# subtotechnoblade/Grok_Alpha_Zero

Measured on AMD Instinct MI355X. Metric: self-play positions/sec (whole node), Connect4 200 sims/move, 1/2/4/8 GPU, higher is better.
Workload: dtype bf16; 1 GPU; Connect4 6x7, 4096 concurrent games/GPU, 200 sims/move (MCTS.run iteration_limit), 6-block x128 ResNet bf16, puct self-play, random-init weights; games_per_gpu=4096, sims_per_move=200, evaluator=resnet

## Files before the change

### grok_alpha_zero_amd/build.py

```python
import os
import subprocess
from concurrent.futures import ThreadPoolExecutor

_PKG = os.path.dirname(os.path.abspath(__file__))
CSRC = os.path.join(_PKG, "csrc")
OBJ = os.path.join(CSRC, "build")
LIB = os.path.join(_PKG, "libgaz_engine.so")
HEADER = os.path.join(os.path.dirname(_PKG), "include", "gaz_engine.h")
UNITS = {
    "engine.hip": ["rt.hpp", "wave.hpp", "det.hpp", "games.hpp", "tree.hpp", "resign.hpp", "puct_core.hpp", "gumbel_core.hpp", "evaluator.hpp", "samples.hpp", "tree_export.hpp"],
    "resnet.hip": ["rt.hpp", "wave.hpp", "evaluator.hpp", "netops.hpp", "conv3x3.hpp", "conv_wide.hpp", "resblock.hpp", "trunk.hpp", "tile_perm.hpp", "net_host.hpp",
                   "det.hpp", "games.hpp", "tree.hpp", "resign.hpp", "puct_core.hpp", "gumbel_core.hpp"],
}
FLAGS = ["-O3", "--offload-arch=gfx950", "-fPIC", "-std=c++17", "-ffp-contract=off", "-Wno-unused-result", "-Wno-unused-value",
         "-Wno-int-to-pointer-cast"]


def _newer(target, deps):
    if not os.path.exists(target):
        return True
    t = os.path.getmtime(target)
    return any(os.path.getmtime(d) > t for d in deps)


def build_engine(force=False, verbose=False):
    hipcc = os.environ.get("HIPCC", "/opt/rocm/bin/hipcc")
    os.makedirs(OBJ, exist_ok=True)
    known = {h for hs in UNITS.values() for h in hs} | set(UNITS)
    extra = [f for f in os.listdir(CSRC) if f.endswith((".hpp", ".hip")) and f not in known]
    jobs = []
    for src, hdrs in UNITS.items():
        obj = os.path.join(OBJ, src.replace(".hip", ".o"))
        deps = [os.path.join(CSRC, src), HEADER, os.path.abspath(__file__)] + [os.path.join(CSRC, h) for h in hdrs + extra]
        if force or _newer(obj, deps):
            jobs.append([hipcc] + FLAGS + ["-c", os.path.join(CSRC, src), "-o", obj])

    def run(cmd):
        if verbose:
            print(" ".join(cmd), flush=True)
        subprocess.check_call(cmd, cwd=CSRC)
    with ThreadPoolExecutor(max_workers=max(len(jobs), 1)) as ex:
        list(ex.map(run, jobs))
    objs = [os.path.join(OBJ, s.replace(".hip", ".o")) for s in UNITS]
    if jobs or _newer(LIB, objs):
        run([hipcc, "--offload-arch=gfx950", "-shared", "-fPIC"] + objs + ["-o", LIB])
    return LIB
```

### grok_alpha_zero_amd/csrc/engine.hip

```cpp
#include <stdio.h>
#include <functional>
#include <string>
#include <vector>
#include "../../include/gaz_engine.h"
#include "rt.hpp"
#include "puct_core.hpp"
#include "gumbel_core.hpp"
#include "samples.hpp"
#include "tree_export.hpp"
#include "evaluator.hpp"

using namespace gaz;

static std::string g_create_error;

#define HIP_OK(expr)                                                                  \
    do { hipError_t _e = (expr); if (_e != hipSuccess) { return fail(std::string(#expr) + ": " + hipGetErrorString(_e)); } } while (0)

template <class G> GAZ_DEV void wave_body(const DevParams<G>& E, int g0, int g1) {
    constexpr int PER = WAVE / G::TEAM;
    GAZ_SHARED Scratch<G> S[PER];
    GAZ_SHARED PuctLocal<G> L[PER];
    const int t = team_in_wave<G>();
    const int g = g0 + block_id() * PER + t;
// ... 288 lines not shown
    atomic_add(reinterpret_cast<unsigned long long*>(out + 2), (unsigned long long)gs.n_evals);
    atomic_add(reinterpret_cast<unsigned long long*>(out + 4), (unsigned long long)gs.n_sims);
    atomic_add(reinterpret_cast<unsigned long long*>(out + 6), (unsigned long long)gs.n_plies);
    atomic_add(reinterpret_cast<unsigned long long*>(out + 8), (unsigned long long)gs.n_hits);
}

struct gaz_engine {
    gaz_engine_config cfg;
    std::string err;
    int grouped = 0;
    virtual void note_grouped() {}
    virtual ~gaz_engine() {}
    int fail(const std::string& m) { err = m; return 1; }
    virtual int init() = 0;
    virtual int load_weights(const gaz_tensor* t, int n) = 0;
    virtual int reset_games(const int32_t* slots, int n) = 0;
    virtual int run_move(int32_t* n_waiting) = 0;
    virtual int get_root_stats(uint32_t*, float*, float*, float*, uint32_t*, float*, int32_t*, int32_t*) = 0;
    virtual int apply_moves(const int32_t* moves) = 0;
    virtual int run_waves(int n) = 0;
    virtual int wave_begin() = 0;
    virtual int wave_end() = 0;
    virtual int batch_ptrs(void**, void**, void**) = 0;
    virtual int read_batch(int8_t*, int32_t*) = 0;
    virtual int batch_rows(int32_t*) = 0;
    virtual int write_outputs(const float*, const float*) = 0;
    virtual int evaluate(const int8_t*, int, float*, float*, int, double*) = 0;
    virtual int record_layout(gaz_record_layout*) = 0;
    virtual int drain(void* out, int max_records, int32_t* n_out) = 0;
    virtual int sample_layout(gaz_sample_layout*) = 0;
    virtual int drain_samples(int max_games, int64_t max_rows, int64_t plane_rows, int64_t row_base, int32_t* games, int8_t* boards, float* policies,
                              float* values, int32_t* n_games, int64_t* n_rows, int32_t* blocked_T) = 0;
    virtual int get_stats(uint64_t out[16]) = 0;
    virtual int synchronize() = 0;
    virtual int timing_reset(int enable) = 0;
    virtual int timing_get(double*, double*, double*, int64_t*, int64_t*) = 0;
    virtual int dominant(char*, int, double*) = 0;
    virtual int set_position(int, const int32_t*, int) = 0;
    virtual int set_search_params(int, int) = 0;
    virtual int stop_search(int) = 0;
    virtual int start_search() = 0;
    virtual int set_hyperparams(const gaz_search_hyperparams*) = 0;
    virtual int set_resignation(const gaz_resign_params*) = 0;
    virtual int get_resign_stats(uint64_t out[8]) = 0;
    virtual int set_eval_symmetry(int32_t mode) = 0;
    virtual int get_eval_symmetry(int32_t* mode) = 0;
    virtual int read_batch_symmetry(uint8_t* sym) = 0;
    virtual int set_solver(int32_t mode) = 0;
    virtual int get_solver(int32_t* mode) = 0;
    virtual int get_solver_stats(uint64_t out[8]) = 0;
    virtual int read_head_features(int, float*, float*, int32_t*, int32_t*) = 0;
    virtual int set_fused_wave(int) = 0;
    virtual int debug_fused_fault(int) = 0;
    virtual int read_positions(int32_t*, uint8_t*, int) = 0;
    typedef std::function<int(int64_t n_nodes, int64_t n_edges, gaz_tree_node** nodes, gaz_tree_edge** edges)> TreePlace;
    virtual int read_trees(const int32_t* slots, int n_slots, int tree, int max_depth, uint32_t min_visits, int64_t* node_first, int64_t* edge_first,
                           bool want_records, const TreePlace& place) = 0;
    virtual int read_pv(int tree, const int32_t* first_action, int max_len, uint8_t* actions, uint32_t* N, float* W, int32_t* len) = 0;
    int short_capacity(int64_t need_nodes, int64_t need_edges, int64_t max_nodes, int64_t max_edges) {
        return fail("read_trees: the export needs " + std::to_string(need_nodes) + " nodes and " + std::to_string(need_edges) + " edges, max_nodes is " +
                    std::to_string(max_nodes) + " and max_edges is " + std::to_string(max_edges));
    }
    virtual int repack(int32_t*, int32_t*) = 0;
    virtual int probe_rules(const int32_t*, const int32_t*, int, int, int8_t*, uint8_t*, int32_t*, int8_t*, int32_t*, const float*, float*) = 0;
};

struct CallScratch {
    std::vector<void*> p;
    ~CallScratch() { for (void* q : p) hipFree(q); }
    template <class T> T* get(size_t n) { void* q = nullptr; if (hipMalloc(&q, (n ? n : 1) * sizeof(T)) != hipSuccess) return nullptr; p.push_back(q); return (T*)q; }
};

static const char* group_fault(const gaz_engine_config& c, int k) {
    if (k < 2 || k > c.n_games) return "game_groups must be in [1, n_games]";
    if (c.sync_moves || c.evaluator == GAZ_EVAL_EXTERNAL) return "game_groups > 1 needs continuous self-play (sync_moves = 0) with a built-in evaluator";
    if (c.games_budget > 0 && c.games_budget < c.n_games) return "game_groups > 1 with a games_budget below n_games: a group could be left without a game (use game_groups = 1)";
    return nullptr;
}

static std::string config_fault(const gaz_engine_config& c, int groups) {
    if (c.game_groups < 0) return "game_groups must be >= 0";
    if (c.gumbel_batch < 0 || c.gumbel_batch > 64) return "gumbel_batch must be in [0, 64] (0 and 1 = one candidate of sequential halving per game and wave)";
    if (c.gumbel_batch > 1) {
        if (c.leaf_batch > 1) return "gumbel_batch > 1 cannot be combined with leaf_batch > 1";
        if (c.search != GAZ_SEARCH_GUMBEL) return "gumbel_batch > 1 needs search = GAZ_SEARCH_GUMBEL (the PUCT search has leaf_batch)";
        if (c.eval_cache_log2 > 0) return "gumbel_batch > 1 cannot be combined with eval_cache_log2 > 0";
        if (c.game_groups > 1) return "gumbel_batch > 1 cannot be combined with game_groups > 1";
    }
    if (c.leaf_batch < 0 || c.leaf_batch > 64) return "leaf_batch must be in [0, 64] (0 and 1 = one leaf per game and wave)";
    if (c.leaf_batch > 1) {
        if (c.search == GAZ_SEARCH_GUMBEL) return "leaf_batch > 1 needs search = GAZ_SEARCH_PUCT (the Gumbel search plans its simulations itself)";
        if (c.eval_cache_log2 > 0) return "leaf_batch > 1 cannot be combined with eval_cache_log2 > 0";
        if (c.game_groups > 1) return "leaf_batch > 1 cannot be combined with game_groups > 1";
    }
    if (c.fast_iterations < 0) return "fast_iterations must be >= 0 (0 = no playout cap), not " + std::to_string(c.fast_iterations);
    if (c.fast_iterations > c.run_iterations) return "fast_iterations (" + std::to_string(c.fast_iterations) + ") must not exceed run_iterations (" + std::to_string(c.run_iterations) + ")";
    if (c.fast_iterations > 0 && !(c.full_search_prob > 0.0 && c.full_search_prob <= 1.0)) return "full_search_prob must be in (0, 1] with fast_iterations > 0, not " + std::to_string(c.full_search_prob);
    if (c.fast_iterations == 0 && !(c.full_search_prob == 0.0)) return "full_search_prob must be 0 with fast_iterations = 0 (the playout cap is off)";
    if (c.fast_iterations > 0 && c.move_time_limit > 0.0) return "fast_iterations > 0 cannot be combined with move_time_limit > 0 (a timed move has no iteration cap to randomise)";
    if (c.forced_playouts_k != c.forced_playouts_k) return "forced_playouts_k must be a number (0 = no forced playouts), not NaN";
    if (c.forced_playouts_k < 0.0) return "forced_playouts_k must be >= 0 (0 = no forced playouts), not " + std::to_string(c.forced_playouts_k);
    if (c.forced_playouts_k > 1.7976931348623157e308) return "forced_playouts_k must be finite (KataGo uses 2), not infinity";
    if (c.forced_playouts_k > 0.0 && c.search == GAZ_SEARCH_GUMBEL) return "forced_playouts_k > 0 cannot be combined with search = GAZ_SEARCH_GUMBEL (sequential halving has no PUCT root to force playouts at)";
    if (groups > 1) { const char* g = group_fault(c, groups); return g ? g : ""; }
    int max_t = 0, n_act = 0;
    switch (c.game) {
// ... 188 lines not shown
        if (slots) {
            if (n > E.n_games) return fail("reset_games: too many slots");
            HIP_OK(hipMemcpyAsync(dSlots, slots, sizeof(int32_t) * n, hipMemcpyHostToDevice, stream));
            GAZ_LAUNCH(k_reset_games<G>, n, WAVE, stream, E, (const int32_t*)dSlots, n);
        } else {
            GAZ_LAUNCH(k_reset_games<G>, E.n_games, WAVE, stream, E, (const int32_t*)nullptr, E.n_games);
        }
        HIP_OK(hipGetLastError());
        return 0;
    }

    int new_event(hipEvent_t* e) { HIP_OK(hipEventCreate(e)); ev.push_back(*e); return 0; }
    static constexpr size_t MAX_TIMING_EVENTS = 1 << 16;

    bool prev_marked = false;
    DevParams<G> wave_params() { DevParams<G> P = E; P.wave_epoch = ++fuse_epoch; P.eval_done = prev_marked ? d_evaldone : nullptr; return P; }
    void launch_wave(hipStream_t st, int g0, int g1) { const DevParams<G> P = wave_params(); prev_marked = false; launch_wave(st, g0, g1, P); }
    void launch_wave(hipStream_t st, int g0, int g1, const DevParams<G>& E) {
        if (E.solver) { if (E.eval_symmetry) launch_wave_v<true, true>(st, g0, g1, E); else launch_wave_v<false, true>(st, g0, g1, E); return; }
        if (E.eval_symmetry) launch_wave_v<true>(st, g0, g1, E); else launch_wave_v<false>(st, g0, g1, E);
    }
    template <bool SYM, bool SOLVE = false> void launch_wave_v(hipStream_t st, int g0, int g1, const DevParams<G>& E) {
        typedef typename SolveSel<SOLVE, typename SymSel<SYM, typename PuctVariant<G>::type>::type>::type GP;
        typedef typename SolveSel<SOLVE, typename SymSel<SYM, G>::type>::type GS;
        if constexpr (!SOLVE) {
        if (gbk > 1) {
            constexpr int PER = WAVE / GP::TEAM;
            GAZ_LAUNCH(k_wave_gb<GP>, (g1 - g0 + PER - 1) / PER, WAVE, st, *reinterpret_cast<const DevParams<GP>*>(&E), GB, g0, g1);
            return;
        }
        if (lbk > 1) {
            constexpr int PER = WAVE / GP::TEAM;
            GAZ_LAUNCH(k_wave_lb<GP>, (g1 - g0 + PER - 1) / PER, WAVE, st, *reinterpret_cast<const DevParams<GP>*>(&E), LB, g0, g1);
            return;
        }
        if (cfg.search == GAZ_SEARCH_GUMBEL) {
            static const int gteams_env = env_int("GAZ_TREE_TEAMS", -1);
            constexpr int GPER = WAVE / GP::TEAM;
            if (GPER > 1 && gteams_env == 1) GAZ_LAUNCH(k_wave_gumbel_teams<GP>, (g1 - g0 + GPER - 1) / GPER, WAVE, st, *reinterpret_cast<const DevParams<GP>*>(&E), g0, g1);
            else GAZ_LAUNCH(k_wave_gumbel<GS>, g1 - g0, WAVE, st, *reinterpret_cast<const DevParams<GS>*>(&E), g0, g1);
            return;
        }
        }
        static const int teams_env = env_int("GAZ_TREE_TEAMS", -1);
        const bool teams = teams_env >= 0 ? teams_env != 0 : E.cache == nullptr;
        constexpr int PER = WAVE / GP::TEAM;
        if (PER > 1 && teams) GAZ_LAUNCH(k_wave_teams<GP>, (g1 - g0 + PER - 1) / PER, WAVE, st, *reinterpret_cast<const DevParams<GP>*>(&E), g0, g1);
        else GAZ_LAUNCH(k_wave<GS>, g1 - g0, WAVE, st, *reinterpret_cast<const DevParams<GS>*>(&E), g0, g1);
    }
    void launch_wave() { launch_wave(stream, 0, n_eff); }

    uint32_t* d_done = nullptr; uint32_t* d_evaldone = nullptr; int32_t* d_fault = nullptr;
    unsigned long long* d_queue = nullptr;
    uint32_t fuse_epoch = 0; int fuse_state = -1;
    uint64_t fuse_faults = 0;
    unsigned debug_fault_mod = 0;
    static constexpr unsigned SPIN_TICKS = 2000000;
    int poll_fuse_fault() {
        if (!d_fault) return 0;
        int32_t n = 0;
        HIP_OK(hipMemcpy(&n, d_fault, sizeof(n), hipMemcpyDeviceToHost));
        if (n) {
            fuse_faults += (uint64_t)n; n = 0; fuse_state = 0; debug_fault_mod = 0;
            fault_wave = waves_launched; fault_strikes++;
            HIP_OK(hipMemcpy(d_fault, &n, sizeof(n), hipMemcpyHostToDevice));
            fprintf(stderr, "[gaz_engine] fused tree + trunk launch: %llu trunk workgroup(s) gave up waiting for their games (dispatch order not as assumed); "
                            "falling back to separate launches%s\n", (unsigned long long)fuse_faults,
                    fault_strikes <= REARM_STRIKES ? " (the one-launch form is tried again after 20000 waves)" : " for good");
        }
        return 0;
    }
    int64_t waves_launched = 0, fault_wave = 0; int fault_strikes = 0;
    static constexpr int64_t REARM_WAVES = 20000; static constexpr int REARM_STRIKES = 2;
    bool can_fuse() {
        if (fuse_state == 0 && fault_strikes > 0 && fault_strikes <= REARM_STRIKES && d_queue_or_done() && waves_launched - fault_wave >= REARM_WAVES) fuse_state = 1;
        if (fuse_state >= 0) return fuse_state == 1;
        fuse_state = 0;
        if (lbk > 1) return false;
        static const bool off = !env_on("GAZ_FUSE_WAVE", true);
        typedef typename PuctVariant<G>::type GP;
        static const bool with_cache = env_on("GAZ_FUSE_CACHE", true);
        const bool gumbel = cfg.search == GAZ_SEARCH_GUMBEL;
        const bool gmk = G::ID == GAME_GMK && !gumbel && !E.cache && env_on("GAZ_FUSE_GOMOKU", true);
        const bool c4 = G::ID == GAME_C4 && WAVE / GP::TEAM >= 4 && !E.compact && !(E.cache && !with_cache);
        if (off || !(c4 || gmk) || !eval || !eval->supports_split()) return false;
        if (gumbel && (!env_on("GAZ_FUSE_GUMBEL", true) || E.cache)) return false;
        if (!gumbel && !env_on("GAZ_TREE_TEAMS", true)) return false;
        if (dalloc(&d_done, (size_t)E.n_games) || !ensure_skip_buffers()) return false;
        if (env_on("GAZ_FUSE_QUEUE", true) && dalloc(&d_queue, (size_t)E.n_games + 64)) return false;
        fuse_state = 1;
        return true;
    }

    bool d_queue_or_done() const { return d_done != nullptr; }
    bool fuse_enabled = true;
    int set_fused_wave(int on) override { fuse_enabled = on != 0; return 0; }
    bool ensure_skip_buffers() {
        if (d_evaldone) return true;
        if (dalloc(&d_evaldone, (size_t)E.n_games) || dalloc(&d_fault, 4)) return false;
        return true;
    }
    int debug_fused_fault(int mod) override {
        if (lbk > 1 && mod > 0) return fail(std::string("debug_fused_fault: ") + (gbk > 1 ? "gumbel_batch" : "leaf_batch") + " > 1 runs separate launches only");
        if (mod > 0 && !ensure_skip_buffers()) return 1;
        debug_fault_mod = mod > 0 ? (unsigned)mod : 0u;
        return 0;
    }

    int n_eff = 0;
    int32_t* dMoveList = nullptr;
    int repack(int32_t* n_active_out, int32_t* n_eff_out) override {
        if (E.sync_moves) return fail("repack needs continuous self-play (sync_moves = 0)");
        if (gbk > 1) return fail("repack: not with gumbel_batch > 1 (a game owns gumbel_batch rows of the batch)");
        if (lbk > 1) return fail("repack: not with leaf_batch > 1 (a game owns leaf_batch rows of the batch)");
        if (quiesce()) return 1;
        GAZ_LAUNCH(k_gather_root<G>, E.n_games, WAVE, stream, E, dN, dW, dP, dPol, dRV, dQ, dChosen, dPhase, dPending);
        std::vector<int32_t> ph(E.n_games);
        HIP_OK(hipMemcpyAsync(ph.data(), dPhase, (size_t)E.n_games * 4, hipMemcpyDeviceToHost, stream));
        HIP_OK(hipStreamSynchronize(stream));
        int n_active = 0;
        for (int g = 0; g < n_eff; ++g) n_active += ph[g] != PH_HALT;
        for (int g = n_eff; g < E.n_games; ++g) if (ph[g] != PH_HALT) return fail("repack: a slot beyond the live range is running");
        if (n_active_out) *n_active_out = n_active;
        const int n_new = n_active > 0 ? n_active : 1;
        std::vector<int32_t> mv;
        int hole = 0;
        for (int g = n_eff - 1; g >= n_new; --g) {
            if (ph[g] == PH_HALT) continue;
            while (hole < n_new && ph[hole] != PH_HALT) ++hole;
            if (hole >= n_new) return fail("repack: internal error (no hole left)");
            mv.push_back(g); mv.push_back(hole); ph[hole] = ph[g]; ph[g] = PH_HALT;
        }
        if (!mv.empty()) {
            if (!dMoveList && dalloc(&dMoveList, (size_t)2 * E.n_games)) return 1;
            HIP_OK(hipMemcpyAsync(dMoveList, mv.data(), mv.size() * 4, hipMemcpyHostToDevice, stream));
            const size_t slot_bytes = (size_t)2 * (E.compact ? 2 : 1) * (size_t)E.nodes_per_tree * (size_t)E.node_bytes;
            const size_t gbytes = cfg.search == GAZ_SEARCH_GUMBEL ? sizeof(GumbelState<G>) : 0;
            DevParams<G> Em = E; Em.eval_done = d_evaldone;
            GAZ_LAUNCH(k_move_slots<G>, (int)(mv.size() / 2), 256, stream, Em, (const int32_t*)dMoveList, (int)(mv.size() / 2), slot_bytes, gbytes);
            HIP_OK(hipGetLastError());
            HIP_OK(hipStreamSynchronize(stream));
        }
        n_eff = n_new;
        if (n_eff_out) *n_eff_out = n_eff;
        return 0;
    }

    int fused_wave(bool timing, hipEvent_t e0, hipEvent_t e1, hipEvent_t e2) {
        static const char* stamp_spec = getenv("GAZ_FUSED_STAMPS");
        static const long stamp_at = stamp_spec && strchr(stamp_spec, ':') ? atol(strchr(stamp_spec, ':') + 1) : 3000;
        unsigned long long* d_stamps = nullptr;
        const size_t stamp_blocks = (size_t)n_eff + 4096;
        if (stamp_spec && n_waves_total == stamp_at && hipMalloc((void**)&d_stamps, stamp_blocks * 128 * 8) == hipSuccess) hipMemsetAsync(d_stamps, 0, stamp_blocks * 128 * 8, stream);
        const FuseHandoff ho{d_done, fuse_epoch + 1, d_evaldone, d_fault, SPIN_TICKS, debug_fault_mod, d_stamps, d_queue};
        const void* plan = eval->trunk_plan(E.nn_in, n_eff, 0, ho);
        if (!plan) return -1;
        if (timing) hipEventRecord(e0, stream);
        DevParams<G> Ef = wave_params(); Ef.done_flag = d_done;
        if (eval->plan_uses_queue(plan)) {
            typedef typename PuctVariant<G>::type GPq;
            static const bool gumbel_teams = env_on("GAZ_FUSE_GUMBEL_TEAMS", true);
            static const int rounds_env = env_int("GAZ_FUSE_TREE_ROUNDS", 0);
            const int rounds = rounds_env > 0 ? rounds_env : (G::ID == GAME_GMK ? (this->grouped > 1 ? 4 : 8) : (cfg.search == GAZ_SEARCH_GUMBEL ? (this->grouped > 1 ? 2 : 4) : 1));
            const int gpb = G::ID == GAME_GMK ? rounds * 8 : rounds * 4 * ((cfg.search == GAZ_SEARCH_GUMBEL && !gumbel_teams) ? 1 : WAVE / GPq::TEAM);
            Ef.done_queue = d_queue; Ef.queue_gpb = gpb; Ef.queue_nfull = n_eff / gpb; Ef.queue_rem = n_eff % gpb;
        }
        Ef.handoff_release = G::ID == GAME_GMK;
        const bool launched = G::ID == GAME_GMK ? launch_wave_trunk_gmk(stream, &Ef, 0, n_eff, plan)
                            : cfg.search == GAZ_SEARCH_GUMBEL ? launch_wave_trunk_c4_gumbel(stream, &Ef, 0, n_eff, plan) : launch_wave_trunk_c4(stream, &Ef, 0, n_eff, plan);
        if (!launched) { fuse_state = 0; --fuse_epoch; return -1; }
        prev_marked = true;
        if (d_stamps) {
            std::vector<unsigned long long> hst(stamp_blocks * 128);
            hipStreamSynchronize(stream);
            hipMemcpy(hst.data(), d_stamps, hst.size() * 8, hipMemcpyDeviceToHost); hipFree(d_stamps);
            std::string path(stamp_spec); if (path.find(':') != std::string::npos) path = path.substr(0, path.find(':'));
            if (FILE* f = fopen(path.c_str(), "wb")) { fwrite(hst.data(), 8, hst.size(), f); fclose(f); }
        }
        if (timing) hipEventRecord(e1, stream);
        eval->forward_heads(stream, E.nn_policy, E.nn_value, n_eff, 0);
        if (E.cache) { Ef.eval_done = d_evaldone; GAZ_LAUNCH(k_cache_insert<G>, n_eff, WAVE, stream, Ef, 0, n_eff); E.cache_epoch++; }
        if (timing) {
            hipEventRecord(e2, stream); ev_eval.push_back({e0, e2}); n_waves_timed++;
            ev_fused.push_back({e0, e1});
        }
        n_waves_total++;
        return 0;
    }

    int one_wave(bool with_eval) {
        ++waves_launched;
        const bool timing = this->timing && n_waves_total % TIMING_STRIDE == 0 && ev.size() + 4 <= MAX_TIMING_EVENTS;
        hipEvent_t e0 = 0, e1 = 0, e2 = 0;
        if (timing && (new_event(&e0) || new_event(&e1) || new_event(&e2))) return 1;
        if (with_eval && eval && fuse_enabled && can_fuse()) { const int rc = fused_wave(timing, e0, e1, e2); if (rc >= 0) return rc; }
        if (timing) hipEventRecord(e0, stream);
        DevParams<G> P = wave_params();
        launch_wave(stream, 0, n_eff, P);
        prev_marked = false;
        if (timing) hipEventRecord(e1, stream);
        if (with_eval && eval) eval->forward(stream, E.nn_in, E.nn_policy, E.nn_value, n_eff * lbk, timing);
        if (timing) { hipEventRecord(e2, stream); ev_tree.push_back({e0, e1}); ev_eval.push_back({e1, e2}); n_waves_timed++; }
        P.eval_done = nullptr;
        if (with_eval && eval && debug_fault_mod && d_evaldone) {
            GAZ_LAUNCH(k_debug_skip<G>, n_eff, WAVE, stream, P, d_evaldone, n_eff, debug_fault_mod, d_fault);
            prev_marked = true; P.eval_done = d_evaldone;
        }
        if (with_eval && eval && E.cache) { GAZ_LAUNCH(k_cache_insert<G>, n_eff, WAVE, stream, P, 0, n_eff); E.cache_epoch++; }
        n_waves_total++;
        return 0;
    }

    hipStream_t tstream = 0, hstream = 0;
    static constexpr int MAXGRP = 8;
    int n_grp = 0, grp0[MAXGRP + 1] = {};
    hipEvent_t ev_tree_done[2][MAXGRP] = {}, ev_trunk_done[2][MAXGRP] = {}, ev_heads_done[2][MAXGRP] = {}, ev_join = 0;
    bool pipeline_ready = false;
    int quiesce() { HIP_OK(hipStreamSynchronize(stream)); if (pipeline_ready) { HIP_OK(hipStreamSynchronize(tstream)); HIP_OK(hipStreamSynchronize(hstream)); } return 0; }
    bool can_pipeline() {
        static const char* spec = getenv("GAZ_PIPELINE");
        if (!spec || !*spec || atoi(spec) == 0) return false;
        if (lbk > 1 || E.sync_moves || !eval || !eval->supports_split() || E.n_games < 1024 || E.cache || n_eff != E.n_games) return false;
        if (!pipeline_ready) {
            std::vector<int> sizes;
            if (strchr(spec, ',')) { for (const char* p = spec; *p;) { sizes.push_back(atoi(p)); p = strchr(p, ','); if (!p) break; ++p; } }
            else { const int round = eval->round_rows(); for (int left = E.n_games; left > 0; left -= round) sizes.push_back(left < round ? left : round); }
            int sum = 0; for (int v : sizes) sum += v;
            if (sizes.size() < 2 || sizes.size() > (size_t)MAXGRP || sum != E.n_games) return false;
            for (int v : sizes) if (v <= 0) return false;
            n_grp = (int)sizes.size(); grp0[0] = 0;
            for (int i = 0; i < n_grp; ++i) grp0[i + 1] = grp0[i] + sizes[i];
            int lo = 0, hi = 0;
            hipDeviceGetStreamPriorityRange(&lo, &hi);
// ... 684 lines not shown
        for (int c = 0; c < K(); ++c) {
            uint64_t s[16];
            if (up(kid[c], kid[c]->get_stats(s))) return 1;
            if (s[0] > out[0]) out[0] = s[0];
            for (int i = 1; i < 9; ++i) out[i] += s[i];
            out[10] += s[10]; out[13] += s[13];
            if (s[9] > out[9]) out[9] = s[9];
            if (!s[12]) out[12] = 0;
        }
        out[14] = (uint64_t)K();
        return 0;
    }
    int synchronize() override { return all(&gaz_engine::synchronize); }
    int timing_reset(int en) override { return all(&gaz_engine::timing_reset, en); }
    int timing_get(double* ms_tree, double* ms_eval, double* ms_dom, int64_t* n_dom, int64_t* n_waves) override {
        double t = 0, e = 0, d = 0; int64_t nd = 0, nw = 0;
        for (int c = 0; c < K(); ++c) {
            double a = 0, b = 0, x = 0; int64_t y = 0, z = 0;
            if (up(kid[c], kid[c]->timing_get(&a, &b, &x, &y, &z))) return 1;
            t += a; e += b; d += x; nd += y; if (z > nw) nw = z;
        }
        if (ms_tree) *ms_tree = t; if (ms_eval) *ms_eval = e; if (ms_dom) *ms_dom = d; if (n_dom) *n_dom = nd; if (n_waves) *n_waves = nw;
        return 0;
    }
    int dominant(char* name, int cap, double* flops) override { return lead(&gaz_engine::dominant, name, cap, flops); }
    int set_position(int slot, const int32_t* a, int n) override {
        if (slot < 0 || slot >= cfg.n_games) return fail("set_position: bad slot / history length");
        const int c = group_of(slot);
        return up(kid[c], kid[c]->set_position(slot - first[c], a, n));
    }
    int set_search_params(int it, int tau) override { return all(&gaz_engine::set_search_params, it, tau); }
    int stop_search(int s) override { return all(&gaz_engine::stop_search, s); }
    int start_search() override { return all(&gaz_engine::start_search); }
    int set_hyperparams(const gaz_search_hyperparams* hp) override { return all(&gaz_engine::set_hyperparams, hp); }
    int set_resignation(const gaz_resign_params* p) override { return all(&gaz_engine::set_resignation, p); }
    int set_eval_symmetry(int32_t mode) override { return all(&gaz_engine::set_eval_symmetry, mode); }
    int get_eval_symmetry(int32_t* mode) override { return lead(&gaz_engine::get_eval_symmetry, mode); }
    int set_solver(int32_t mode) override { return all(&gaz_engine::set_solver, mode); }
    int get_solver(int32_t* mode) override { return lead(&gaz_engine::get_solver, mode); }
    int get_solver_stats(uint64_t out[8]) override { return sum8(&gaz_engine::get_solver_stats, out); }
    int get_resign_stats(uint64_t out[8]) override { return sum8(&gaz_engine::get_resign_stats, out); }
    int read_head_features(int n, float* p, float* v, int32_t* p_row, int32_t* v_row) override {
        if (n < 0 || n > cfg.n_games) return fail("read_head_features: n must be in [0, n_games]");
        int32_t pr = 0, vr = 0;
        if (lead(&gaz_engine::read_head_features, 0, nullptr, nullptr, &pr, &vr)) return 1;
        if (p_row) *p_row = pr; if (v_row) *v_row = vr;
        return each([&](gaz_engine* k, int c) {
            const int nc = rows_of(c, n);
            return nc ? k->read_head_features(nc, p ? p + (size_t)first[c] * pr : p, v ? v + (size_t)first[c] * vr : v, nullptr, nullptr) : 0;
        });
    }
    int set_fused_wave(int on) override { return all(&gaz_engine::set_fused_wave, on); }
    int debug_fused_fault(int mod) override { return all(&gaz_engine::debug_fused_fault, mod); }
    int read_positions(int32_t* n_hist, uint8_t* hist, int stride) override {
        if (!n_hist || !hist || stride < lay.max_T) return fail("read_positions: hist must hold at least max_T actions per slot");
        return each([&](gaz_engine* k, int c) { return k->read_positions(n_hist + first[c], hist + (size_t)first[c] * stride, stride); });
    }
    int read_trees(const int32_t* slots, int n, int tree, int max_depth, uint32_t min_visits, int64_t* node_first, int64_t* edge_first,
                   bool want_records, const TreePlace& place) override {
        std::vector<std::vector<int32_t>> local(K()), pos(K());
        for (int i = 0; i < n; ++i) { const int c = group_of(slots[i]); local[c].push_back(slots[i] - first[c]); pos[c].push_back(i); }
        std::vector<std::vector<int64_t>> nf(K()), ef(K());
        std::vector<std::vector<gaz_tree_node>> tn(K()); std::vector<std::vector<gaz_tree_edge>> te(K());
        std::vector<int64_t> cn((size_t)n, 0), ce((size_t)n, 0);
        for (int c = 0; c < K(); ++c) {
            const int m = (int)local[c].size();
            nf[c].assign((size_t)m + 1, 0); ef[c].assign((size_t)m + 1, 0);
            const TreePlace stage = [&, c](int64_t nn, int64_t ne, gaz_tree_node** pn, gaz_tree_edge** pe) {
                tn[c].resize((size_t)nn + 1); te[c].resize((size_t)ne + 1); *pn = tn[c].data(); *pe = te[c].data(); return 0;
            };
            if (up(kid[c], kid[c]->read_trees(local[c].data(), m, tree, max_depth, min_visits, nf[c].data(), ef[c].data(), want_records, stage))) return 1;
            for (int j = 0; j < m; ++j) { cn[pos[c][j]] = nf[c][j + 1] - nf[c][j]; ce[pos[c][j]] = ef[c][j + 1] - ef[c][j]; }
        }
        node_first[0] = 0; edge_first[0] = 0;
        for (int i = 0; i < n; ++i) { node_first[i + 1] = node_first[i] + cn[i]; edge_first[i + 1] = edge_first[i] + ce[i]; }
        if (!want_records) return 0;
        gaz_tree_node* nodes = nullptr; gaz_tree_edge* edges = nullptr;
        if (place(node_first[n], edge_first[n], &nodes, &edges)) return 1;
        for (int c = 0; c < K(); ++c)
            for (size_t j = 0; j < pos[c].size(); ++j) {
                const int i = pos[c][j];
                if (cn[i]) memcpy(nodes + node_first[i], tn[c].data() + nf[c][j], sizeof(gaz_tree_node) * (size_t)cn[i]);
                if (ce[i]) memcpy(edges + edge_first[i], te[c].data() + ef[c][j], sizeof(gaz_tree_edge) * (size_t)ce[i]);
            }
        return 0;
    }
    int read_pv(int tree, const int32_t* fa, int max_len, uint8_t* actions, uint32_t* N, float* W, int32_t* len) override {
        return each([&](gaz_engine* k, int c) {
            const size_t o = (size_t)first[c] * (size_t)max_len;
            return k->read_pv(tree, fa ? fa + first[c] : fa, max_len, actions + o, N + o, W + o, len + first[c]);
        });
    }
    int repack(int32_t* n_active, int32_t* n_launch) override {
        int32_t a = 0, l = 0;
        if (each([&](gaz_engine* k, int) { int32_t x = 0, y = 0; if (k->repack(&x, &y)) return 1; a += x; l += y; return 0; })) return 1;
        if (n_active) *n_active = a; if (n_launch) *n_launch = l;
        return 0;
    }
    int probe_rules(const int32_t* actions, const int32_t* n_actions, int n_pos, int stride, int8_t* b, uint8_t* l, int32_t* w, int8_t* in, int32_t* t,
                    const float* pin, float* pout) override { return lead(&gaz_engine::probe_rules, actions, n_actions, n_pos, stride, b, l, w, in, t, pin, pout); }
};

static int choose_game_groups(const gaz_engine_config& c) {
    if (c.game_groups != 0) return c.game_groups;
    if (c.leaf_batch > 1 || c.gumbel_batch > 1) return 1;
    static const int env = env_int("GAZ_GAME_GROUPS", 0);
// ... 49 lines not shown
int gaz_engine_evaluate(gaz_engine* h, const int8_t* in, int32_t n, float* p, float* v, int32_t repeats, double* ms) { return h->evaluate(in, n, p, v, repeats, ms); }
int gaz_engine_record_layout(gaz_engine* h, gaz_record_layout* o) { return h->record_layout(o); }
int gaz_engine_drain_finished(gaz_engine* h, void* out, int32_t max_records, int32_t* n_out) { return h->drain(out, max_records, n_out); }
int gaz_engine_sample_layout(gaz_engine* h, gaz_sample_layout* o) { return o ? h->sample_layout(o) : h->fail("sample_layout: null argument"); }
int gaz_engine_drain_samples(gaz_engine* h, int32_t max_games, int64_t max_rows, int32_t* games, int8_t* boards, float* policies, float* values,
                             int32_t* n_games, int64_t* n_rows) {
    if (!games || !boards || !policies || !values || !n_games || !n_rows) return h->fail("drain_samples: null argument");
    if (max_games < 0 || max_rows < 0) return h->fail("drain_samples: max_games and max_rows must be >= 0");
    int32_t blocked = 0;
    if (h->drain_samples(max_games, max_rows, max_rows, 0, games, boards, policies, values, n_games, n_rows, &blocked)) return 1;
    if (*n_games == 0 && blocked)
        return h->fail("drain_samples: the oldest finished game has " + std::to_string(blocked) + " rows, max_rows is " + std::to_string(max_rows) +
                       " (no game was taken: call again with room for at least max_T rows)");
    return 0;
}
int gaz_engine_get_stats(gaz_engine* h, uint64_t out[16]) { return h->get_stats(out); }
int gaz_engine_synchronize(gaz_engine* h) { return h->synchronize(); }
int gaz_engine_timing_reset(gaz_engine* h, int32_t enable) { return h->timing_reset(enable); }
int gaz_engine_set_position(gaz_engine* h, int32_t slot, const int32_t* actions, int32_t n) { return h->set_position(slot, actions, n); }
int gaz_engine_set_search_params(gaz_engine* h, int32_t run_iterations, int32_t tau_mode) { return h->set_search_params(run_iterations, tau_mode); }
int gaz_engine_stop_search(gaz_engine* h, int32_t stop) { return h->stop_search(stop); }
int gaz_engine_start_search(gaz_engine* h) { return h->start_search(); }
int gaz_engine_set_hyperparams(gaz_engine* h, const gaz_search_hyperparams* hp) { return h->set_hyperparams(hp); }
int gaz_engine_set_resignation(gaz_engine* h, const gaz_resign_params* p) {
    if (!p) return h->fail("set_resignation: null argument");
    if (p->struct_size != sizeof(gaz_resign_params))
        return h->fail("set_resignation: struct_size is " + std::to_string(p->struct_size) + ", this library's gaz_resign_params has " + std::to_string(sizeof(gaz_resign_params)) + " bytes");
    if (p->threshold != p->threshold) return h->fail("set_resignation: threshold must be a number (0 = no resignation), not NaN");
    if (p->threshold > 1.7976931348623157e308 || p->threshold < -1.7976931348623157e308) return h->fail("set_resignation: threshold must be finite, not infinity");
    if (p->threshold < 0.0) return h->fail("set_resignation: threshold must be >= 0 (0 = no resignation), not " + std::to_string(p->threshold));
    if (p->threshold >= 1.0) return h->fail("set_resignation: threshold must be below 1 (q lies in [-1, 1], so no ply could trigger), not " + std::to_string(p->threshold));
    if (p->threshold == 0.0) return h->set_resignation(p);
    if (p->consecutive < 1 || p->consecutive > RESIGN_MAX_CONSECUTIVE)
        return h->fail("set_resignation: consecutive must be in [1, " + std::to_string(RESIGN_MAX_CONSECUTIVE) + "], not " + std::to_string(p->consecutive));
    if (p->min_ply < 0) return h->fail("set_resignation: min_ply must be >= 0, not " + std::to_string(p->min_ply));
    if (!(p->no_resign_prob >= 0.0 && p->no_resign_prob <= 1.0)) return h->fail("set_resignation: no_resign_prob must be in [0, 1], not " + std::to_string(p->no_resign_prob));
    return h->set_resignation(p);
}
int gaz_engine_get_resign_stats(gaz_engine* h, uint64_t out[8]) { return out ? h->get_resign_stats(out) : h->fail("get_resign_stats: null argument"); }
int gaz_engine_set_eval_symmetry(gaz_engine* h, int32_t mode) {
    if (mode != 0 && mode != 1) return h->fail("set_eval_symmetry: mode must be 0 (off) or 1 (a random board symmetry per evaluator request), not " + std::to_string(mode));
    return h->set_eval_symmetry(mode);
}
int gaz_engine_set_solver(gaz_engine* h, int32_t mode) {
    if (mode != 0 && mode != 1) return h->fail("set_solver: mode must be 0 (off) or 1 (prove wins, draws and losses in the PUCT tree), not " + std::to_string(mode));
    return h->set_solver(mode);
}
int gaz_engine_get_solver(gaz_engine* h, int32_t* mode) { return mode ? h->get_solver(mode) : h->fail("get_solver: null argument"); }
int gaz_engine_get_solver_stats(gaz_engine* h, uint64_t out[8]) { return out ? h->get_solver_stats(out) : h->fail("get_solver_stats: null argument"); }
int gaz_engine_get_eval_symmetry(gaz_engine* h, int32_t* mode) { return mode ? h->get_eval_symmetry(mode) : h->fail("get_eval_symmetry: null argument"); }
int gaz_engine_read_batch_symmetry(gaz_engine* h, uint8_t* sym) { return sym ? h->read_batch_symmetry(sym) : h->fail("read_batch_symmetry: null argument"); }
int gaz_engine_set_fused_wave(gaz_engine* h, int32_t on) { return h->set_fused_wave(on); }
int gaz_engine_debug_fused_fault(gaz_engine* h, int32_t mod) { return h->debug_fused_fault(mod); }
int gaz_engine_read_positions(gaz_engine* h, int32_t* n_hist, uint8_t* hist, int32_t stride) { return h->read_positions(n_hist, hist, stride); }
static int check_tree_arg(gaz_engine* h, const char* fn, int32_t tree) {
    if (tree < -1 || tree > 1) return h->fail(std::string(fn) + ": tree must be 0, 1 or -1 (the tree running the game's move), not " + std::to_string(tree));
    if (tree == 1 && (h->cfg.single_tree || h->cfg.search == GAZ_SEARCH_GUMBEL))
        return h->fail(std::string(fn) + ": tree = 1 on an engine with one tree per game (single_tree or the Gumbel search); use tree = 0 or -1");
    return 0;
}
int gaz_engine_read_trees(gaz_engine* h, const int32_t* slots, int32_t n_slots, int32_t tree, int32_t max_depth, uint32_t min_visits, int64_t max_nodes,
                          int64_t max_edges, gaz_tree_node* nodes, gaz_tree_edge* edges, int64_t* node_first, int64_t* edge_first) {
    if (n_slots < 0) return h->fail("read_trees: n_slots must be >= 0, not " + std::to_string(n_slots));
    if (!node_first || !edge_first || (n_slots > 0 && !slots)) return h->fail("read_trees: slots, node_first and edge_first must not be null");
    if (check_tree_arg(h, "read_trees", tree)) return 1;
    if ((nodes == nullptr) != (edges == nullptr)) return h->fail("read_trees: nodes and edges must both be given, or both be null (counting call)");
    if (nodes && (max_nodes < 0 || max_edges < 0)) return h->fail("read_trees: max_nodes and max_edges must be >= 0");
    for (int32_t i = 0; i < n_slots; ++i)
        if (slots[i] < 0 || slots[i] >= h->cfg.n_games)
            return h->fail("read_trees: slots[" + std::to_string(i) + "] = " + std::to_string(slots[i]) + " is out of range [0, " + std::to_string(h->cfg.n_games) + ")");
    const gaz_engine::TreePlace place = [&](int64_t nn, int64_t ne, gaz_tree_node** pn, gaz_tree_edge** pe) {
        if (nn > max_nodes || ne > max_edges) return h->short_capacity(nn, ne, max_nodes, max_edges);
        *pn = nodes; *pe = edges; return 0;
    };
    return h->read_trees(slots, n_slots, tree, max_depth, min_visits, node_first, edge_first, nodes != nullptr, place);
}
int gaz_engine_read_pv(gaz_engine* h, int32_t tree, const int32_t* first_action, int32_t max_len, uint8_t* actions, uint32_t* N, float* W, int32_t* len) {
    if (max_len <= 0) return h->fail("read_pv: max_len must be positive, not " + std::to_string(max_len));
    if (!actions || !N || !W || !len) return h->fail("read_pv: actions, N, W and len must not be null");
    if (check_tree_arg(h, "read_pv", tree)) return 1;
    return h->read_pv(tree, first_action, max_len, actions, N, W, len);
}
int gaz_engine_repack(gaz_engine* h, int32_t* n_active, int32_t* n_launch) { return h->repack(n_active, n_launch); }
int gaz_engine_read_head_features(gaz_engine* h, int32_t n, float* p, float* v, int32_t* p_row, int32_t* v_row) { return h->read_head_features(n, p, v, p_row, v_row); }
int gaz_engine_probe_rules(gaz_engine* h, const int32_t* actions, const int32_t* n_actions, int32_t n_positions, int32_t stride, int8_t* board,
                           uint8_t* legal, int32_t* winner, int8_t* input, int32_t* terminal, const float* policy_in, float* policy_out) {
    return h->probe_rules(actions, n_actions, n_positions, stride, board, legal, winner, input, terminal, policy_in, policy_out);
}
int gaz_engine_dominant_kernel(gaz_engine* h, char* name, int32_t cap, double* flops) { return h->dominant(name, cap, flops); }
int gaz_engine_timing_get(gaz_engine* h, double* a, double* b, double* c, int64_t* d, int64_t* e) { return h->timing_get(a, b, c, d, e); }

}
```

### grok_alpha_zero_amd/csrc/evaluator.hpp

```cpp
#pragma once
#include <string>
#include "../../include/gaz_engine.h"
#include "rt.hpp"

namespace gaz {

struct FuseHandoff { const unsigned* ready; unsigned epoch; unsigned* eval_done; int* fuse_fault; unsigned spin_ticks; unsigned test_fault_mod;
                     unsigned long long* stamps;
                     const unsigned long long* queue; };

struct Evaluator {
    virtual ~Evaluator() {}
    virtual int load(const gaz_tensor* t, int n, hipStream_t s, std::string* err) { (void)t; (void)n; (void)s; (void)err; return 0; }
    virtual void forward(hipStream_t s, const int8_t* in, float* policy, float* value, int n, bool timing, int p0 = 0) = 0;
    virtual bool supports_row_base() const { return false; }
    virtual bool supports_split() const { return false; }
    virtual int round_rows() const { return 0; }
    virtual void forward_trunk(hipStream_t s, const int8_t* in, int n, bool timing, int p0) { (void)s; (void)in; (void)n; (void)timing; (void)p0; }
    virtual void forward_heads(hipStream_t s, float* policy, float* value, int n, int p0) { (void)s; (void)policy; (void)value; (void)n; (void)p0; }
    virtual const void* trunk_plan(const int8_t* in, int n, int p0, const struct FuseHandoff& h) { (void)in; (void)n; (void)p0; (void)h; return nullptr; }
    virtual bool plan_uses_queue(const void* plan) const { (void)plan; return false; }
    virtual void set_shared_chip(bool on) { (void)on; }
    virtual bool ready() const { return true; }
    virtual void timing_reset() {}
    virtual void timing_get(double* ms, int64_t* launches) { *ms = 0; *launches = 0; }
    virtual const char* dominant_kernel(int n, double* flops) { (void)n; *flops = 0; return ""; }
    virtual bool head_features(const float** p_feat, const float** v_feat, int* p_row_floats, int* v_row_floats) { (void)p_feat; (void)v_feat; (void)p_row_floats; (void)v_row_floats; return false; }
};

GAZ_DEV uint32_t hash_row(const int8_t* s, int n, uint32_t seed) {
    uint32_t h = 2166136261u ^ seed;
    for (int i = 0; i < n; ++i) { h ^= (uint8_t)s[i]; h *= 16777619u; }
    h ^= h >> 16; h *= 0x85EBCA6Bu; h ^= h >> 13; h *= 0xC2B2AE35u; h ^= h >> 16;
    return h;
}

template <int UNUSED> GAZ_KERNEL_WIDE k_hash_eval(const int8_t* in, float* policy, float* value, int n, int row_bytes, int A, uint32_t salt) {
#ifdef GAZ_HOST_EMU
    const int first = block_id(), step = 1 << 30;
#else
    const int first = blockIdx.x * blockDim.x + threadIdx.x, step = gridDim.x * blockDim.x;
#endif
    for (int idx = first; idx < n * (A + 1); idx += step) {
        const int g = idx / (A + 1), a = idx % (A + 1);
        const int8_t* row = in + (size_t)g * row_bytes;
        if (a < A) {
            uint32_t h = hash_row(row, row_bytes, salt ^ ((uint32_t)(a + 1) * 0x9E3779B1u));
            policy[(size_t)g * A + a] = (float)((h >> 8) + 1u) * (1.0f / 16777216.0f);
        } else {
            uint32_t h = hash_row(row, row_bytes, salt ^ 0x51ED270Bu);
            value[g] = (float)(h >> 8) * (1.0f / 8388608.0f) - 1.0f;
        }
    }
}

struct HashEvaluator : Evaluator {
    int row_bytes, A; uint32_t salt;
    HashEvaluator(int rb, int a, uint32_t s) : row_bytes(rb), A(a), salt(s) {}
    void forward(hipStream_t s, const int8_t* in, float* policy, float* value, int n, bool, int = 0) override {
        const int total = n * (A + 1);
#ifdef GAZ_HOST_EMU
        GAZ_LAUNCH(k_hash_eval<0>, total, 1, s, in, policy, value, n, row_bytes, A, salt);
#else
        GAZ_LAUNCH(k_hash_eval<0>, (total + 255) / 256, 256, s, in, policy, value, n, row_bytes, A, salt);
#endif
    }
};

Evaluator* make_resnet_evaluator(const gaz_engine_config& cfg, int H, int W, int C, int A, std::string* err);
bool launch_wave_trunk_c4(hipStream_t s, const void* dev_params, int g0, int g1, const void* plan);
bool launch_wave_trunk_c4_gumbel(hipStream_t s, const void* dev_params, int g0, int g1, const void* plan);
bool launch_wave_trunk_gmk(hipStream_t s, const void* dev_params, int g0, int g1, const void* plan);

inline Evaluator* make_evaluator(const gaz_engine_config& cfg, int H, int W, int C, int A, std::string* err) {
// ... 9 lines not shown
```

### grok_alpha_zero_amd/csrc/resnet.hip

```cpp
#include <math.h>
#include <map>
#include <string>
#include <vector>
#include <algorithm>
#include "evaluator.hpp"
#include "conv3x3.hpp"
#include "conv_wide.hpp"
#include "netops.hpp"
#include "resblock.hpp"
#include "trunk.hpp"
#include "tile_perm.hpp"
#include "net_host.hpp"
#include "puct_core.hpp"
#include "gumbel_core.hpp"

namespace gaz {

struct Rb3Plan { int tm, halo, tile_rows; };
static Rb3Plan rb3_plan(int M, int H, int W, int n_cus) {
    Rb3Plan best{3, W + 1, 64 * 3 - 2 * (W + 1)}; double best_cost = 1e30;
    for (int aligned = 0; aligned < 2; ++aligned)
        for (int c = 2; c <= 4; ++c) {
            const int rows = aligned ? (64 * c / (H * W)) * (H * W) : 64 * c - 2 * (W + 1);
            if (rows <= 0) continue;
// ... 281 lines not shown
            const size_t rb = (size_t)min(b0 + p, a.B - 1) * F;
#pragma unroll
            for (int c = 0; c < 6; ++c) v[pi][c] = feat[rb + min(lane + 64 * c, F - 1)];
        }
#pragma unroll
        for (int pi = 0; pi < 4; ++pi) {
            const int p = wave + 8 * pi;
            const bool rok = b0 + p < a.B;
#pragma unroll
            for (int c = 0; c < 6; ++c) { const int k = lane + 64 * c; if (k < FP) fl[p * FP + k] = (rok && k < F) ? v[pi][c] : 0.0f; }
        }
        for (int p = wave; p < 32; p += 8)
            for (int k = lane + 64 * 6; k < FP; k += 64) fl[p * FP + k] = (b0 + p < a.B && k < F) ? feat[(size_t)min(b0 + p, a.B - 1) * F + k] : 0.0f;
    }
    __syncthreads();
    f32x16 acc;
#pragma unroll
    for (int r = 0; r < 16; ++r) acc[r] = 0.0f;
    for (int g0 = gA; g0 < gB; g0 += D) {
#pragma unroll
        for (int d = 0; d < D; ++d) {
            const int g = g0 + d;
            ldg(g + D - 1, bq[(d + D - 1) % D]);
            if (g < gB) {
                float av[G];
#pragma unroll
                for (int j = 0; j < G; ++j) av[j] = fl[l31 * FP + g * 2 * G + 2 * j + lhi];
#pragma unroll
                for (int j = 0; j < G; ++j) acc = __builtin_amdgcn_mfma_f32_32x32x2f32(av[j], bq[d][j], acc, 0, 0, 0);
            }
        }
    }
    float* part = fl + 32 * FP;
    if (half) {
#pragma unroll
        for (int r = 0; r < 16; ++r) part[(wq * 16 + r) * 64 + lane] = acc[r];
    }
    __syncthreads();
    if (half) return;
    const float s = a.scale[head][n], t = a.shift[head][n];
#pragma unroll
    for (int r = 0; r < 16; ++r) {
        const int row = (r & 3) + 8 * (r >> 2) + 4 * lhi;
        if (b0 + row < a.B) a.out[head][(size_t)(b0 + row) * 128 + n] = fmaxf((acc[r] + part[(wq * 16 + r) * 64 + lane]) * s + t, 0.0f);
    }
}

struct TailArgs {
    const float* p_d1; const float* v_d1;
    const float* p_w2; const float* p_b2; const float* p_w3; const float* p_b3;
    const float* v_w2; const float* v_b2; const float* v_w3; const float* v_b3;
    float* policy; float* value; int B, A, logits;
};
__device__ __forceinline__ float policy_entry(const float* lg, int nout, int o, int logits) {
    if (logits == 1) return lg[o];
    if (logits == 2) {
        float sum = 0.f;
        for (int k = 0; k < nout; ++k) { const float x = lg[k]; sum += x >= 0.0f ? x + 1.0f : 1.0f / (1.0f - x); }
        const float x = lg[o];
        return (x >= 0.0f ? x + 1.0f : 1.0f / (1.0f - x)) / sum;
    }
    float mx = lg[0];
    for (int k = 1; k < nout; ++k) mx = fmaxf(mx, lg[k]);
    float sum = 0.f;
    for (int k = 0; k < nout; ++k) sum += expf(lg[k] - mx);
    return expf(lg[o] - mx) / sum;
}
__global__ __launch_bounds__(128) void k_tail(TailArgs a) {
    __shared__ float w2l[128 * 64]; __shared__ float xl[16][128]; __shared__ float hl[16][64]; __shared__ float lg[16][64];
    __shared__ float w3l[64 * 8];
    const int head = blockIdx.y, tid = threadIdx.x, p = tid >> 3, q = tid & 7, b0 = blockIdx.x * 16;
    const float* d1 = head == 0 ? a.p_d1 : a.v_d1;
    const float* w2 = head == 0 ? a.p_w2 : a.v_w2; const float* b2 = head == 0 ? a.p_b2 : a.v_b2;
    const float* w3 = head == 0 ? a.p_w3 : a.v_w3; const float* b3 = head == 0 ? a.p_b3 : a.v_b3;
    const int nout = head == 0 ? a.A : 1;
    {
        float4 wv[16], xv[4];
#pragma unroll
        for (int c = 0; c < 16; ++c) wv[c] = reinterpret_cast<const float4*>(w2)[tid + 128 * c];
#pragma unroll
        for (int c = 0; c < 4; ++c) {
            const int i = tid + 128 * c, pp = min(b0 + i / 32, a.B - 1);
            xv[c] = reinterpret_cast<const float4*>(d1 + (size_t)pp * 128)[i % 32];
        }
#pragma unroll
        for (int c = 0; c < 16; ++c) reinterpret_cast<float4*>(w2l)[tid + 128 * c] = wv[c];
#pragma unroll
        for (int c = 0; c < 4; ++c) reinterpret_cast<float4*>(&xl[0][0])[tid + 128 * c] = xv[c];
        if (nout <= 8) {
            float w3v[4];
#pragma unroll
            for (int c = 0; c < 4; ++c) w3v[c] = w3[min(tid + 128 * c, 64 * nout - 1)];
#pragma unroll
            for (int c = 0; c < 4; ++c) w3l[tid + 128 * c] = w3v[c];
        }
    }
    __syncthreads();
    float acc[8];
#pragma unroll
    for (int j = 0; j < 8; ++j) acc[j] = b2[q * 8 + j];
    for (int k = 0; k < 128; ++k) {
        const float xv = xl[p][k];
        const float4 wa = *reinterpret_cast<const float4*>(&w2l[k * 64 + q * 8]), wb = *reinterpret_cast<const float4*>(&w2l[k * 64 + q * 8 + 4]);
        acc[0] += xv * wa.x; acc[1] += xv * wa.y; acc[2] += xv * wa.z; acc[3] += xv * wa.w;
        acc[4] += xv * wb.x; acc[5] += xv * wb.y; acc[6] += xv * wb.z; acc[7] += xv * wb.w;
    }
#pragma unroll
    for (int j = 0; j < 8; ++j) hl[p][q * 8 + j] = acc[j];
    __syncthreads();
    for (int o = q; o < nout; o += 8) {
        float z = b3[o];
        if (nout <= 8) { for (int k = 0; k < 64; ++k) z += hl[p][k] * w3l[k * nout + o]; }
        else { for (int k = 0; k < 64; ++k) z += hl[p][k] * w3[k * nout + o]; }
        lg[p][o] = z;
    }
    __syncthreads();
    if (b0 + p >= a.B) return;
    const int b = b0 + p;
    if (head == 0) {
        for (int o = q; o < nout; o += 8) a.policy[(size_t)b * a.A + o] = policy_entry(lg[p], nout, o, a.logits);
    } else if (q == 0) {
        a.value[b] = tanhf(lg[p][0]);
    }
}

struct HeadsC4Args {
    const float* feat[2]; const float* w1[2]; const float* s1[2]; const float* t1[2];
    const float* w2[2]; const float* b2[2]; const float* w3[2]; const float* b3[2];
    float* policy; float* value; int B, F, A, logits;
};
constexpr int HC4_THREADS = 256, HC4_POS = 32, HC4_XP = 132;
constexpr int HC4_FCH = 6, HC4_TAIL = 128 * 64 + HC4_POS * 64 + HC4_POS * 8;
static size_t heads_c4_lds_bytes(int F) { return (size_t)(std::max(HC4_POS * (F + 1), HC4_TAIL) + HC4_POS * HC4_XP + 64 * 8) * 4; }
__global__ __launch_bounds__(HC4_THREADS) void k_heads_c4(HeadsC4Args a) {
    typedef __attribute__((ext_vector_type(4))) float f32x4;
    extern __shared__ float fl[];
    constexpr int D = 12;
    const int tid = threadIdx.x, F = a.F, FP = F + 1, F4 = F >> 2;
    float* const w2l = fl; float* const hl = fl + 128 * 64; float* const lg = hl + HC4_POS * 64;
    float* const xl = fl + max(HC4_POS * FP, HC4_TAIL);
    float* const w3l = xl + HC4_POS * HC4_XP;
    const int lane = tid & 63, wave = tid >> 6, c = lane & 15, kq = lane >> 4, half = wave >> 1, n0 = (wave & 1) * 64 + c * 4;
    const int NG = F >> 4, NGH = (NG + 1) / 2, sA = half ? NGH * 4 : 0, sB = half ? NG * 4 : NGH * 4;
    const int p = tid >> 3, q = tid & 7;
    const int items = 2 * ((a.B + HC4_POS - 1) / HC4_POS);
    for (int item = blockIdx.x; item < items; item += gridDim.x) {
        const int head = item & 1, b0 = (item >> 1) * HC4_POS, nout = head == 0 ? a.A : 1;
        const float* feat = a.feat[head]; const float* w1 = a.w1[head]; const float* w3 = a.w3[head];
        float4 bq[D]; f32x4 wv[8];
        auto ldw = [&](int s) { return *reinterpret_cast<const float4*>(w1 + (size_t)min(4 * s + kq, F - 1) * 128 + n0); };
#pragma unroll
        for (int d = 0; d < D - 1; ++d) bq[d] = ldw(sA + d);
        {
            float w3v[2];
#pragma unroll
            for (int i = 0; i < 2; ++i) w3v[i] = w3[min(tid + HC4_THREADS * i, 64 * nout - 1)];
#pragma unroll 1
            for (int e0 = tid; e0 < HC4_POS * F4; e0 += HC4_THREADS * HC4_FCH) {
                float4 fv[HC4_FCH];
#pragma unroll
                for (int i = 0; i < HC4_FCH; ++i) {
                    const int e = min(e0 + HC4_THREADS * i, HC4_POS * F4 - 1), r = e / F4;
                    fv[i] = reinterpret_cast<const float4*>(feat + (size_t)min(b0 + r, a.B - 1) * F)[e - r * F4];
                }
#pragma unroll
                for (int i = 0; i < HC4_FCH; ++i) {
                    const int e = e0 + HC4_THREADS * i, r = e / F4, k = (e - r * F4) * 4;
                    if (e < HC4_POS * F4) {
                        const bool rok = b0 + r < a.B;
                        float* dst = fl + r * FP + k;
                        dst[0] = rok ? fv[i].x : 0.0f; dst[1] = rok ? fv[i].y : 0.0f; dst[2] = rok ? fv[i].z : 0.0f; dst[3] = rok ? fv[i].w : 0.0f;
                    }
                }
            }
#pragma unroll
            for (int i = 0; i < 2; ++i) w3l[tid + HC4_THREADS * i] = w3v[i];
#pragma unroll
            for (int i = 0; i < 8; ++i) wv[i] = reinterpret_cast<const f32x4*>(a.w2[head])[tid + HC4_THREADS * i];
        }
        __syncthreads();
        f32x4 acc[2][4];
#pragma unroll
        for (int m = 0; m < 2; ++m)
#pragma unroll
            for (int t = 0; t < 4; ++t) acc[m][t] = f32x4{0.0f, 0.0f, 0.0f, 0.0f};
        for (int s0 = sA; s0 < sB; s0 += D) {
#pragma unroll
            for (int d = 0; d < D; ++d) {
                const int s = s0 + d;
                if (s + D - 1 < sB) bq[(d + D - 1) % D] = ldw(s + D - 1);
                if (s < sB) {
#pragma unroll
                    for (int m = 0; m < 2; ++m) {
                        const float av = fl[(16 * m + c) * FP + 4 * s + kq];
                        acc[m][0] = __builtin_amdgcn_mfma_f32_16x16x4f32(av, bq[d].x, acc[m][0], 0, 0, 0);
                        acc[m][1] = __builtin_amdgcn_mfma_f32_16x16x4f32(av, bq[d].y, acc[m][1], 0, 0, 0);
                        acc[m][2] = __builtin_amdgcn_mfma_f32_16x16x4f32(av, bq[d].z, acc[m][2], 0, 0, 0);
                        acc[m][3] = __builtin_amdgcn_mfma_f32_16x16x4f32(av, bq[d].w, acc[m][3], 0, 0, 0);
                    }
                }
            }
        }
        if (half) {
#pragma unroll
            for (int m = 0; m < 2; ++m)
#pragma unroll
                for (int r = 0; r < 4; ++r)
                    *reinterpret_cast<float4*>(&xl[(16 * m + 4 * kq + r) * HC4_XP + n0]) = make_float4(acc[m][0][r], acc[m][1][r], acc[m][2][r], acc[m][3][r]);
        }
        __syncthreads();
        if (!half) {
            const float4 s = *reinterpret_cast<const float4*>(a.s1[head] + n0), t = *reinterpret_cast<const float4*>(a.t1[head] + n0);
#pragma unroll
            for (int m = 0; m < 2; ++m)
#pragma unroll
                for (int r = 0; r < 4; ++r) {
                    float4* x = reinterpret_cast<float4*>(&xl[(16 * m + 4 * kq + r) * HC4_XP + n0]);
                    const float4 pv = *x;
                    *x = make_float4(fmaxf((acc[m][0][r] + pv.x) * s.x + t.x, 0.0f), fmaxf((acc[m][1][r] + pv.y) * s.y + t.y, 0.0f),
                                     fmaxf((acc[m][2][r] + pv.z) * s.z + t.z, 0.0f), fmaxf((acc[m][3][r] + pv.w) * s.w + t.w, 0.0f));
                }
        }
#pragma unroll
        for (int i = 0; i < 8; ++i) reinterpret_cast<f32x4*>(w2l)[tid + HC4_THREADS * i] = wv[i];
        __syncthreads();
        {
            const float* b2 = a.b2[head];
            float h[8];
#pragma unroll
            for (int j = 0; j < 8; ++j) h[j] = b2[q * 8 + j];
            for (int k = 0; k < 128; ++k) {
                const float xv = xl[p * HC4_XP + k];
                const float4 wa = *reinterpret_cast<const float4*>(&w2l[k * 64 + q * 8]), wb = *reinterpret_cast<const float4*>(&w2l[k * 64 + q * 8 + 4]);
                h[0] += xv * wa.x; h[1] += xv * wa.y; h[2] += xv * wa.z; h[3] += xv * wa.w;
                h[4] += xv * wb.x; h[5] += xv * wb.y; h[6] += xv * wb.z; h[7] += xv * wb.w;
            }
#pragma unroll
            for (int j = 0; j < 8; ++j) hl[p * 64 + q * 8 + j] = h[j];
        }
        __syncthreads();
        for (int o = q; o < nout; o += 8) {
            float z = a.b3[head][o];
            for (int k = 0; k < 64; ++k) z += hl[p * 64 + k] * w3l[k * nout + o];
            lg[p * 8 + o] = z;
        }
        __syncthreads();
        const int b = b0 + p;
        if (b < a.B) {
            if (head == 0) { for (int o = q; o < nout; o += 8) a.policy[(size_t)b * a.A + o] = policy_entry(lg + p * 8, nout, o, a.logits); }
            else if (q == 0) a.value[b] = tanhf(lg[p * 8]);
        }
        __syncthreads();
    }
}

static bool net_width_supported(int f) { return f == 64 || f == 128 || f == 192 || f == 256; }
static std::string net_width_error(int f) {
    return "num_filters (net_filters) = " + std::to_string(f) + " is not supported: the Connect4 and Gomoku networks run num_filters in {64, 128, 192, 256}";
}

struct ResNetEvaluator : Evaluator {
    int H, W, C, A, HW, blocks, filters, nmax, logits;
    DeviceStore st;
    bf16_t *X = nullptr, *Aa = nullptr, *Hh = nullptr, *X2 = nullptr;
    bool fused = true;
    int stamp_calls = 0, n_cus = 256;
    bf16_t* stem_frag = nullptr;
    bool trunk_m16 = true;
    bool trunk_mix = true;
    bool trunk_whole = true;
    bool trunk = true;
    bool heads_one = true;
    int heads_wgs = 128;
    int heads_one_rows = 2048;
    bf16_t* trunk_w = nullptr; float* trunk_prm = nullptr;
    std::string dom_label;
    uint8_t *perm_big = nullptr, *perm_small = nullptr;
    unsigned boff_big = 0, boff_small = 0; int perm_clashes = 0;
    float *pfeat = nullptr, *vfeat = nullptr, *pd1 = nullptr, *vd1 = nullptr;
    bool loaded = false;
    TrunkTimer timer;
    int64_t n_trunk_launches = 0;

    int load(const gaz_tensor* t, int n, hipStream_t s, std::string* err) override {
        st.set_tensors(t, n);
        if (!load_tensors()) { *err = st.err; return 1; }
        hipStreamSynchronize(s);
        loaded = true;
        return 0;
    }
    bool load_tensors() {
        const int Fc = filters, F = HW * 8;
        if (!st.up_f32("stem.w", 9 * 128 * C) || !st.up_f32("stem.scale", 128) || !st.up_f32("stem.shift", 128)) return false;
        {
            if (C != 4) { st.err = "stem expects 4 input planes"; return false; }
            const std::vector<bf16_t> h = stem_fragments(st.by["stem.w"]->data, st.by["stem.scale"]->data, 4, 128);
            if (!(stem_frag = st.upload(h.data(), h.size()))) return false;
        }
        for (int i = 0; i < blocks; ++i) {
            const std::string b = "block" + std::to_string(i); const int cin = i == 0 && Fc != 128 ? 128 : Fc;
            if (!st.up_f32(b + ".bn1.scale", cin) || !st.up_f32(b + ".bn1.shift", cin)) return false;
            if (Fc == 128 ? !st.up_conv_pair(b + ".conv1.w", b + ".conv2.w", Fc)
                          : !st.up_conv(b + ".conv1.w", Fc, cin, 9, CONV_WIDE) || !st.up_conv(b + ".conv2.w", Fc, Fc, 9, CONV_WIDE)) return false;
            if (!st.up_f32(b + ".conv1.scale", Fc) || !st.up_f32(b + ".conv1.shift", Fc) || !st.up_f32(b + ".conv2.bias", Fc)) return false;
        }
        if (Fc != 128 && (!st.up_conv("block0.proj.w", Fc, 128, 1, CONV_WIDE) || !st.up_f32("block0.proj.bias", Fc) ||
                          !st.up_bias_sum("block0.bias2p", "block0.conv2.bias", "block0.proj.bias"))) return false;
        if (Fc == 128 && !st.pack_trunk(0, blocks, &trunk_w, &trunk_prm)) return false;
        if (env_on("GAZ_TILE_PERM", true) && !perm_big && 96 / HW >= 1 && Fc == 128) {
            unsigned want_big[8] = {0x007u, 0x049u, 0, 0, 0x1C0u, 0x124u, 0, 0}, want_small[6] = {0x007u, 0x1C0u, 0x049u, 0, 0, 0};
            const TileLayout lb = tile_layout(H, W, 128 / HW, 128, 64, 2, want_big), ls = tile_layout(H, W, 96 / HW, 96, 96, 3, want_small);
            const bool ok = !lb.perm.empty() && !ls.perm.empty() && lb.boff.size() <= 3 && ls.boff.size() <= 3;
            if (ok && (perm_big = st.upload(lb.perm.data(), lb.perm.size())) && (perm_small = st.upload(ls.perm.data(), ls.perm.size()))) {
                boff_big = boff_small = 0;
                for (size_t b = 0; b < lb.boff.size(); ++b) boff_big |= (unsigned)lb.boff[b] << (8 * b);
                for (size_t b = 0; b < ls.boff.size(); ++b) boff_small |= (unsigned)ls.boff[b] << (8 * b);
                perm_clashes = lb.clashes + ls.clashes;
            } else { perm_big = perm_small = nullptr; }
        }
        if (!st.up_conv("heads.conv.w", 32, Fc, 9, Fc == 128 ? CONV_MFMA : CONV_WIDE) || !st.up_f32("heads.conv.bias", 32)) return false;
        for (const char* pre : {"p", "v"}) {
            const std::string p = pre; const int nout = p == "p" ? A : 1;
            if (!st.up_f32(p + ".bn0.scale", F) || !st.up_f32(p + ".bn0.shift", F) || !st.up_f32(p + ".d1.w", (int64_t)F * 128) ||
                !st.up_f32(p + ".d1.scale", 128) || !st.up_f32(p + ".d1.shift", 128) || !st.up_f32(p + ".d2.w", 128 * 64) ||
                !st.up_f32(p + ".d2.bias", 64) || !st.up_f32(p + ".d3.w", 64 * nout) || !st.up_f32(p + ".d3.bias", nout)) return false;
        }
        return true;
    }

    void conv_trunk(hipStream_t s, const bf16_t* in, const bf16_t* w, const float* sA, const float* tA, const bf16_t* res,
                    bf16_t* out1, int act1, const float* sB, const float* tB, bf16_t* out2, int M) {
        ConvArgs a; memset(&a, 0, sizeof(a));
        a.in = in; a.wgt = w; a.scaleA = sA; a.shiftA = tA; a.res = res; a.out1 = out1; a.act1 = act1;
        a.scaleB = sB; a.shiftB = tB; a.out2 = out2; a.M = M; a.H = H; a.W = W;
        static const int variant = env_int("GAZ_CONV_VARIANT", 0);
        if (variant == 0) {
            const size_t lds = conv_lds_bytes<128, 128, 256, 1>();
            hipLaunchKernelGGL((k_conv3x3<128, 128, 256, 4, 2, 2, 2, 1, 1, 0>), dim3((M + 255) / 256), dim3(512), lds, s, a);
        } else {
            const size_t lds = conv_lds_bytes<128, 128, 128, 2>();
            hipLaunchKernelGGL((k_conv3x3<128, 128, 128, 2, 2, 2, 2, 2, 2, 0>), dim3((M + 127) / 128), dim3(256), lds, s, a);
        }
        n_trunk_launches++;
    }

    bool supports_row_base() const override { return true; }
    bool head_features(const float** p, const float** v, int* pr, int* vr) override { *p = pfeat; *v = vfeat; *pr = HW * 8; *vr = HW * 8; return true; }
    bool supports_split() const override { return filters == 128 && fused && trunk && trunk_whole && blocks > 0 && HW <= 128; }
    void make_trunk_plan(const int8_t* in, int n, int p0, bool mix_allowed, bool fill_big, TrunkLaunchPlan& P) {
        TrunkArgs& r = P.args; memset(&r, 0, sizeof(r));
        r.xin = this->X + (size_t)p0 * HW * 128; r.xout = this->X2 + (size_t)p0 * HW * 128; r.w = trunk_w; r.prm = trunk_prm; r.M = n * HW; r.H = H; r.W = W; r.nblocks = blocks;
        r.tile_rows = (128 / HW) * HW; r.stamps = nullptr; r.perm = perm_big; r.perm_small = perm_small; r.boff = boff_big; r.boff_small = boff_small;
        r.planes = in; r.stem_frag = reinterpret_cast<const uint4*>(stem_frag); r.stem_shift = st.g("stem.shift");
        r.hw = st.w("heads.conv.w"); r.hbias = st.g("heads.conv.bias"); r.p_fs = st.g("p.bn0.scale"); r.p_ft = st.g("p.bn0.shift");
        r.v_fs = st.g("v.bn0.scale"); r.v_ft = st.g("v.bn0.shift");
        r.p_feat = this->pfeat + (size_t)p0 * HW * 8; r.v_feat = this->vfeat + (size_t)p0 * HW * 8;
        const TrunkSplit sp = trunk_split(n, HW, n_cus, mix_allowed, fill_big);
        if (sp.mix) { r.n_big = sp.n_big; r.small_rows = (96 / HW) * HW; }
        P.nwg = sp.nwg; P.mix = sp.mix; P.lds_bytes = (unsigned)trunk_lds_bytes(128);
    }
    TrunkLaunchPlan fused_plan;
    const void* trunk_plan(const int8_t* in, int n, int p0, const FuseHandoff& h) override {
        if (!trunk_m16 || !loaded || !supports_split()) return nullptr;
        make_trunk_plan(in, n, p0, trunk_mix, shared_chip && perm_big && perm_small, fused_plan);
        TrunkArgs& r = fused_plan.args;
        r.ready = h.ready; r.epoch = h.epoch; r.eval_done = h.eval_done; r.fuse_fault = h.fuse_fault; r.spin_ticks = h.spin_ticks; r.test_fault_mod = h.test_fault_mod; r.stamps = h.stamps;
        r.queue = (perm_big && perm_small && fused_plan.mix) ? h.queue : nullptr;
        return &fused_plan;
    }
    bool plan_uses_queue(const void* plan) const override { return plan && static_cast<const TrunkLaunchPlan*>(plan)->args.queue != nullptr; }
    bool shared_chip = false;
    bool grouped = false;
    void set_shared_chip(bool on) override { static const bool off = !env_on("GAZ_GROUP_BIG_TILES", true); shared_chip = on && !off; grouped = on; }
    int round_rows() const override { return 2 * n_cus * (128 / HW); }
    void forward(hipStream_t s, const int8_t* in, float* policy, float* value, int n, bool timing, int p0 = 0) override {
        forward_trunk(s, in, n, timing, p0);
        forward_heads(s, policy, value, n, p0);
    }
    void forward_trunk(hipStream_t s, const int8_t* in, int n, bool timing, int p0) override {
        if (!loaded) return;
        if (filters != 128) { forward_trunk_wide(s, in, n, timing, p0); return; }
        const int M = n * HW;
        bf16_t* const X = this->X + (size_t)p0 * HW * 128; bf16_t* const X2 = this->X2 + (size_t)p0 * HW * 128;
        bf16_t* const Aa = this->Aa + (size_t)p0 * HW * 128; bf16_t* const Hh = this->Hh + (size_t)p0 * HW * 128;
        float* const pfeat = this->pfeat + (size_t)p0 * HW * 8; float* const vfeat = this->vfeat + (size_t)p0 * HW * 8;
        StemArgs sa; sa.in = in; sa.w = st.g("stem.w"); sa.scale = st.g("stem.scale"); sa.shift = st.g("stem.shift");
        sa.scaleB = blocks ? st.g("block0.bn1.scale") : st.g("stem.scale"); sa.shiftB = blocks ? st.g("block0.bn1.shift") : st.g("stem.shift");
        sa.out1 = X; sa.out2 = fused ? nullptr : Aa; sa.M = M; sa.H = H; sa.W = W;
        const bool use_trunk = fused && trunk && blocks > 0 && HW <= 128;
        const bool whole = use_trunk && trunk_whole;
        if (whole) {
        } else if (fused) {
            StemMArgs sm; memset(&sm, 0, sizeof(sm)); sm.in = in; sm.wfrag = reinterpret_cast<const uint4*>(stem_frag); sm.shift = st.g("stem.shift"); sm.out = X;
            sm.M = M; sm.H = H; sm.W = W;
            launch_stem_mfma<4, 128, true, false>(s, sm);
        } else {
            hipLaunchKernelGGL(k_stem, dim3((M + 63) / 64), dim3(256), 0, s, sa);
        }
        timer.begin(s, timing);
        bf16_t* cur = X;
        if (use_trunk) {
            TrunkLaunchPlan P; make_trunk_plan(in, n, p0, whole && trunk_mix, false, P);
            TrunkArgs& r = P.args;
            const int nwg = P.nwg; const bool mix = P.mix;
            static const char* stamp_path = getenv("GAZ_TRUNK_STAMPS");
            StampDump stamps(stamp_path && ++stamp_calls == 3 ? stamp_path : nullptr, (size_t)nwg * 128, s);
            r.stamps = stamps.dev;
            if (mix && trunk_m16 && r.perm && r.perm_small) hipLaunchKernelGGL((k_trunk_mix<8, 2, true, true, true, true>), dim3(nwg), dim3(TR_THREADS), trunk_lds_bytes(128), s, r);
            else if (mix && trunk_m16) hipLaunchKernelGGL((k_trunk_mix<8, 2, true, true, true>), dim3(nwg), dim3(TR_THREADS), trunk_lds_bytes(128), s, r);
            else if (whole && trunk_m16) hipLaunchKernelGGL((k_trunk<2, 2, 8, 2, true, true, false, true>), dim3(nwg), dim3(TR_THREADS), trunk_lds_bytes(128), s, r);
            else if (mix) hipLaunchKernelGGL((k_trunk_mix<8, 2, true, true>), dim3(nwg), dim3(TR_THREADS), trunk_lds_bytes(128), s, r);
            else if (whole) hipLaunchKernelGGL((k_trunk<2, 2, 8, 2, true, true>), dim3(nwg), dim3(TR_THREADS), trunk_lds_bytes(128), s, r);
            else hipLaunchKernelGGL((k_trunk<2, 2, 8, 2, false, false>), dim3(nwg), dim3(TR_THREADS), trunk_lds_bytes(128), s, r);
            stamps.finish();
            cur = X2;
        }
        for (int i = 0; fused && !use_trunk && i < blocks; ++i) {
            const std::string b = "block" + std::to_string(i);
            ResBlockArgs r; r.xin = cur; r.xout = cur == X ? X2 : X; r.w1 = st.w(b + ".conv1.w"); r.w2 = st.w(b + ".conv2.w");
            r.s1 = st.g(b + ".bn1.scale"); r.t1 = st.g(b + ".bn1.shift"); r.s2 = st.g(b + ".conv1.scale"); r.t2 = st.g(b + ".conv1.shift");
            r.b2 = st.g(b + ".conv2.bias"); r.M = M; r.H = H; r.W = W; r.stamps = nullptr;
            static const int rbv = env_int("GAZ_RB", 3);
            static const int rb_tm = env_int("GAZ_RB_TM", 0);
            static const int rb_ring = env_int("GAZ_RB_RING", 8);
            Rb3Plan plan = rb3_plan(M, H, W, n_cus);
            if (rb_tm) plan = Rb3Plan{rb_tm, W + 1, 64 * rb_tm - 2 * (W + 1)};
            const int bmo = rbv == 3 ? plan.tile_rows : RB_ROWS - 2 * (W + 1);
            const size_t lds = conv_lds_bytes<128, 128, 256, 1>();
            const int nwg = (M + bmo - 1) / bmo;
            static const char* stamp_path = getenv("GAZ_RB_STAMPS");
            StampDump stamps(stamp_path && i == 1 && ++stamp_calls == 3 ? stamp_path : nullptr, (size_t)nwg * RB_STAMPS, s);
            r.stamps = stamps.dev;
            if (rbv == 3) rb3_launch(s, r, plan, rb_ring);
            else hipLaunchKernelGGL(k_resblock, dim3(nwg), dim3(RB_THREADS), lds, s, r);
            stamps.finish();
            cur = r.xout;
        }
        for (int i = 0; !fused && i < blocks; ++i) {
            const std::string b = "block" + std::to_string(i), nb = "block" + std::to_string(i + 1);
            conv_trunk(s, Aa, st.w(b + ".conv1.w"), st.g(b + ".conv1.scale"), st.g(b + ".conv1.shift"), nullptr, Hh, ACT_RELU,
                       nullptr, nullptr, nullptr, M);
            const bool last = i + 1 == blocks;
            conv_trunk(s, Hh, st.w(b + ".conv2.w"), nullptr, st.g(b + ".conv2.bias"), X, X, ACT_NONE,
                       last ? nullptr : st.g(nb + ".bn1.scale"), last ? nullptr : st.g(nb + ".bn1.shift"), last ? nullptr : Aa, M);
        }
        timer.end(s);
        if (!whole) {
            HeadsConvArgs hc; hc.in = cur; hc.wgt = st.w("heads.conv.w"); hc.bias = st.g("heads.conv.bias");
            hc.p_fs = st.g("p.bn0.scale"); hc.p_ft = st.g("p.bn0.shift"); hc.v_fs = st.g("v.bn0.scale"); hc.v_ft = st.g("v.bn0.shift");
            hc.p_feat = pfeat; hc.v_feat = vfeat; hc.M = M; hc.H = H; hc.W = W;
            hipLaunchKernelGGL(k_conv_heads, dim3((M + HC_ROWS - 1) / HC_ROWS), dim3(RB3_THREADS), hc_lds_bytes(), s, hc);
        }
    }
    void forward_trunk_wide(hipStream_t s, const int8_t* in, int n, bool timing, int p0) {
        const int M = n * HW, CW = std::max(filters, 128);
        bf16_t* const X = this->X + (size_t)p0 * HW * CW; bf16_t* const X2 = this->X2 + (size_t)p0 * HW * CW;
        bf16_t* const Aa = this->Aa + (size_t)p0 * HW * CW; bf16_t* const Hh = this->Hh + (size_t)p0 * HW * CW;
        float* const pfeat = this->pfeat + (size_t)p0 * HW * 8; float* const vfeat = this->vfeat + (size_t)p0 * HW * 8;
        StemMArgs sm; memset(&sm, 0, sizeof(sm)); sm.in = in; sm.wfrag = reinterpret_cast<const uint4*>(stem_frag); sm.shift = st.g("stem.shift"); sm.out = X;
        sm.M = M; sm.H = H; sm.W = W;
        launch_stem_mfma<4, 128, true, false>(s, sm);
        WideTrunk t; t.stem_c = 128; t.F = filters; t.blocks = blocks; t.M = M; t.H = H; t.W = W;
        t.x0 = X; t.a0 = X2; t.x = X2; t.a = Aa; t.h = Hh; t.policy_preact = false;
        gaz::forward_trunk_wide(s, st, timer, timing, t);
        WideConvArgs h; memset(&h, 0, sizeof(h));
        h.in = X2; h.wgt = st.w("heads.conv.w"); h.shiftA = st.g("heads.conv.bias"); h.M = M; h.H = H; h.W = W;
        h.feat_p = pfeat; h.feat_v = vfeat; h.p_fs = st.g("p.bn0.scale"); h.p_ft = st.g("p.bn0.shift"); h.v_fs = st.g("v.bn0.scale"); h.v_ft = st.g("v.bn0.shift");
        with_width(filters, [&](auto Fc) { conv_wide_launch<decltype(Fc)::value, 32, 9, 0, CW_EPI_HEADS>(s, h); });
    }
    void forward_heads(hipStream_t s, float* policy, float* value, int n, int p0) override {
        if (!loaded) return;
        float* const pfeat = this->pfeat + (size_t)p0 * HW * 8; float* const vfeat = this->vfeat + (size_t)p0 * HW * 8;
        float* const pd1 = this->pd1 + (size_t)p0 * 128; float* const vd1 = this->vd1 + (size_t)p0 * 128;
        const int F = HW * 8;
        if (heads_one && filters == 128 && F % 16 == 0 && F <= 384 && A <= 8 && !(grouped && n > heads_one_rows)) {
            HeadsC4Args h; h.B = n; h.F = F; h.A = A; h.logits = logits; h.policy = policy; h.value = value;
            h.feat[0] = pfeat; h.feat[1] = vfeat;
            for (int i = 0; i < 2; ++i) {
                const std::string p = i == 0 ? "p" : "v";
                h.w1[i] = st.g(p + ".d1.w"); h.s1[i] = st.g(p + ".d1.scale"); h.t1[i] = st.g(p + ".d1.shift");
                h.w2[i] = st.g(p + ".d2.w"); h.b2[i] = st.g(p + ".d2.bias"); h.w3[i] = st.g(p + ".d3.w"); h.b3[i] = st.g(p + ".d3.bias");
            }
            const int items = 2 * ((n + HC4_POS - 1) / HC4_POS);
            hipLaunchKernelGGL(k_heads_c4, dim3(grouped ? std::min(items, heads_wgs) : items), dim3(HC4_THREADS), heads_c4_lds_bytes(F), s, h);
            return;
        }
        Dense1Args d; d.B = n; d.F = F;
        d.feat[0] = pfeat; d.w[0] = st.g("p.d1.w"); d.scale[0] = st.g("p.d1.scale"); d.shift[0] = st.g("p.d1.shift"); d.out[0] = pd1;
        d.feat[1] = vfeat; d.w[1] = st.g("v.d1.w"); d.scale[1] = st.g("v.d1.scale"); d.shift[1] = st.g("v.d1.shift"); d.out[1] = vd1;
        hipLaunchKernelGGL(k_dense1_mfma, dim3((n + 31) / 32, 2), dim3(D1_THREADS), (size_t)32 * ((F + 15) / 16 * 16 + 1) * 4 + 4 * 16 * 64 * 4, s, d);
        TailArgs t; t.p_d1 = pd1; t.v_d1 = vd1; t.p_w2 = st.g("p.d2.w"); t.p_b2 = st.g("p.d2.bias"); t.p_w3 = st.g("p.d3.w");
        t.p_b3 = st.g("p.d3.bias"); t.v_w2 = st.g("v.d2.w"); t.v_b2 = st.g("v.d2.bias"); t.v_w3 = st.g("v.d3.w"); t.v_b3 = st.g("v.d3.bias");
        t.policy = policy; t.value = value; t.B = n; t.A = A; t.logits = logits;
        hipLaunchKernelGGL(k_tail, dim3((n + 15) / 16, 2), dim3(128), 0, s, t);
    }

    bool ready() const override { return loaded; }
    void timing_reset() override { timer.reset(); n_trunk_launches = 0; }
    void timing_get(double* ms, int64_t* launches) override {
        *ms = timer.total_ms();
        const bool per_forward = filters != 128 || (fused && trunk);
        *launches = timer.brackets() * (per_forward ? 1 : (fused ? 1 : 2) * blocks);
    }
    const char* dominant_kernel(int n, double* flops) override {
        if (filters != 128) {
            const double Fw = filters, rows = (double)n * HW;
            *flops = 2.0 * rows * (9.0 * 128.0 * Fw + 9.0 * Fw * Fw + 128.0 * Fw) + 2.0 * rows * 2.0 * 9.0 * Fw * Fw * (blocks - 1);
            dom_label = "k_conv_wide (the residual trunk at " + std::to_string(filters) + " filters, priced per forward: block 0 = 3x3 conv 128->F + 3x3 conv "
                        "F->F with the 1x1 projection 128->F in one accumulator, then blocks - 1 x two 3x3 convs F->F; implicit GEMM on v_mfma_f32_32x32x16_bf16)";
            return dom_label.c_str();
        }
        const double conv = 2.0 * (double)n * HW * 128.0 * 1152.0;
        *flops = fused ? 2 * conv : conv;
        if (fused && trunk) {
            *flops = 2 * conv * blocks;
            if (trunk_whole && trunk_m16 && trunk_mix && perm_big && perm_small) {
                const TrunkSplit sp = trunk_split(n, HW, n_cus, true, false);
                const bool mix = sp.mix;
                const double share = n > 0 && mix ? (sp.n_big * 128.0 * 30.0 / 36.0 + sp.n_small * 96.0 * 45.0 / 54.0) / ((double)n * HW) : 1.0;
                char buf[640];
                snprintf(buf, sizeof(buf), "k_trunk_mix (stem + the whole residual trunk + heads' first conv in one launch: blocks x two 3x3 convs 128->128 counted, "
                         "implicit GEMM on v_mfma_f32_16x16x32_bf16, activations resident in LDS; the cells of each board edge form whole MFMA tiles that sit out "
                         "the taps on which they read only zero padding: MFMA work issued = %.3f of the counted FLOPs)", share);
                dom_label = buf;
                if (mix) return dom_label.c_str();
            }
            if (trunk_whole) return trunk_m16 ? "k_trunk_mix (stem + the whole residual trunk + heads' first conv in one launch: blocks x two 3x3 convs 128->128 counted, implicit GEMM on v_mfma_f32_16x16x32_bf16, activations resident in LDS)"
                                              : "k_trunk_mix (stem + the whole residual trunk + heads' first conv in one launch: blocks x two 3x3 convs 128->128 counted, implicit GEMM on v_mfma_f32_32x32x16_bf16, activations resident in LDS)";
            return trunk_m16 ? "k_trunk (the whole residual trunk: blocks x two 3x3 convs 128->128, implicit GEMM on v_mfma_f32_16x16x32_bf16, activations resident in LDS)"
                             : "k_trunk (the whole residual trunk: blocks x two 3x3 convs 128->128, implicit GEMM on v_mfma_f32_32x32x16_bf16, activations resident in LDS)";
        }
        return fused ? "k_resblock3 (whole residual block: two 3x3 convs 128->128, implicit GEMM on MFMA 32x32x16 bf16)"
                     : "k_conv3x3<128,128> (trunk 3x3 conv, implicit GEMM on MFMA 32x32x16 bf16)";
    }
};
// ... 361 lines not shown
    if (!gomoku && cfg.net_filters != 64 && cfg.net_filters != 0 && cfg.net_filters != 128) { *err = "TicTacToe net uses 64 filters"; return nullptr; }
    if (cfg.net_blocks < 1 || cfg.net_blocks > 64) { *err = "net_blocks out of range"; return nullptr; }
    GenericEvaluator* e = new GenericEvaluator();
    e->H = H; e->W = W; e->C = C; e->A = A; e->HW = H * W; e->blocks = cfg.net_blocks; e->F = gomoku ? cfg.net_filters : 64; e->nmax = cfg.n_games;
    e->logits = cfg.policy_is_logits; e->gomoku = gomoku;
    e->fused = env_on("GAZ_FUSED", true);
    e->trunk = env_on("GAZ_TRUNK", true);
    e->trunk_m16 = env_on("GAZ_TRUNK_M16", true);
    e->block0_in_trunk = env_on("GAZ_BLOCK0_IN_TRUNK", true);
    e->stem_in_trunk_ok = env_on("GAZ_STEM_IN_TRUNK", false);
    { hipDeviceProp_t pr; int dev = 0; hipGetDevice(&dev); if (hipGetDeviceProperties(&pr, dev) == hipSuccess) e->n_cus = pr.multiProcessorCount; }
    const size_t M = (size_t)cfg.n_games * e->HW, SC = gomoku ? 256 : 128, F = e->F, n = cfg.n_games;
    e->X0 = e->st.dalloc<bf16_t>(M * SC); e->A0 = e->st.dalloc<bf16_t>(M * SC); e->X = e->st.dalloc<bf16_t>(M * F); e->Aa = e->st.dalloc<bf16_t>(M * F);
    e->Hh = e->st.dalloc<bf16_t>(M * F); e->Va = e->st.dalloc<bf16_t>(M * F); e->PH = e->st.dalloc<bf16_t>(M * 32); e->VH = e->st.dalloc<bf16_t>(M * 32);
    e->pfeat = e->st.dalloc<float>(n * e->HW * 8); e->vfeat = e->st.dalloc<float>(n * e->HW * 8); e->pd1 = e->st.dalloc<float>(n * 512); e->vd1 = e->st.dalloc<float>(n * 256);
    e->pd2 = e->st.dalloc<float>(n * 128); e->vd2 = e->st.dalloc<float>(n * 128); e->plog = e->st.dalloc<float>(n * 256);
    if (!e->X0 || !e->A0 || !e->X || !e->Aa || !e->Hh || !e->Va || !e->PH || !e->VH || !e->pfeat || !e->vfeat || !e->pd1 || !e->vd1 || !e->pd2 || !e->vd2 || !e->plog) {
        *err = "hipMalloc failed"; delete e; return nullptr;
    }
    hipFuncSetAttribute((const void*)(k_block0<4, 4>), hipFuncAttributeMaxDynamicSharedMemorySize, (int)rb3_lds_bytes<4>());
    hipFuncSetAttribute((const void*)k_conv_head32, hipFuncAttributeMaxDynamicSharedMemorySize, (int)hc_lds_bytes());
    hipFuncSetAttribute((const void*)(k_trunk<4, 2, 4, 2, false, false, true>), hipFuncAttributeMaxDynamicSharedMemorySize, (int)trunk_lds_bytes(256, true));
    hipFuncSetAttribute((const void*)(k_trunk<2, 2, 8, 2, false, false, false, true, 8>), hipFuncAttributeMaxDynamicSharedMemorySize, (int)trunk_lds_bytes(256));
    hipFuncSetAttribute((const void*)(k_trunk<2, 2, 8, 2, false, false, false, true, 8, true>), hipFuncAttributeMaxDynamicSharedMemorySize, (int)trunk_lds_bytes(256));
    hipFuncSetAttribute((const void*)(k_trunk<2, 2, 8, 2, false, false, false, true, 8, true, 0, true>), hipFuncAttributeMaxDynamicSharedMemorySize, (int)trunk_lds_bytes_s0());
    hipFuncSetAttribute((const void*)(k_resblock3<4, 4>), hipFuncAttributeMaxDynamicSharedMemorySize, (int)rb3_lds_bytes<4>());
    hipFuncSetAttribute((const void*)(k_conv3x3<128, 128, 256, 4, 2, 2, 2, 1, 1, 0, 9>), hipFuncAttributeMaxDynamicSharedMemorySize, 160 * 1024);
    hipFuncSetAttribute((const void*)(k_conv3x3<256, 128, 128, 2, 2, 2, 2, 4, 1, 0, 9>), hipFuncAttributeMaxDynamicSharedMemorySize, 160 * 1024);
    hipFuncSetAttribute((const void*)(k_conv3x3<256, 128, 128, 2, 2, 2, 2, 4, 1, 0, 1>), hipFuncAttributeMaxDynamicSharedMemorySize, 160 * 1024);
    hipFuncSetAttribute((const void*)(k_conv3x3<128, 128, 256, 4, 2, 2, 2, 1, 1, 0, 1>), hipFuncAttributeMaxDynamicSharedMemorySize, 160 * 1024);
    hipFuncSetAttribute((const void*)(k_conv3x3<128, 32, 256, 8, 1, 1, 1, 1, 1, 0, 9>), hipFuncAttributeMaxDynamicSharedMemorySize, 160 * 1024);
    hipFuncSetAttribute((const void*)k_dense, hipFuncAttributeMaxDynamicSharedMemorySize, 64 * 1024);
    return e;
}

Evaluator* make_resnet_evaluator(const gaz_engine_config& cfg, int H, int W, int C, int A, std::string* err) {
    if (H == 15 && W == 15) return make_generic_evaluator(cfg, H, W, C, A, true, err);
    if (H == 3 && W == 3) return make_generic_evaluator(cfg, H, W, C, A, false, err);
    if (!(H == 6 && W == 7 && C == 4)) { *err = "no network is defined for this board"; return nullptr; }
    if (!net_width_supported(cfg.net_filters)) { *err = net_width_error(cfg.net_filters); return nullptr; }
    if (cfg.net_blocks < 1 || cfg.net_blocks > 64) { *err = "net_blocks out of range"; return nullptr; }
    ResNetEvaluator* e = new ResNetEvaluator();
    e->H = H; e->W = W; e->C = C; e->A = A; e->HW = H * W; e->blocks = cfg.net_blocks; e->filters = cfg.net_filters; e->nmax = cfg.n_games;
    e->logits = cfg.policy_is_logits;
    const size_t M = (size_t)cfg.n_games * e->HW, CW = std::max(cfg.net_filters, 128);
    e->X2 = e->st.dalloc<bf16_t>(M * CW + 1024); e->fused = env_on("GAZ_FUSED", true);
    e->trunk = env_on("GAZ_TRUNK", true);
    e->trunk_whole = env_on("GAZ_TRUNK_WHOLE", true);
    e->trunk_mix = env_on("GAZ_TRUNK_MIX", true);
    e->trunk_m16 = env_on("GAZ_TRUNK_M16", true);
    e->heads_one = env_on("GAZ_HEADS_ONE", true);
    e->heads_wgs = std::max(1, env_int("GAZ_HEADS_WGS", e->heads_wgs));
    e->heads_one_rows = env_int("GAZ_HEADS_ONE_ROWS", e->heads_one_rows);
    { hipDeviceProp_t pr; int dev = 0; hipGetDevice(&dev); if (hipGetDeviceProperties(&pr, dev) == hipSuccess) e->n_cus = pr.multiProcessorCount; }
    e->X = e->st.dalloc<bf16_t>(M * CW + 1024); e->Aa = e->st.dalloc<bf16_t>(M * CW + 1024); e->Hh = e->st.dalloc<bf16_t>(M * CW + 1024);
    e->pfeat = e->st.dalloc<float>((size_t)cfg.n_games * e->HW * 8); e->vfeat = e->st.dalloc<float>((size_t)cfg.n_games * e->HW * 8);
    e->pd1 = e->st.dalloc<float>((size_t)cfg.n_games * 128); e->vd1 = e->st.dalloc<float>((size_t)cfg.n_games * 128);
    if (!e->X || !e->Aa || !e->Hh || !e->pfeat || !e->vfeat || !e->pd1 || !e->vd1) { *err = "hipMalloc failed"; delete e; return nullptr; }
    hipFuncSetAttribute((const void*)k_resblock, hipFuncAttributeMaxDynamicSharedMemorySize, 160 * 1024);
    hipFuncSetAttribute((const void*)(k_resblock3<4, 4>), hipFuncAttributeMaxDynamicSharedMemorySize, (int)rb3_lds_bytes<4>());
    hipFuncSetAttribute((const void*)k_conv_heads, hipFuncAttributeMaxDynamicSharedMemorySize, (int)hc_lds_bytes());
    hipFuncSetAttribute((const void*)k_heads_c4, hipFuncAttributeMaxDynamicSharedMemorySize, (int)heads_c4_lds_bytes(384));
    hipFuncSetAttribute((const void*)(k_trunk<2, 2, 8, 2, true, true>), hipFuncAttributeMaxDynamicSharedMemorySize, (int)trunk_lds_bytes(128));
    hipFuncSetAttribute((const void*)(k_trunk_mix<8, 2, true, true>), hipFuncAttributeMaxDynamicSharedMemorySize, (int)trunk_lds_bytes(128));
    hipFuncSetAttribute((const void*)(k_trunk<2, 2, 8, 2, true, true, false, true>), hipFuncAttributeMaxDynamicSharedMemorySize, (int)trunk_lds_bytes(128));
    hipFuncSetAttribute((const void*)(k_trunk_mix<8, 2, true, true, true>), hipFuncAttributeMaxDynamicSharedMemorySize, (int)trunk_lds_bytes(128));
    hipFuncSetAttribute((const void*)(k_trunk_mix<8, 2, true, true, true, true>), hipFuncAttributeMaxDynamicSharedMemorySize, (int)trunk_lds_bytes(128));
    hipFuncSetAttribute((const void*)(k_trunk<2, 2, 8, 2, false, false>), hipFuncAttributeMaxDynamicSharedMemorySize, (int)trunk_lds_bytes(128));
    hipFuncSetAttribute((const void*)(k_conv3x3<128, 128, 256, 4, 2, 2, 2, 1, 1, 0>), hipFuncAttributeMaxDynamicSharedMemorySize, 160 * 1024);
    hipFuncSetAttribute((const void*)(k_conv3x3<128, 128, 128, 2, 2, 2, 2, 2, 2, 0>), hipFuncAttributeMaxDynamicSharedMemorySize, 160 * 1024);
    return e;
}

}

namespace gaz {

typedef TeamGame<GAME_C4> GP4;

#ifndef GAZ_TREE_ROLE_ATTR
#define GAZ_TREE_ROLE_ATTR __forceinline__
#endif
template <class GP, class LOCAL, bool GUMBEL, int THREADS = TR_THREADS, size_t LDS_BYTES = trunk_lds_bytes(96)>
__device__ GAZ_TREE_ROLE_ATTR void tree_role(const DevParams<GP>& E, int g0, int g1, uint4* lds) {
    constexpr int PER = WAVE / GP::TEAM, NT = (THREADS / WAVE) * PER;
    Scratch<GP>* S = reinterpret_cast<Scratch<GP>*>(lds);
    LOCAL* L = reinterpret_cast<LOCAL*>(S + NT);
    uint32_t* rank = reinterpret_cast<uint32_t*>(L + NT);
    static_assert(NT * (sizeof(Scratch<GP>) + sizeof(LOCAL)) + 16 <= LDS_BYTES, "tree scratch must fit the trunk's LDS allocation");
    if (E.done_queue) {
        if (threadIdx.x == 0) *rank = 0;
        __syncthreads();
    }
    const int w = threadIdx.x >> 6, t = team_in_wave<GP>(), i = w * PER + t;
    const int per_block = E.done_queue ? E.queue_gpb : NT;
    for (int r = 0; r * NT < per_block; ++r) {
        const int g = g0 + (int)blockIdx.x * per_block + r * NT + w * PER + t;
        if (g < g1) {
            if constexpr (GUMBEL) g_game_step<GP>(E, g, S[i], L[i], rank, (int)blockIdx.x);
            else game_step<GP>(E, g, S[i], L[i], rank, (int)blockIdx.x);
        }
    }
}

template <bool MIX, bool SKIP, class GP, class LOCAL, bool GUMBEL>
__device__ __forceinline__ void wave_trunk_body(const DevParams<GP>& E, int g0, int g1, int n_tree_blocks, const TrunkArgs& a) {
    if ((int)blockIdx.x < n_tree_blocks) {
        extern __shared__ uint4 lds[];
        const DevParams<GP> El = E;
        if (a.stamps && (threadIdx.x & 63) == 0) a.stamps[(size_t)blockIdx.x * 128 + (threadIdx.x >> 6)] = wall_clock64();
        tree_role<GP, LOCAL, GUMBEL>(El, g0, g1, lds);
        if (a.stamps && (threadIdx.x & 63) == 0) a.stamps[(size_t)blockIdx.x * 128 + 4 + (threadIdx.x >> 6)] = wall_clock64();
        return;
    }
    const int bid = (int)blockIdx.x - n_tree_blocks;
    if (MIX && bid >= a.n_big) trunk_tile<3, 4, 8, true, true, false, true, 4, false, SKIP ? 2 : 0>(a, (long)a.n_big * a.tile_rows + (long)(bid - a.n_big) * a.small_rows, a.small_rows, SKIP ? a.perm_small : nullptr, a.boff_small);
    else trunk_tile<2, 2, 8, true, true, false, true, 4, false, SKIP ? 1 : 0>(a, (long)bid * a.tile_rows, a.tile_rows, SKIP ? a.perm : nullptr, a.boff);
}

template <bool MIX, bool SKIP, bool SYM = false, bool SOLVE = false> __global__ __launch_bounds__(TR_THREADS, 2) void k_wave_trunk(DevParams<typename SolveSel<SOLVE, typename SymSel<SYM, GP4>::type>::type> E, int g0, int g1, int n_tree_blocks, TrunkArgs a) {
    typedef typename SolveSel<SOLVE, typename SymSel<SYM, GP4>::type>::type GP;
    wave_trunk_body<MIX, SKIP, GP, PuctLocal<GP>, false>(E, g0, g1, n_tree_blocks, a);
}

typedef Game<GAME_GMK> GGMK;
template <bool SYM, bool SOLVE = false> __global__ __launch_bounds__(512, 1) void k_wave_trunk_gmk(DevParams<typename SolveSel<SOLVE, typename SymSel<SYM, GGMK>::type>::type> E, int g0, int g1, int n_tree_blocks, TrunkArgs a) {
    typedef typename SolveSel<SOLVE, typename SymSel<SYM, GGMK>::type>::type GP;
    if ((int)blockIdx.x < n_tree_blocks) {
        extern __shared__ uint4 lds[];
        if (a.stamps && (threadIdx.x & 63) == 0) a.stamps[(size_t)blockIdx.x * 128 + (threadIdx.x >> 6)] = wall_clock64();
        tree_role<GP, PuctLocal<GP>, false, 512, trunk_lds_bytes_s0()>(E, g0, g1, lds);
        if (a.stamps && (threadIdx.x & 63) == 0) a.stamps[(size_t)blockIdx.x * 128 + 8 + (threadIdx.x >> 6)] = wall_clock64();
        return;
    }
    const int bid = (int)blockIdx.x - n_tree_blocks;
    trunk_tile<2, 2, 8, false, false, false, true, 8, true, 0, true>(a, (long)bid * a.tile_rows, a.tile_rows, nullptr, 0);
}

template <class GP> static bool wave_trunk_launch(void (*kernel)(DevParams<GP>, int, int, int, TrunkArgs), int threads, int games_per_block, hipStream_t s,
                                                  const void* dev_params, int g0, int g1, const void* plan) {
    if (!plan || !dev_params) return false;
    const TrunkLaunchPlan& P = *static_cast<const TrunkLaunchPlan*>(plan);
    const DevParams<GP>& E = *static_cast<const DevParams<GP>*>(dev_params);
    const int per_block = E.done_queue ? E.queue_gpb : games_per_block, n_tree = (g1 - g0 + per_block - 1) / per_block;
    hipLaunchKernelGGL(kernel, dim3(n_tree + P.nwg), dim3(threads), P.lds_bytes, s, E, g0, g1, n_tree, P.args);
    return true;
}

bool launch_wave_trunk_gmk(hipStream_t s, const void* dev_params, int g0, int g1, const void* plan) {
    const bool sym = dev_params && static_cast<const DevParams<GGMK>*>(dev_params)->eval_symmetry != 0;
    const bool solve = dev_params && static_cast<const DevParams<GGMK>*>(dev_params)->solver != 0;
    static bool attr = false;
    if (!attr) {
        hipFuncSetAttribute((const void*)k_wave_trunk_gmk<false>, hipFuncAttributeMaxDynamicSharedMemorySize, (int)trunk_lds_bytes_s0());
        hipFuncSetAttribute((const void*)k_wave_trunk_gmk<true>, hipFuncAttributeMaxDynamicSharedMemorySize, (int)trunk_lds_bytes_s0());
        hipFuncSetAttribute((const void*)k_wave_trunk_gmk<false, true>, hipFuncAttributeMaxDynamicSharedMemorySize, (int)trunk_lds_bytes_s0());
        hipFuncSetAttribute((const void*)k_wave_trunk_gmk<true, true>, hipFuncAttributeMaxDynamicSharedMemorySize, (int)trunk_lds_bytes_s0());
        attr = true;
    }
    if (solve && sym) return wave_trunk_launch<WithSolve<WithSym<GGMK>>>(k_wave_trunk_gmk<true, true>, 512, 8, s, dev_params, g0, g1, plan);
    if (solve) return wave_trunk_launch<WithSolve<GGMK>>(k_wave_trunk_gmk<false, true>, 512, 8, s, dev_params, g0, g1, plan);
    if (sym) return wave_trunk_launch<WithSym<GGMK>>(k_wave_trunk_gmk<true>, 512, 8, s, dev_params, g0, g1, plan);
    return wave_trunk_launch<GGMK>(k_wave_trunk_gmk<false>, 512, 8, s, dev_params, g0, g1, plan);
}

template <bool MIX, bool SKIP, bool TEAMS, bool SYM = false> __global__ __launch_bounds__(TR_THREADS, 2) void k_wave_trunk_gumbel(DevParams<typename SymSel<SYM, Game<GAME_C4>>::type> E, int g0, int g1, int n_tree_blocks, TrunkArgs a) {
    typedef typename SymSel<SYM, GP4>::type GT;
    typedef typename SymSel<SYM, Game<GAME_C4>>::type GW;
    if constexpr (TEAMS) wave_trunk_body<MIX, SKIP, GT, GumbelLocal<GT>, true>(*reinterpret_cast<const DevParams<GT>*>(&E), g0, g1, n_tree_blocks, a);
    else wave_trunk_body<MIX, SKIP, GW, GumbelLocal<GW>, true>(E, g0, g1, n_tree_blocks, a);
}

bool launch_wave_trunk_c4_gumbel(hipStream_t s, const void* dev_params, int g0, int g1, const void* plan) {
    const bool sym = dev_params && static_cast<const DevParams<GP4>*>(dev_params)->eval_symmetry != 0;
    static const bool teams = env_on("GAZ_FUSE_GUMBEL_TEAMS", true);
    const TrunkLaunchPlan* P = static_cast<const TrunkLaunchPlan*>(plan);
    if (!P || !P->mix || !(P->args.perm && P->args.perm_small)) return false;
    if (sym) return wave_trunk_launch<WithSym<Game<GAME_C4>>>(teams ? k_wave_trunk_gumbel<true, true, true, true> : k_wave_trunk_gumbel<true, true, false, true>, TR_THREADS,
                                                              (TR_THREADS / WAVE) * (teams ? WAVE / GP4::TEAM : 1), s, dev_params, g0, g1, plan);
    return wave_trunk_launch<Game<GAME_C4>>(teams ? k_wave_trunk_gumbel<true, true, true> : k_wave_trunk_gumbel<true, true, false>, TR_THREADS,
                                            (TR_THREADS / WAVE) * (teams ? WAVE / GP4::TEAM : 1), s, dev_params, g0, g1, plan);
}

bool launch_wave_trunk_c4(hipStream_t s, const void* dev_params, int g0, int g1, const void* plan) {
    const bool sym = dev_params && static_cast<const DevParams<GP4>*>(dev_params)->eval_symmetry != 0;
    const TrunkLaunchPlan* P = static_cast<const TrunkLaunchPlan*>(plan);
    const bool mix = P && P->mix, skip = P && P->args.perm && P->args.perm_small;
    const bool solve = dev_params && static_cast<const DevParams<GP4>*>(dev_params)->solver != 0;
    if (solve && sym) return wave_trunk_launch<WithSolve<WithSym<GP4>>>(mix && skip ? k_wave_trunk<true, true, true, true> : mix ? k_wave_trunk<true, false, true, true> : k_wave_trunk<false, false, true, true>,
                                                                       TR_THREADS, (TR_THREADS / WAVE) * (WAVE / GP4::TEAM), s, dev_params, g0, g1, plan);
    if (solve) return wave_trunk_launch<WithSolve<GP4>>(mix && skip ? k_wave_trunk<true, true, false, true> : mix ? k_wave_trunk<true, false, false, true> : k_wave_trunk<false, false, false, true>,
                                                        TR_THREADS, (TR_THREADS / WAVE) * (WAVE / GP4::TEAM), s, dev_params, g0, g1, plan);
    if (sym) return wave_trunk_launch<WithSym<GP4>>(mix && skip ? k_wave_trunk<true, true, true> : mix ? k_wave_trunk<true, false, true> : k_wave_trunk<false, false, true>, TR_THREADS,
                                                    (TR_THREADS / WAVE) * (WAVE / GP4::TEAM), s, dev_params, g0, g1, plan);
    return wave_trunk_launch<GP4>(mix && skip ? k_wave_trunk<true, true> : mix ? k_wave_trunk<true, false> : k_wave_trunk<false, false>, TR_THREADS,
                                  (TR_THREADS / WAVE) * (WAVE / GP4::TEAM), s, dev_params, g0, g1, plan);
}

}
```

### grok_alpha_zero_amd/csrc/trunk.hpp

```cpp
#pragma once
#include "resblock.hpp"

namespace gaz {

struct TrunkArgs {
    const bf16_t* xin; bf16_t* xout;
    const bf16_t* w;
    const float* prm;
    int M, H, W, nblocks;
    int tile_rows;
    int n_big, small_rows;
    unsigned long long* stamps;
    const int8_t* planes; const uint4* stem_frag; const float* stem_shift;
    const unsigned* ready; unsigned epoch;
    unsigned* eval_done; int* fuse_fault; unsigned spin_ticks;
    const unsigned long long* queue;
    unsigned test_fault_mod;
    const bf16_t* x0; const float* prm0;
    const uint8_t* perm; const uint8_t* perm_small;
    unsigned boff, boff_small;
    const bf16_t* hw; const float* hbias;
    const float* p_fs; const float* p_ft; const float* v_fs; const float* v_ft; float* p_feat; float* v_feat;
};

struct TrunkLaunchPlan { TrunkArgs args; int nwg; int mix; unsigned lds_bytes; };

typedef float f32x2_t __attribute__((ext_vector_type(2)));
__device__ __forceinline__ float gelu_as(float v) {
    const float x = fabsf(v) * 0.70710678118654752440f;
    const float t = __builtin_amdgcn_rcpf(__builtin_fmaf(0.3275911f, x, 1.0f));
    float p = __builtin_fmaf(t, 1.061405429f, -1.453152027f);
    p = __builtin_fmaf(t, p, 1.421413741f); p = __builtin_fmaf(t, p, -0.284496736f); p = __builtin_fmaf(t, p, 0.254829592f);
    p = p * t;
    const float e = __builtin_amdgcn_exp2f((x * x) * -1.44269504088896340736f);
    p = (0.5f * p) * e;
    return v * (v < 0.0f ? p : 1.0f - p);
}
__device__ __forceinline__ f32x2_t gelu_as2(f32x2_t v) {
    const f32x2_t av = {fabsf(v.x), fabsf(v.y)};
    const f32x2_t x = av * 0.70710678118654752440f;
    const f32x2_t d = __builtin_elementwise_fma((f32x2_t)(0.3275911f), x, (f32x2_t)(1.0f));
    const f32x2_t t = {__builtin_amdgcn_rcpf(d.x), __builtin_amdgcn_rcpf(d.y)};
    f32x2_t p = __builtin_elementwise_fma(t, (f32x2_t)(1.061405429f), (f32x2_t)(-1.453152027f));
    p = __builtin_elementwise_fma(t, p, (f32x2_t)(1.421413741f)); p = __builtin_elementwise_fma(t, p, (f32x2_t)(-0.284496736f)); p = __builtin_elementwise_fma(t, p, (f32x2_t)(0.254829592f));
    p = p * t;
    const f32x2_t q = (x * x) * -1.44269504088896340736f;
    const f32x2_t e = {__builtin_amdgcn_exp2f(q.x), __builtin_amdgcn_exp2f(q.y)};
    p = (p * 0.5f) * e;
    const f32x2_t one_m = (f32x2_t)(1.0f) - p;
    const f32x2_t ph = {v.x < 0.0f ? p.x : one_m.x, v.y < 0.0f ? p.y : one_m.y};
    return v * ph;
}
__device__ __forceinline__ unsigned s8x2_to_bf16x2(int lo, int hi) {
    return (__float_as_uint((float)lo) >> 16) | (__float_as_uint((float)hi) & 0xFFFF0000u);
}
#define TR_STAMP(i) do { if (a.stamps && tid == 0) { a.stamps[(size_t)blockIdx.x * 128 + (i)] = wall_clock64(); a.stamps[(size_t)blockIdx.x * 128 + 64 + (i)] = clock64(); } } while (0)
constexpr int TR_THREADS = 256, TR_PRM = 5 * 128;
constexpr int TR_ZROWS = 16;
constexpr int TR_XTRA = 64;
constexpr size_t trunk_lds_bytes(int rows, bool resg = false) { return (size_t)((resg ? 1 : 2) * rows + TR_ZROWS) * 256 + 2 * TR_PRM * 4 + TR_XTRA; }

template <bool M16> __device__ __forceinline__ int swz_slot(int g, int row) { return M16 ? (((g & 1) << 3) | ((g >> 1) ^ (row & 7))) : (g ^ (row & 15)); }
template <bool M16> __device__ __forceinline__ int swz_inv(int sp, int row) { return M16 ? ((((sp & 7) ^ (row & 7)) << 1) | (sp >> 3)) : (sp ^ (row & 15)); }

template <int TM, int WN, int RING, bool STEM, bool HEADS, bool RESG = false, bool M16 = false, int NW = 4, bool B0 = false, int SKIPSET = 0, bool S0 = false>
__device__ __forceinline__ void trunk_tile(const TrunkArgs& a, const long m0_, const int tile_rows, const uint8_t* perm = nullptr, const unsigned boffp = 0) {
    static_assert(!S0 || (B0 && TM == 2 && WN == 2), "in-kernel 256-channel stem: block-0 variant, 64 x 64 wave tile");
    long m0 = m0_;
    static_assert(!B0 || (M16 && !STEM && !HEADS && !RESG), "block 0 inside the launch: 16x16x32 build with both images in LDS");
    static_assert(SKIPSET == 0 || (STEM && HEADS && M16), "board offsets in the image: only where the kernel itself maps image rows to global rows");
    constexpr int SL0 = B0 ? 29 : 0;
    constexpr int BN = 128, SLOTS = 16, WM = NW / WN, TN = 4 / WN, KS = 8, ROWS = 32 * TM * WM, ZROW = ROWS, BSL = BN * SLOTS, THREADS = 64 * NW;
    static_assert(NW == 4 || (!STEM && !HEADS), "stem / heads phases assume four waves");
    static_assert(KS % RING == 0, "ring slot must not depend on the tap");
    extern __shared__ uint4 lds[];
    uint4* As = lds;
    uint4* Xs = lds + (ROWS + TR_ZROWS) * SLOTS;
    float* Ps = reinterpret_cast<float*>(Xs + (RESG ? 0 : ROWS * SLOTS));
    volatile int* Xt = reinterpret_cast<volatile int*>(Ps + 2 * TR_PRM);
    static_assert(!RESG || (!STEM && !HEADS), "the stem / heads phases work on the x image");
    constexpr int NB = TM >= 4 ? 2 : 4, PD = NB - 1;
    char* Ab = reinterpret_cast<char*>(As);
    char* Xb = reinterpret_cast<char*>(Xs);

    const int tid = threadIdx.x, lane = tid & 63, wave = tid >> 6;
    const int wm = wave / WN, wn = wave % WN, l31 = lane & 31, lhi = lane >> 5;
    const int HW = a.H * a.W;
    auto cell_yx = [&](const int cell, int& y, int& x) { y = (int)(((unsigned)cell * (unsigned)Xt[4]) >> 16); x = cell - y * a.W; };
    if (tid == 0) {
        Xt[4] = (int)((65536u + (unsigned)a.W - 1u) / (unsigned)a.W); Xt[5] = (int)((65536u + (unsigned)HW - 1u) / (unsigned)HW);
        Xt[6] = (int)((unsigned)m0_ / (unsigned)HW);
    }
    auto locate = [&](const int row, int& cell, long& grow, const unsigned bo = 0xFFFFFFFFu) -> bool {
        const unsigned boffq = bo == 0xFFFFFFFFu ? boffp : bo;
        if constexpr (SKIPSET == 0) {
            cell = row - (int)(((unsigned)row * (unsigned)Xt[5]) >> 16) * HW; grow = m0 + row;
            return row < tile_rows && grow < a.M;
        } else {
            bool ok = false; cell = 0; grow = 0;
#pragma unroll
            for (int b = 0; b < 3; ++b) {
                const int o = (int)((boffq >> (8 * b)) & 0xFFu);
                if (b * HW < tile_rows && row >= o && row < o + HW) {
                    cell = row - o;
                    const long gb = a.queue ? (long)Xt[1 + b] : (long)(Xt[6] + b);
                    ok = gb >= 0; grow = gb * HW + cell;
                }
            }
            return ok && grow < a.M;
        }
    };
    const uint4* in4 = reinterpret_cast<const uint4*>(a.xin);
    const int last_slice = SL0 + a.nblocks * 18 - 1;
    TR_STAMP(0);

    constexpr int n_slots = ROWS * SLOTS;
    auto load_x0_half = [&](int half) {
        const uint4* x04 = reinterpret_cast<const uint4*>(a.x0);
        for (int base = wave * 64; base < n_slots; base += THREADS) {
            const int i = base + lane, lr = i / SLOTS, sp = i % SLOTS;
// ... 30 lines not shown
    if (!M16)
#pragma unroll
    for (int g = 0; g < RING; ++g)
#pragma unroll
        for (int tn = 0; tn < TN; ++tn) bfr[g][tn] = ldb(0, g, tn);

    int lrow[TM]; unsigned vmask[TM];
#pragma unroll
    for (int tm = 0; tm < TM; ++tm) lrow[tm] = (wm * TM + tm) * 32 + l31;
    auto img_off = [&](int tm, int tn, int j) -> int {
        const int row = lrow[tm], cslot = (wn * TN + tn) * 4 + j;
        return row * 256 + (swz_slot<M16>(cslot, row) << 4) + lhi * 8;
    };
    if ((STEM || S0) && (a.ready || a.queue)) {
        if (tid == 0) Xt[0] = 0;
        const long b = (long)((unsigned)m0_ / (unsigned)HW) + tid;
        if (tid < tile_rows / HW) {
            int game = -1;
            if (b * HW < a.M) {
                bool fail = a.test_fault_mod && blockIdx.x % a.test_fault_mod == 1;
                auto arrived = [&]() -> bool {
                    if ((SKIPSET != 0 || S0) && a.queue) {
                        const unsigned long long v = __hip_atomic_load(a.queue + b, __ATOMIC_RELAXED, __HIP_MEMORY_SCOPE_SYSTEM);
                        game = (int)(unsigned)v;
                        return (unsigned)(v >> 32) == a.epoch;
                    }
                    game = (int)b;
                    return (int)(__hip_atomic_load(a.ready + b, __ATOMIC_RELAXED, __HIP_MEMORY_SCOPE_SYSTEM) - a.epoch) >= 0;
                };
                if (!fail && !arrived()) {
                    const unsigned long long t0 = wall_clock64();
                    fail = a.fuse_fault && __hip_atomic_load(a.fuse_fault, __ATOMIC_RELAXED, __HIP_MEMORY_SCOPE_SYSTEM) != 0;
                    while (!fail && !arrived()) {
                        __builtin_amdgcn_s_sleep(16);
                        fail = wall_clock64() - t0 > (unsigned long long)a.spin_ticks;
                    }
                }
                if (fail) { Xt[0] = 1; game = -1; }
                else if (S0) {
                    __builtin_amdgcn_fence(__ATOMIC_ACQUIRE, "agent");
                    asm volatile("s_waitcnt vmcnt(0)" ::: "memory");
                }
            }
            Xt[1 + tid] = game;
        }
        asm volatile("" ::: "memory");
    }
    __syncthreads();
    if ((STEM || S0) && (a.ready || a.queue)) {
        if (__builtin_amdgcn_readfirstlane(Xt[0])) {
            if (tid == 0 && a.fuse_fault) atomicAdd(a.fuse_fault, 1);
            return;
        }
        if (tid < tile_rows / HW && Xt[1 + tid] >= 0 && a.eval_done) a.eval_done[Xt[1 + tid]] = a.epoch;
        if (S0 && a.queue) m0 = (long)__builtin_amdgcn_readfirstlane(Xt[1]) * HW;
    }
#pragma unroll
    for (int tm = 0; tm < TM; ++tm) {
        unsigned mm = 0;
        int cell; long grow_;
        if (locate(lrow[tm], cell, grow_)) {
            int y, x; cell_yx(cell, y, x);
#pragma unroll
            for (int t = 0; t < 9; ++t) {
                const int dy = t / 3 - 1, dx = t % 3 - 1;
                mm |= (((unsigned)(y + dy) < (unsigned)a.H && (unsigned)(x + dx) < (unsigned)a.W) ? 1u : 0u) << t;
            }
        }
        vmask[tm] = mm;
    }
    TR_STAMP(1);

    f32x16 acc[TM][TN];
    if (STEM) {
        const int* in32 = reinterpret_cast<const int*>(a.planes);
        uint4 sw[6][TN];
#pragma unroll
        for (int ks2 = 0; ks2 < 6; ++ks2)
#pragma unroll
            for (int tn = 0; tn < TN; ++tn) sw[ks2][tn] = a.stem_frag[(ks2 * 2 + lhi) * 128 + col0 + tn * 32];
#pragma unroll
        for (int tm = 0; tm < TM; ++tm) {
            int cell_; long gr;
            const bool rok = locate(lrow[tm], cell_, gr);
            uint4 cf[3];
#pragma unroll
            for (int ks = 0; ks < 3; ++ks) {
                int pl[8];
#pragma unroll
                for (int h = 0; h < 2; ++h) {
                    const int tap = ks * 4 + lhi * 2 + h;
                    const int dy = tap / 3 - 1, dx = tap - (tap / 3) * 3 - 1;
                    int packed = 0;
                    if (rok && tap < 9 && ((vmask[tm] >> tap) & 1u))
                        packed = (a.ready || a.queue) ? __hip_atomic_load(in32 + (gr + dy * a.W + dx), __ATOMIC_RELAXED, __HIP_MEMORY_SCOPE_SYSTEM) : in32[gr + dy * a.W + dx];
#pragma unroll
                    for (int c = 0; c < 4; ++c) pl[h * 4 + c] = (int)(int8_t)((packed >> (8 * c)) & 0xFF);
                }
                cf[ks] = make_uint4(s8x2_to_bf16x2(pl[0], pl[1]), s8x2_to_bf16x2(pl[2], pl[3]), s8x2_to_bf16x2(pl[4], pl[5]), s8x2_to_bf16x2(pl[6], pl[7]));
            }
#pragma unroll
            for (int tn = 0; tn < TN; ++tn) {
#pragma unroll
                for (int r = 0; r < 16; ++r) acc[tm][tn][r] = 0.0f;
#pragma unroll
                for (int ks2 = 0; ks2 < 6; ++ks2)
                    acc[tm][tn] = __builtin_amdgcn_mfma_f32_32x32x16_bf16(*reinterpret_cast<const bf16x8*>(&sw[ks2][tn]), *reinterpret_cast<const bf16x8*>(&cf[ks2 % 3]), acc[tm][tn], 0, 0, 0);
// ... 533 lines not shown
        int hcell; long hgr;
        const bool hok = locate(hrow, hcell, hgr, boh);
        if (hok) {
            int y, x; cell_yx(hcell, y, x);
#pragma unroll
            for (int t = 0; t < 9; ++t) {
                const int dy = t / 3 - 1, dx = t % 3 - 1;
                hmask |= (((unsigned)(y + dy) < (unsigned)a.H && (unsigned)(x + dx) < (unsigned)a.W) ? 1u : 0u) << t;
            }
        }
        float4 hbi[2], hsc[2], hsh[2];
#pragma unroll
        for (int j = 0; j < 2; ++j) { hbi[j] = hsc[j] = hsh[j] = make_float4(0.0f, 0.0f, 0.0f, 0.0f); }
        if (hok) {
            const int f = hcell * 8 + 4 * lhih;
#pragma unroll
            for (int j = 0; j < 2; ++j) {
                hbi[j] = *reinterpret_cast<const float4*>(a.hbias + 8 * j + 4 * lhih);
                hsc[j] = *reinterpret_cast<const float4*>((j ? a.v_fs : a.p_fs) + f);
                hsh[j] = *reinterpret_cast<const float4*>((j ? a.v_ft : a.p_ft) + f);
            }
        }
        if (waveh * 32 < ROWS) {
        f32x16 hacc;
#pragma unroll
        for (int r = 0; r < 16; ++r) hacc[r] = 0.0f;
#pragma unroll 1
        for (int t3 = 0; t3 < 3; ++t3) {
#pragma unroll
            for (int tt = 0; tt < 3; ++tt) {
                const int tap = t3 * 3 + tt, off = (t3 - 1) * a.W + (tt - 1);
                const bool ok = (hmask >> tap) & 1u;
                const int ar = hrow + off;
                const int pbh = (ok ? ROWS + TR_ZROWS + ar : ZROW + (ar & 15)) * 256 + (swz_slot<M16>(lhih, ar) << 4);
                uint4 hf[KS];
#pragma unroll
                for (int ks = 0; ks < KS; ++ks) hf[ks] = *reinterpret_cast<const uint4*>(Ab + (pbh ^ (ks * (M16 ? 16 : 32))));
#pragma unroll
                for (int ks = 0; ks < KS; ++ks) {
                    hacc = __builtin_amdgcn_mfma_f32_32x32x16_bf16(*reinterpret_cast<bf16x8*>(&hfr[tt * KS + ks]), *reinterpret_cast<bf16x8*>(&hf[ks]), hacc, 0, 0, 0);
                    const int ntap = tap + 3 < 9 ? tap + 3 : tap;
                    hfr[tt * KS + ks] = ldh(ntap, ks);
                }
            }
        }
        const long gr = hgr;
        if (hok) {
#pragma unroll
            for (int j = 0; j < 2; ++j) {
                const float4 bi = hbi[j], sc = hsc[j], sh = hsh[j];
                float4 o;
                o.x = fmaxf((hacc[4 * j + 0] + bi.x) * sc.x + sh.x, 0.0f); o.y = fmaxf((hacc[4 * j + 1] + bi.y) * sc.y + sh.y, 0.0f);
                o.z = fmaxf((hacc[4 * j + 2] + bi.z) * sc.z + sh.z, 0.0f); o.w = fmaxf((hacc[4 * j + 3] + bi.w) * sc.w + sh.w, 0.0f);
                *reinterpret_cast<float4*>((j ? a.v_feat : a.p_feat) + (size_t)gr * 8 + 4 * lhih) = o;
            }
        }
        }
    } else if (!RESG) {
    uint4* out4 = reinterpret_cast<uint4*>(a.xout);
    for (int i = tid; i < tile_rows * SLOTS; i += THREADS) {
        const int lr = i / SLOTS, sp = i % SLOTS;
        const long gr = m0 + lr;
        if (gr < a.M) out4[gr * SLOTS + sp] = Xs[lr * SLOTS + swz_slot<M16>(sp, lr)];
    }
    }
    TR_STAMP(63);
}

template <int TM, int WN, int RING, int OCC, bool STEM, bool HEADS, bool RESG = false, bool M16 = false, int NW = 4, bool B0 = false, int SKIPSET = 0, bool S0 = false>
__global__ __launch_bounds__(64 * NW, OCC) void k_trunk(TrunkArgs a) {
    trunk_tile<TM, WN, RING, STEM, HEADS, RESG, M16, NW, B0, SKIPSET, S0>(a, (long)blockIdx.x * a.tile_rows, a.tile_rows, SKIPSET ? a.perm : nullptr, a.boff);
}
constexpr size_t trunk_lds_bytes_s0() { return trunk_lds_bytes(256) + 4 * 2 * 2 * 64 * 16; }

template <int RING, int OCC, bool STEM, bool HEADS, bool M16 = false, bool SKIP = false>
__global__ __launch_bounds__(TR_THREADS, OCC) void k_trunk_mix(TrunkArgs a) {
    if ((int)blockIdx.x < a.n_big) trunk_tile<2, 2, RING, STEM, HEADS, false, M16, 4, false, SKIP ? 1 : 0>(a, (long)blockIdx.x * a.tile_rows, a.tile_rows, SKIP ? a.perm : nullptr, a.boff);
    else trunk_tile<3, 4, RING, STEM, HEADS, false, M16, 4, false, SKIP ? 2 : 0>(a, (long)a.n_big * a.tile_rows + (long)((int)blockIdx.x - a.n_big) * a.small_rows, a.small_rows, SKIP ? a.perm_small : nullptr, a.boff_small);
}

}
```

### grok_alpha_zero_amd/engine.py

```python
import ctypes as C
import os

import numpy as np

_PKG = os.path.dirname(os.path.abspath(__file__))
DEFAULT_LIB = os.path.join(_PKG, "libgaz_engine.so")

GAME_IDS = {"TicTacToe": 0, "Connect4": 1, "Gomoku": 2}
GAME_DIMS = {0: (3, 3, 2, 9), 1: (6, 7, 4, 7), 2: (15, 15, 2, 225)}
SEARCH_PUCT, SEARCH_GUMBEL = 0, 1
EVAL_HASH, EVAL_RESNET, EVAL_EXTERNAL = 0, 1, 2
PH_WAIT_HOST, PH_HALT, PH_IDLE = 5, 8, 9


ABI_VERSION = 10


class EngineConfig(C.Structure):
    _fields_ = [("struct_size", C.c_uint32), ("game", C.c_int32), ("search", C.c_int32), ("n_games", C.c_int32), ("run_iterations", C.c_int32),
                ("max_actions", C.c_int32), ("num_explore_actions_first", C.c_int32), ("num_explore_actions_second", C.c_int32),
                ("c_puct_init", C.c_double), ("c_puct_base", C.c_double), ("dirichlet_alpha", C.c_double),
                ("dirichlet_epsilon", C.c_double), ("use_dirichlet", C.c_int32), ("create_new_root", C.c_int32),
                ("sync_moves", C.c_int32), ("nodes_per_tree", C.c_int32), ("ring_capacity", C.c_int32),
                ("seed", C.c_uint64), ("slot_offset", C.c_uint32), ("evaluator", C.c_int32), ("hash_salt", C.c_uint32),
# ... 47 lines not shown
def load_library(lib_path=None):
    path = lib_path or os.environ.get("GAZ_ENGINE_LIB") or DEFAULT_LIB
    if path in _LIBS:
        return _LIBS[path]
    if not os.path.exists(path):
        raise RuntimeError(f"{path} not found: build the HIP engine first (python -c 'import __graft_entry__ as g; g.build()'); "
                           "there is no CPU fallback")
    L = C.CDLL(path)
    H = C.c_void_p
    L.gaz_engine_abi_version.restype = C.c_int; L.gaz_engine_config_size.restype = C.c_int
    if L.gaz_engine_abi_version() != ABI_VERSION or L.gaz_engine_config_size() != C.sizeof(EngineConfig):
        raise RuntimeError(f"{path}: ABI version {L.gaz_engine_abi_version()} / config size {L.gaz_engine_config_size()} does not match "
                           f"this binding ({ABI_VERSION} / {C.sizeof(EngineConfig)}): rebuild the library")
    L.gaz_engine_create.argtypes = [C.POINTER(EngineConfig), C.POINTER(H)]
    L.gaz_engine_destroy.argtypes = [H]; L.gaz_engine_destroy.restype = None
    L.gaz_engine_last_error.argtypes = [H]; L.gaz_engine_last_error.restype = C.c_char_p
    L.gaz_engine_load_weights.argtypes = [H, C.POINTER(Tensor), C.c_int32]
    L.gaz_engine_reset_games.argtypes = [H, C.POINTER(C.c_int32), C.c_int32]
    L.gaz_engine_run_move.argtypes = [H, C.POINTER(C.c_int32)]
    L.gaz_engine_get_root_stats.argtypes = [H] + [C.c_void_p] * 8
    L.gaz_engine_apply_moves.argtypes = [H, C.POINTER(C.c_int32)]
    L.gaz_engine_run_waves.argtypes = [H, C.c_int32]
    L.gaz_engine_wave_begin.argtypes = [H]
    L.gaz_engine_wave_end.argtypes = [H]
    L.gaz_engine_batch_ptrs.argtypes = [H, C.POINTER(C.c_void_p), C.POINTER(C.c_void_p), C.POINTER(C.c_void_p)]
    L.gaz_engine_read_batch.argtypes = [H, C.c_void_p, C.c_void_p]
    L.gaz_engine_write_outputs.argtypes = [H, C.c_void_p, C.c_void_p]
    L.gaz_engine_batch_rows.argtypes = [H, C.POINTER(C.c_int32)]
    L.gaz_engine_evaluate.argtypes = [H, C.c_void_p, C.c_int32, C.c_void_p, C.c_void_p, C.c_int32, C.POINTER(C.c_double)]
    L.gaz_engine_record_layout.argtypes = [H, C.POINTER(RecordLayout)]
    L.gaz_engine_drain_finished.argtypes = [H, C.c_void_p, C.c_int32, C.POINTER(C.c_int32)]
    L.gaz_engine_sample_layout.argtypes = [H, C.POINTER(SampleLayout)]
    L.gaz_engine_drain_samples.argtypes = [H, C.c_int32, C.c_int64, C.c_void_p, C.c_void_p, C.c_void_p, C.c_void_p,
                                           C.POINTER(C.c_int32), C.POINTER(C.c_int64)]
    L.gaz_engine_get_stats.argtypes = [H, C.POINTER(C.c_uint64)]
    L.gaz_engine_synchronize.argtypes = [H]
    L.gaz_engine_timing_reset.argtypes = [H, C.c_int32]
    L.gaz_engine_set_position.argtypes = [H, C.c_int32, C.POINTER(C.c_int32), C.c_int32]
    L.gaz_engine_set_search_params.argtypes = [H, C.c_int32, C.c_int32]
    L.gaz_engine_stop_search.argtypes = [H, C.c_int32]
    L.gaz_engine_start_search.argtypes = [H]
    L.gaz_engine_set_hyperparams.argtypes = [H, C.POINTER(SearchHyperparams)]
    L.gaz_engine_set_resignation.argtypes = [H, C.POINTER(ResignParams)]
    L.gaz_engine_get_resign_stats.argtypes = [H, C.POINTER(C.c_uint64)]
    L.gaz_engine_set_eval_symmetry.argtypes = [H, C.c_int32]
    L.gaz_engine_get_eval_symmetry.argtypes = [H, C.POINTER(C.c_int32)]
    L.gaz_engine_read_batch_symmetry.argtypes = [H, C.c_void_p]
    L.gaz_engine_set_solver.argtypes = [H, C.c_int32]
    L.gaz_engine_get_solver.argtypes = [H, C.POINTER(C.c_int32)]
    L.gaz_engine_get_solver_stats.argtypes = [H, C.POINTER(C.c_uint64)]
    L.gaz_engine_probe_rules.argtypes = [H, C.c_void_p, C.c_void_p, C.c_int32, C.c_int32] + [C.c_void_p] * 7
    L.gaz_engine_set_fused_wave.argtypes = [H, C.c_int32]
    L.gaz_engine_debug_fused_fault.argtypes = [H, C.c_int32]
    L.gaz_engine_read_positions.argtypes = [H, C.c_void_p, C.c_void_p, C.c_int32]
    L.gaz_engine_repack.argtypes = [H, C.POINTER(C.c_int32), C.POINTER(C.c_int32)]
    L.gaz_engine_read_trees.argtypes = [H, C.c_void_p, C.c_int32, C.c_int32, C.c_int32, C.c_uint32, C.c_int64, C.c_int64] + [C.c_void_p] * 4
    L.gaz_engine_read_pv.argtypes = [H, C.c_int32, C.c_void_p, C.c_int32] + [C.c_void_p] * 4
    L.gaz_engine_read_head_features.argtypes = [H, C.c_int32, C.c_void_p, C.c_void_p, C.POINTER(C.c_int32), C.POINTER(C.c_int32)]
    L.gaz_engine_dominant_kernel.argtypes = [H, C.c_char_p, C.c_int32, C.POINTER(C.c_double)]
    L.gaz_engine_timing_get.argtypes = [H, C.POINTER(C.c_double), C.POINTER(C.c_double), C.POINTER(C.c_double),
                                        C.POINTER(C.c_int64), C.POINTER(C.c_int64)]
    for f in ("create", "load_weights", "reset_games", "run_move", "get_root_stats", "apply_moves", "run_waves", "wave_begin",
              "wave_end", "batch_ptrs", "read_batch", "write_outputs", "batch_rows", "evaluate", "record_layout", "drain_finished", "sample_layout", "drain_samples", "get_stats",
              "synchronize", "timing_reset", "timing_get", "dominant_kernel", "set_position", "set_search_params", "start_search", "stop_search",
              "set_hyperparams", "set_resignation", "get_resign_stats", "set_eval_symmetry", "get_eval_symmetry", "read_batch_symmetry", "set_solver", "get_solver", "get_solver_stats", "probe_rules", "read_head_features", "set_fused_wave", "debug_fused_fault", "read_positions", "repack", "read_trees", "read_pv"):
        getattr(L, "gaz_engine_" + f).restype = C.c_int
    _LIBS[path] = L
    return L


class EngineError(RuntimeError):
    pass


class SampleBatch:

    def __init__(self, games, boards, policies, values):
        self.games, self.boards, self.policies, self.values = games, boards, policies, values

    @property
    def n(self):
        return self.games.shape[0]

    def __len__(self):
        return self.games.shape[0]

    @property
    def rows(self):
        return self.values.shape[0]

    @property
    def nbytes(self):
        return self.games.nbytes + self.boards.nbytes + self.policies.nbytes + self.values.nbytes

    def copy(self):
        return SampleBatch(self.games.copy(), self.boards.copy(), self.policies.copy(), self.values.copy())

    def game(self, i):
        T, winner, r0 = int(self.games[i, 0]), int(self.games[i, 1]), int(self.games[i, 4]) - int(self.games[0, 4])
        n = T - int(self.games[i, 5])
        v = np.broadcast_to(self.values[None, r0:r0 + n], (self.policies.shape[0], n, 1))
        return self.boards[:, r0:r0 + n], self.policies[:, r0:r0 + n], v, T, T, winner


class SearchTree:

# ... 312 lines not shown
            self._ck(self.L.gaz_engine_sample_layout(self.h, C.byref(sl)))
            cap_games = max(int(self.cfg.ring_capacity), 1)
            row_bytes = sl.n_aug * (sl.state_bytes + 4 * sl.A) + 4
            cap_rows = max(min(cap_games * sl.max_T, self.sample_buffer_bytes // row_bytes), sl.max_T)
            self._sbuf = (sl, cap_games, cap_rows, np.empty((cap_games, 6), np.int32), np.empty((sl.n_aug, cap_rows, self.H, self.W, self.Cc), np.int8),
                          np.empty((sl.n_aug, cap_rows, sl.A), np.float32), np.empty((cap_rows, 1), np.float32))
        sl, cap_games, cap_rows, games, boards, policies, values = self._sbuf
        n, r = C.c_int32(), C.c_int64()
        take_rows, b, p = cap_rows, boards, policies
        if max_rows is not None and int(max_rows) < cap_rows:
            take_rows = int(max_rows)
            b = np.empty((sl.n_aug, max(take_rows, 1), self.H, self.W, self.Cc), np.int8)
            p = np.empty((sl.n_aug, max(take_rows, 1), sl.A), np.float32)
        self._ck(self.L.gaz_engine_drain_samples(self.h, min(int(max_games), cap_games) if max_games else cap_games, take_rows, games.ctypes.data,
                                                 b.ctypes.data, p.ctypes.data, values.ctypes.data, C.byref(n), C.byref(r)))
        return SampleBatch(games[:n.value], b[:, :r.value], p[:, :r.value], values[:r.value])

    def decode_record(self, raw):
        lay, A = self.layout, self.A
        hdr = raw[lay.off_hdr:lay.off_hdr + 16].view(np.int32)
        T, winner, slot, seq = (int(x) for x in hdr)

        def arr(off, dt, shape):
            n = int(np.prod(shape)) * np.dtype(dt).itemsize
            return raw[off:off + n].view(dt).reshape(shape).copy()
        actions = arr(lay.off_actions, np.uint8, (lay.t_pad,))[:T].astype(np.int32)
        q = arr(lay.off_q, np.float32, (lay.max_T,))[:T]
        mover = np.where(np.arange(T) % 2 == 0, -1, 1)
        z = (mover * winner).astype(np.float32)
        raw_kind = arr(lay.off_move_kind, np.uint8, (lay.t_pad,))[:T]
        resigned_at = np.flatnonzero(raw_kind & MK_RESIGNED)
        return dict(T=T, winner=winner, slot=slot, game_seq=seq, actions=actions, q=q, z=z,
                    values=(np.float32(0.5) * (z + q)).astype(np.float32),
                    policies=arr(lay.off_policy, np.float32, (lay.max_T, A))[:T],
                    root_N=arr(lay.off_N, np.uint32, (lay.max_T, A))[:T], root_W=arr(lay.off_W, np.float32, (lay.max_T, A))[:T],
                    root_P=arr(lay.off_P, np.float32, (lay.max_T, A))[:T],
                    root_visits=arr(lay.off_root_visits, np.uint32, (lay.max_T,))[:T],
                    evals=arr(lay.off_evals, np.uint32, (lay.max_T,))[:T],
                    move_kind=raw_kind & np.uint8(MK_KIND_MASK), proven=(raw_kind & np.uint8(MK_PROVEN)) != 0, resigned=bool(resigned_at.size),
                    resign_ply=int(resigned_at[0]) if resigned_at.size else -1,
                    would_resign_plies=np.flatnonzero(raw_kind & MK_WOULD_RESIGN).astype(np.int32))

    def repack(self):
        a, b = C.c_int32(), C.c_int32()
        self._ck(self.L.gaz_engine_repack(self.h, C.byref(a), C.byref(b)))
        return a.value, b.value

    def set_fused_wave(self, on=True):
        self._ck(self.L.gaz_engine_set_fused_wave(self.h, int(bool(on))))

    def debug_fused_fault(self, mod):
        self._ck(self.L.gaz_engine_debug_fused_fault(self.h, int(mod)))

    def timing_reset(self, enable=True):
        self._ck(self.L.gaz_engine_timing_reset(self.h, int(enable)))

    def dominant_kernel(self):
        buf = C.create_string_buffer(1024); fl = C.c_double()
        self._ck(self.L.gaz_engine_dominant_kernel(self.h, buf, 1024, C.byref(fl)))
        return buf.value.decode(), fl.value

    def timing(self):
        a, b, c = C.c_double(), C.c_double(), C.c_double()
        d, e = C.c_int64(), C.c_int64()
        self._ck(self.L.gaz_engine_timing_get(self.h, C.byref(a), C.byref(b), C.byref(c), C.byref(d), C.byref(e)))
        return dict(ms_tree=a.value, ms_eval=b.value, ms_dominant=c.value, n_dominant=d.value, n_waves=e.value)
```

### include/gaz_engine.h

```cpp
#ifndef GAZ_ENGINE_H
#define GAZ_ENGINE_H
#include <stdint.h>
#ifdef __cplusplus
extern "C" {
#endif

typedef struct gaz_engine gaz_engine;

enum { GAZ_GAME_TICTACTOE = 0, GAZ_GAME_CONNECT4 = 1, GAZ_GAME_GOMOKU = 2 };
enum { GAZ_SEARCH_PUCT = 0, GAZ_SEARCH_GUMBEL = 1 };
enum { GAZ_EVAL_HASH = 0,
       GAZ_EVAL_RESNET = 1,
       GAZ_EVAL_EXTERNAL = 2    };

#define GAZ_ENGINE_ABI_VERSION 10

typedef struct {
    uint32_t struct_size;
    int32_t game;
    int32_t search;
    int32_t n_games;
    int32_t run_iterations;
    int32_t max_actions;
    int32_t num_explore_actions_first, num_explore_actions_second;
// ... 79 lines not shown
int gaz_engine_read_batch(gaz_engine* h, int8_t* inputs, int32_t* pending);
int gaz_engine_write_outputs(gaz_engine* h, const float* policy, const float* value);
int gaz_engine_batch_rows(gaz_engine* h, int32_t* rows);

int gaz_engine_set_eval_symmetry(gaz_engine* h, int32_t mode);
int gaz_engine_get_eval_symmetry(gaz_engine* h, int32_t* mode);
int gaz_engine_read_batch_symmetry(gaz_engine* h, uint8_t* sym);

int gaz_engine_set_solver(gaz_engine* h, int32_t mode);
int gaz_engine_get_solver(gaz_engine* h, int32_t* mode);
int gaz_engine_get_solver_stats(gaz_engine* h, uint64_t out[8]);

int gaz_engine_set_position(gaz_engine* h, int32_t slot, const int32_t* actions, int32_t n);
int gaz_engine_set_search_params(gaz_engine* h, int32_t run_iterations, int32_t tau_mode);
int gaz_engine_set_hyperparams(gaz_engine* h, const gaz_search_hyperparams* hp);
typedef struct {
    uint32_t struct_size;
    int32_t consecutive;
    int32_t min_ply;
    int32_t reserved_;
    double threshold;
    double no_resign_prob;
} gaz_resign_params;
int gaz_engine_set_resignation(gaz_engine* h, const gaz_resign_params* p);
int gaz_engine_get_resign_stats(gaz_engine* h, uint64_t out[8]);
int gaz_engine_stop_search(gaz_engine* h, int32_t stop);

int gaz_engine_start_search(gaz_engine* h);

int gaz_engine_probe_rules(gaz_engine* h, const int32_t* actions, const int32_t* n_actions, int32_t n_positions, int32_t stride,
                           int8_t* board, uint8_t* legal, int32_t* winner, int8_t* input, int32_t* terminal,
                           const float* policy_in, float* policy_out);

int gaz_engine_evaluate(gaz_engine* h, const int8_t* inputs, int32_t n, float* policy, float* value, int32_t repeats, double* ms_per_batch);

int gaz_engine_read_head_features(gaz_engine* h, int32_t n, float* p_feat, float* v_feat, int32_t* p_row_floats, int32_t* v_row_floats);

int gaz_engine_record_layout(gaz_engine* h, gaz_record_layout* out);
int gaz_engine_drain_finished(gaz_engine* h, void* out, int32_t max_records, int32_t* n_out);

typedef struct { int32_t n_aug, state_bytes, A, max_T; } gaz_sample_layout;
int gaz_engine_sample_layout(gaz_engine* h, gaz_sample_layout* out);
int gaz_engine_drain_samples(gaz_engine* h, int32_t max_games, int64_t max_rows,
                             int32_t* games, int8_t* boards, float* policies, float* values,
                             int32_t* n_games, int64_t* n_rows);

int gaz_engine_get_stats(gaz_engine* h, uint64_t out[16]);
int gaz_engine_synchronize(gaz_engine* h);

int gaz_engine_set_fused_wave(gaz_engine* h, int32_t on);

int gaz_engine_debug_fused_fault(gaz_engine* h, int32_t mod);

int gaz_engine_repack(gaz_engine* h, int32_t* n_active, int32_t* n_launch);

int gaz_engine_read_positions(gaz_engine* h, int32_t* n_hist, uint8_t* hist, int32_t stride);

typedef struct {
    int32_t parent;
    int32_t slot;
    int32_t depth;
    int32_t edge0;
    int32_t n_actions;
    int32_t n_children;
    int32_t flags;
    int32_t n_reserved;
    int32_t player;
    int32_t action;
    int32_t n_hist;
    int32_t reserved_;
} gaz_tree_node;
typedef struct {
    int32_t action;
    uint32_t N;
    float W;
    float P;
    float raw;
    int32_t child;
} gaz_tree_edge;
enum { GAZ_TREE_CHILD_NONE = -1, GAZ_TREE_CHILD_DRAW = -2, GAZ_TREE_CHILD_WIN = -3, GAZ_TREE_CHILD_FILTERED = -4 };

int gaz_engine_read_trees(gaz_engine* h, const int32_t* slots, int32_t n_slots, int32_t tree, int32_t max_depth, uint32_t min_visits,
                          int64_t max_nodes, int64_t max_edges, gaz_tree_node* nodes, gaz_tree_edge* edges,
                          int64_t* node_first , int64_t* edge_first );
int gaz_engine_read_pv(gaz_engine* h, int32_t tree, const int32_t* first_action , int32_t max_len,
                       uint8_t* actions, uint32_t* N, float* W , int32_t* len );

int gaz_engine_timing_reset(gaz_engine* h, int32_t enable);
int gaz_engine_dominant_kernel(gaz_engine* h, char* name, int32_t cap, double* flops_per_launch);
int gaz_engine_timing_get(gaz_engine* h, double* ms_tree, double* ms_eval, double* ms_dominant, int64_t* n_dominant, int64_t* n_waves);

#ifdef __cplusplus
}
#endif
#endif
```

Measured before the change: 70120 positions/s.

## Run Connect4 policy/value heads inside the fused tree+trunk launch

Moves the Connect4 head MLP (previously a separate k_heads_c4 launch after the trunk) into the fused wave/trunk kernel. Each trunk tile atomically counts finished games per 32-position item using epoch-tagged counters, and the workgroup that completes an item runs both heads for it in LDS, then publishes eval_done. This removes a separate kernel launch and its serialization point, letting tree work consume evaluations sooner. In exchange it adds atomics, a fence, extra LDS pressure and per-tile tail work that can unbalance workgroups. A debug counter API is added to report how many head items ran in-launch.

```diff
diff --git a/grok_alpha_zero_amd/build.py b/grok_alpha_zero_amd/build.py
--- a/grok_alpha_zero_amd/build.py
+++ b/grok_alpha_zero_amd/build.py
@@ -9,7 +9,7 @@
 HEADER = os.path.join(os.path.dirname(_PKG), "include", "gaz_engine.h")
 UNITS = {
     "engine.hip": ["rt.hpp", "wave.hpp", "det.hpp", "games.hpp", "tree.hpp", "resign.hpp", "puct_core.hpp", "gumbel_core.hpp", "evaluator.hpp", "samples.hpp", "tree_export.hpp"],
-    "resnet.hip": ["rt.hpp", "wave.hpp", "evaluator.hpp", "netops.hpp", "conv3x3.hpp", "conv_wide.hpp", "resblock.hpp", "trunk.hpp", "tile_perm.hpp", "net_host.hpp",
+    "resnet.hip": ["rt.hpp", "wave.hpp", "evaluator.hpp", "netops.hpp", "conv3x3.hpp", "conv_wide.hpp", "resblock.hpp", "trunk.hpp", "heads_c4.hpp", "tile_perm.hpp", "net_host.hpp",
                    "det.hpp", "games.hpp", "tree.hpp", "resign.hpp", "puct_core.hpp", "gumbel_core.hpp"],
 }
 FLAGS = ["-O3", "--offload-arch=gfx950", "-fPIC", "-std=c++17", "-ffp-contract=off", "-Wno-unused-result", "-Wno-unused-value",
diff --git a/grok_alpha_zero_amd/csrc/engine.hip b/grok_alpha_zero_amd/csrc/engine.hip
--- a/grok_alpha_zero_amd/csrc/engine.hip
+++ b/grok_alpha_zero_amd/csrc/engine.hip
@@ -364,6 +364,7 @@
     virtual int read_head_features(int, float*, float*, int32_t*, int32_t*) = 0;
     virtual int set_fused_wave(int) = 0;
     virtual int debug_fused_fault(int) = 0;
+    virtual int debug_heads_in_launch(uint64_t*) = 0;
     virtual int read_positions(int32_t*, uint8_t*, int) = 0;
     typedef std::function<int(int64_t n_nodes, int64_t n_edges, gaz_tree_node** nodes, gaz_tree_edge** edges)> TreePlace;
     virtual int read_trees(const int32_t* slots, int n_slots, int tree, int max_depth, uint32_t min_visits, int64_t* node_first, int64_t* edge_first,
@@ -658,6 +659,16 @@
 
     uint32_t* d_done = nullptr; uint32_t* d_evaldone = nullptr; int32_t* d_fault = nullptr;
     unsigned long long* d_queue = nullptr;
+    unsigned long long* d_hitems = nullptr; unsigned long long* d_hrun = nullptr;
+    int debug_heads_in_launch(uint64_t* out) override {
+        *out = 0;
+        if (!d_hrun) return 0;
+        if (quiesce()) return 1;
+        unsigned long long n = 0;
+        HIP_OK(hipMemcpy(&n, d_hrun, sizeof(n), hipMemcpyDeviceToHost));
+        *out = n;
+        return 0;
+    }
     uint32_t fuse_epoch = 0; int fuse_state = -1;
     uint64_t fuse_faults = 0;
     unsigned debug_fault_mod = 0;
@@ -694,6 +705,7 @@
         if (!gumbel && !env_on("GAZ_TREE_TEAMS", true)) return false;
         if (dalloc(&d_done, (size_t)E.n_games) || !ensure_skip_buffers()) return false;
         if (env_on("GAZ_FUSE_QUEUE", true) && dalloc(&d_queue, (size_t)E.n_games + 64)) return false;
+        if (G::ID == GAME_C4 && !gumbel && (dalloc(&d_hitems, (size_t)(E.n_games + 31) / 32) || dalloc(&d_hrun, 1))) return false;
         fuse_state = 1;
         return true;
     }
@@ -758,7 +770,7 @@
         unsigned long long* d_stamps = nullptr;
         const size_t stamp_blocks = (size_t)n_eff + 4096;
         if (stamp_spec && n_waves_total == stamp_at && hipMalloc((void**)&d_stamps, stamp_blocks * 128 * 8) == hipSuccess) hipMemsetAsync(d_stamps, 0, stamp_blocks * 128 * 8, stream);
-        const FuseHandoff ho{d_done, fuse_epoch + 1, d_evaldone, d_fault, SPIN_TICKS, debug_fault_mod, d_stamps, d_queue};
+        const FuseHandoff ho{d_done, fuse_epoch + 1, d_evaldone, d_fault, SPIN_TICKS, debug_fault_mod, d_stamps, d_queue, d_hitems, d_hrun, E.nn_policy, E.nn_value, stream};
         const void* plan = eval->trunk_plan(E.nn_in, n_eff, 0, ho);
         if (!plan) return -1;
         if (timing) hipEventRecord(e0, stream);
@@ -784,7 +796,7 @@
             if (FILE* f = fopen(path.c_str(), "wb")) { fwrite(hst.data(), 8, hst.size(), f); fclose(f); }
         }
         if (timing) hipEventRecord(e1, stream);
-        eval->forward_heads(stream, E.nn_policy, E.nn_value, n_eff, 0);
+        if (!eval->plan_runs_heads(plan)) eval->forward_heads(stream, E.nn_policy, E.nn_value, n_eff, 0);
         if (E.cache) { Ef.eval_done = d_evaldone; GAZ_LAUNCH(k_cache_insert<G>, n_eff, WAVE, stream, Ef, 0, n_eff); E.cache_epoch++; }
         if (timing) {
             hipEventRecord(e2, stream); ev_eval.push_back({e0, e2}); n_waves_timed++;
@@ -1575,6 +1587,11 @@
     }
     int set_fused_wave(int on) override { return all(&gaz_engine::set_fused_wave, on); }
     int debug_fused_fault(int mod) override { return all(&gaz_engine::debug_fused_fault, mod); }
+    int debug_heads_in_launch(uint64_t* out) override {
+        *out = 0;
+        for (int c = 0; c < K(); ++c) { uint64_t n = 0; if (up(kid[c], kid[c]->debug_heads_in_launch(&n))) return 1; *out += n; }
+        return 0;
+    }
     int read_positions(int32_t* n_hist, uint8_t* hist, int stride) override {
         if (!n_hist || !hist || stride < lay.max_T) return fail("read_positions: hist must hold at least max_T actions per slot");
         return each([&](gaz_engine* k, int c) { return k->read_positions(n_hist + first[c], hist + (size_t)first[c] * stride, stride); });
@@ -1730,6 +1747,7 @@
 int gaz_engine_read_batch_symmetry(gaz_engine* h, uint8_t* sym) { return sym ? h->read_batch_symmetry(sym) : h->fail("read_batch_symmetry: null argument"); }
 int gaz_engine_set_fused_wave(gaz_engine* h, int32_t on) { return h->set_fused_wave(on); }
 int gaz_engine_debug_fused_fault(gaz_engine* h, int32_t mod) { return h->debug_fused_fault(mod); }
+int gaz_engine_debug_heads_in_launch(gaz_engine* h, uint64_t* n_items) { return n_items ? h->debug_heads_in_launch(n_items) : h->fail("debug_heads_in_launch: null argument"); }
 int gaz_engine_read_positions(gaz_engine* h, int32_t* n_hist, uint8_t* hist, int32_t stride) { return h->read_positions(n_hist, hist, stride); }
 static int check_tree_arg(gaz_engine* h, const char* fn, int32_t tree) {
     if (tree < -1 || tree > 1) return h->fail(std::string(fn) + ": tree must be 0, 1 or -1 (the tree running the game's move), not " + std::to_string(tree));
diff --git a/grok_alpha_zero_amd/csrc/evaluator.hpp b/grok_alpha_zero_amd/csrc/evaluator.hpp
--- a/grok_alpha_zero_amd/csrc/evaluator.hpp
+++ b/grok_alpha_zero_amd/csrc/evaluator.hpp
@@ -7,7 +7,8 @@
 
 struct FuseHandoff { const unsigned* ready; unsigned epoch; unsigned* eval_done; int* fuse_fault; unsigned spin_ticks; unsigned test_fault_mod;
                      unsigned long long* stamps;
-                     const unsigned long long* queue; };
+                     const unsigned long long* queue;
+                     unsigned long long* heads_items; unsigned long long* heads_run; float* policy; float* value; hipStream_t stream; };
 
 struct Evaluator {
     virtual ~Evaluator() {}
@@ -20,6 +21,7 @@
     virtual void forward_heads(hipStream_t s, float* policy, float* value, int n, int p0) { (void)s; (void)policy; (void)value; (void)n; (void)p0; }
     virtual const void* trunk_plan(const int8_t* in, int n, int p0, const struct FuseHandoff& h) { (void)in; (void)n; (void)p0; (void)h; return nullptr; }
     virtual bool plan_uses_queue(const void* plan) const { (void)plan; return false; }
+    virtual bool plan_runs_heads(const void* plan) const { (void)plan; return false; }
     virtual void set_shared_chip(bool on) { (void)on; }
     virtual bool ready() const { return true; }
     virtual void timing_reset() {}
diff --git a/grok_alpha_zero_amd/csrc/heads_c4.hpp b/grok_alpha_zero_amd/csrc/heads_c4.hpp
--- /dev/null
+++ b/grok_alpha_zero_amd/csrc/heads_c4.hpp
@@ -0,0 +1,154 @@
+#pragma once
+#include <hip/hip_runtime.h>
+#include <algorithm>
+
+namespace gaz {
+
+__device__ __forceinline__ float policy_entry(const float* lg, int nout, int o, int logits) {
+    if (logits == 1) return lg[o];
+    if (logits == 2) {
+        float sum = 0.f;
+        for (int k = 0; k < nout; ++k) { const float x = lg[k]; sum += x >= 0.0f ? x + 1.0f : 1.0f / (1.0f - x); }
+        const float x = lg[o];
+        return (x >= 0.0f ? x + 1.0f : 1.0f / (1.0f - x)) / sum;
+    }
+    float mx = lg[0];
+    for (int k = 1; k < nout; ++k) mx = fmaxf(mx, lg[k]);
+    float sum = 0.f;
+    for (int k = 0; k < nout; ++k) sum += expf(lg[k] - mx);
+    return expf(lg[o] - mx) / sum;
+}
+
+struct HeadsC4Args {
+    const float* feat[2]; const float* w1[2]; const float* s1[2]; const float* t1[2];
+    const float* w2[2]; const float* b2[2]; const float* w3[2]; const float* b3[2];
+    float* policy; float* value; int B, F, A, logits;
+};
+struct HeadsInLaunch { HeadsC4Args h; unsigned long long* items; unsigned long long* n_run; };
+
+constexpr int HC4_THREADS = 256, HC4_POS = 32, HC4_XP = 132;
+constexpr int HC4_FCH = 6, HC4_TAIL = 128 * 64 + HC4_POS * 64 + HC4_POS * 8;
+constexpr size_t heads_c4_lds_bytes(int F) { return (size_t)((HC4_POS * (F + 1) > HC4_TAIL ? HC4_POS * (F + 1) : HC4_TAIL) + HC4_POS * HC4_XP + 64 * 8) * 4; }
+
+#ifndef GAZ_HEADS_ITEM_ATTR
+#define GAZ_HEADS_ITEM_ATTR __forceinline__
+#endif
+template <class ARGS> __device__ GAZ_HEADS_ITEM_ATTR void heads_c4_item(ARGS& a, const int item, float* const fl) {
+    typedef __attribute__((ext_vector_type(4))) float f32x4;
+    constexpr int D = 12;
+    const int tid = threadIdx.x, F = a.F, FP = F + 1, F4 = F >> 2;
+    float* const w2l = fl; float* const hl = fl + 128 * 64; float* const lg = hl + HC4_POS * 64;
+    float* const xl = fl + max(HC4_POS * FP, HC4_TAIL);
+    float* const w3l = xl + HC4_POS * HC4_XP;
+    const int lane = tid & 63, wave = tid >> 6, c = lane & 15, kq = lane >> 4, half = wave >> 1, n0 = (wave & 1) * 64 + c * 4;
+    const int NG = F >> 4, NGH = (NG + 1) / 2, sA = half ? NGH * 4 : 0, sB = half ? NG * 4 : NGH * 4;
+    const int p = tid >> 3, q = tid & 7;
+    const int head = item & 1, b0 = (item >> 1) * HC4_POS, nout = head == 0 ? a.A : 1;
+    const float* feat = a.feat[head]; const float* w1 = a.w1[head]; const float* w3 = a.w3[head];
+    float4 bq[D]; f32x4 wv[8];
+    auto ldw = [&](int s) { return *reinterpret_cast<const float4*>(w1 + (size_t)min(4 * s + kq, F - 1) * 128 + n0); };
+#pragma unroll
+    for (int d = 0; d < D - 1; ++d) bq[d] = ldw(sA + d);
+    {
+        float w3v[2];
+#pragma unroll
+        for (int i = 0; i < 2; ++i) w3v[i] = w3[min(tid + HC4_THREADS * i, 64 * nout - 1)];
+#pragma unroll 1
+        for (int e0 = tid; e0 < HC4_POS * F4; e0 += HC4_THREADS * HC4_FCH) {
+            float4 fv[HC4_FCH];
+#pragma unroll
+            for (int i = 0; i < HC4_FCH; ++i) {
+                const int e = min(e0 + HC4_THREADS * i, HC4_POS * F4 - 1), r = e / F4;
+                fv[i] = reinterpret_cast<const float4*>(feat + (size_t)min(b0 + r, a.B - 1) * F)[e - r * F4];
+            }
+#pragma unroll
+            for (int i = 0; i < HC4_FCH; ++i) {
+                const int e = e0 + HC4_THREADS * i, r = e / F4, k = (e - r * F4) * 4;
+                if (e < HC4_POS * F4) {
+                    const bool rok = b0 + r < a.B;
+                    float* dst = fl + r * FP + k;
+                    dst[0] = rok ? fv[i].x : 0.0f; dst[1] = rok ? fv[i].y : 0.0f; dst[2] = rok ? fv[i].z : 0.0f; dst[3] = rok ? fv[i].w : 0.0f;
+                }
+            }
+        }
+#pragma unroll
+        for (int i = 0; i < 2; ++i) w3l[tid + HC4_THREADS * i] = w3v[i];
+#pragma unroll
+        for (int i = 0; i < 8; ++i) wv[i] = reinterpret_cast<const f32x4*>(a.w2[head])[tid + HC4_THREADS * i];
+    }
+    __syncthreads();
+    f32x4 acc[2][4];
+#pragma unroll
+    for (int m = 0; m < 2; ++m)
+#pragma unroll
+        for (int t = 0; t < 4; ++t) acc[m][t] = f32x4{0.0f, 0.0f, 0.0f, 0.0f};
+    for (int s0 = sA; s0 < sB; s0 += D) {
+#pragma unroll
+        for (int d = 0; d < D; ++d) {
+            const int s = s0 + d;
+            if (s + D - 1 < sB) bq[(d + D - 1) % D] = ldw(s + D - 1);
+            if (s < sB) {
+#pragma unroll
+                for (int m = 0; m < 2; ++m) {
+                    const float av = fl[(16 * m + c) * FP + 4 * s + kq];
+                    acc[m][0] = __builtin_amdgcn_mfma_f32_16x16x4f32(av, bq[d].x, acc[m][0], 0, 0, 0);
+                    acc[m][1] = __builtin_amdgcn_mfma_f32_16x16x4f32(av, bq[d].y, acc[m][1], 0, 0, 0);
+                    acc[m][2] = __builtin_amdgcn_mfma_f32_16x16x4f32(av, bq[d].z, acc[m][2], 0, 0, 0);
+                    acc[m][3] = __builtin_amdgcn_mfma_f32_16x16x4f32(av, bq[d].w, acc[m][3], 0, 0, 0);
+                }
+            }
+        }
+    }
+    if (half) {
+#pragma unroll
+        for (int m = 0; m < 2; ++m)
+#pragma unroll
+            for (int r = 0; r < 4; ++r)
+                *reinterpret_cast<float4*>(&xl[(16 * m + 4 * kq + r) * HC4_XP + n0]) = make_float4(acc[m][0][r], acc[m][1][r], acc[m][2][r], acc[m][3][r]);
+    }
+    __syncthreads();
+    if (!half) {
+        const float4 s = *reinterpret_cast<const float4*>(a.s1[head] + n0), t = *reinterpret_cast<const float4*>(a.t1[head] + n0);
+#pragma unroll
+        for (int m = 0; m < 2; ++m)
+#pragma unroll
+            for (int r = 0; r < 4; ++r) {
+                float4* x = reinterpret_cast<float4*>(&xl[(16 * m + 4 * kq + r) * HC4_XP + n0]);
+                const float4 pv = *x;
+                *x = make_float4(fmaxf((acc[m][0][r] + pv.x) * s.x + t.x, 0.0f), fmaxf((acc[m][1][r] + pv.y) * s.y + t.y, 0.0f),
+                                 fmaxf((acc[m][2][r] + pv.z) * s.z + t.z, 0.0f), fmaxf((acc[m][3][r] + pv.w) * s.w + t.w, 0.0f));
+            }
+    }
+#pragma unroll
+    for (int i = 0; i < 8; ++i) reinterpret_cast<f32x4*>(w2l)[tid + HC4_THREADS * i] = wv[i];
+    __syncthreads();
+    {
+        const float* b2 = a.b2[head];
+        float h[8];
+#pragma unroll
+        for (int j = 0; j < 8; ++j) h[j] = b2[q * 8 + j];
+        for (int k = 0; k < 128; ++k) {
+            const float xv = xl[p * HC4_XP + k];
+            const float4 wa = *reinterpret_cast<const float4*>(&w2l[k * 64 + q * 8]), wb = *reinterpret_cast<const float4*>(&w2l[k * 64 + q * 8 + 4]);
+            h[0] += xv * wa.x; h[1] += xv * wa.y; h[2] += xv * wa.z; h[3] += xv * wa.w;
+            h[4] += xv * wb.x; h[5] += xv * wb.y; h[6] += xv * wb.z; h[7] += xv * wb.w;
+        }
+#pragma unroll
+        for (int j = 0; j < 8; ++j) hl[p * 64 + q * 8 + j] = h[j];
+    }
+    __syncthreads();
+    for (int o = q; o < nout; o += 8) {
+        float z = a.b3[head][o];
+        for (int k = 0; k < 64; ++k) z += hl[p * 64 + k] * w3l[k * nout + o];
+        lg[p * 8 + o] = z;
+    }
+    __syncthreads();
+    const int b = b0 + p;
+    if (b < a.B) {
+        if (head == 0) { for (int o = q; o < nout; o += 8) a.policy[(size_t)b * a.A + o] = policy_entry(lg + p * 8, nout, o, a.logits); }
+        else if (q == 0) a.value[b] = tanhf(lg[p * 8]);
+    }
+    __syncthreads();
+}
+
+}
diff --git a/grok_alpha_zero_amd/csrc/resnet.hip b/grok_alpha_zero_amd/csrc/resnet.hip
--- a/grok_alpha_zero_amd/csrc/resnet.hip
+++ b/grok_alpha_zero_amd/csrc/resnet.hip
@@ -357,20 +357,6 @@
     const float* v_w2; const float* v_b2; const float* v_w3; const float* v_b3;
     float* policy; float* value; int B, A, logits;
 };
-__device__ __forceinline__ float policy_entry(const float* lg, int nout, int o, int logits) {
-    if (logits == 1) return lg[o];
-    if (logits == 2) {
-        float sum = 0.f;
-        for (int k = 0; k < nout; ++k) { const float x = lg[k]; sum += x >= 0.0f ? x + 1.0f : 1.0f / (1.0f - x); }
-        const float x = lg[o];
-        return (x >= 0.0f ? x + 1.0f : 1.0f / (1.0f - x)) / sum;
-    }
-    float mx = lg[0];
-    for (int k = 1; k < nout; ++k) mx = fmaxf(mx, lg[k]);
-    float sum = 0.f;
-    for (int k = 0; k < nout; ++k) sum += expf(lg[k] - mx);
-    return expf(lg[o] - mx) / sum;
-}
 __global__ __launch_bounds__(128) void k_tail(TailArgs a) {
     __shared__ float w2l[128 * 64]; __shared__ float xl[16][128]; __shared__ float hl[16][64]; __shared__ float lg[16][64];
     __shared__ float w3l[64 * 8];
@@ -429,134 +415,10 @@
     }
 }
 
-struct HeadsC4Args {
-    const float* feat[2]; const float* w1[2]; const float* s1[2]; const float* t1[2];
-    const float* w2[2]; const float* b2[2]; const float* w3[2]; const float* b3[2];
-    float* policy; float* value; int B, F, A, logits;
-};
-constexpr int HC4_THREADS = 256, HC4_POS = 32, HC4_XP = 132;
-constexpr int HC4_FCH = 6, HC4_TAIL = 128 * 64 + HC4_POS * 64 + HC4_POS * 8;
-static size_t heads_c4_lds_bytes(int F) { return (size_t)(std::max(HC4_POS * (F + 1), HC4_TAIL) + HC4_POS * HC4_XP + 64 * 8) * 4; }
 __global__ __launch_bounds__(HC4_THREADS) void k_heads_c4(HeadsC4Args a) {
-    typedef __attribute__((ext_vector_type(4))) float f32x4;
     extern __shared__ float fl[];
-    constexpr int D = 12;
-    const int tid = threadIdx.x, F = a.F, FP = F + 1, F4 = F >> 2;
-    float* const w2l = fl; float* const hl = fl + 128 * 64; float* const lg = hl + HC4_POS * 64;
-    float* const xl = fl + max(HC4_POS * FP, HC4_TAIL);
-    float* const w3l = xl + HC4_POS * HC4_XP;
-    const int lane = tid & 63, wave = tid >> 6, c = lane & 15, kq = lane >> 4, half = wave >> 1, n0 = (wave & 1) * 64 + c * 4;
-    const int NG = F >> 4, NGH = (NG + 1) / 2, sA = half ? NGH * 4 : 0, sB = half ? NG * 4 : NGH * 4;
-    const int p = tid >> 3, q = tid & 7;
     const int items = 2 * ((a.B + HC4_POS - 1) / HC4_POS);
-    for (int item = blockIdx.x; item < items; item += gridDim.x) {
-        const int head = item & 1, b0 = (item >> 1) * HC4_POS, nout = head == 0 ? a.A : 1;
-        const float* feat = a.feat[head]; const float* w1 = a.w1[head]; const float* w3 = a.w3[head];
-        float4 bq[D]; f32x4 wv[8];
-        auto ldw = [&](int s) { return *reinterpret_cast<const float4*>(w1 + (size_t)min(4 * s + kq, F - 1) * 128 + n0); };
-#pragma unroll
-        for (int d = 0; d < D - 1; ++d) bq[d] = ldw(sA + d);
-        {
-            float w3v[2];
-#pragma unroll
-            for (int i = 0; i < 2; ++i) w3v[i] = w3[min(tid + HC4_THREADS * i, 64 * nout - 1)];
-#pragma unroll 1
-            for (int e0 = tid; e0 < HC4_POS * F4; e0 += HC4_THREADS * HC4_FCH) {
-                float4 fv[HC4_FCH];
-#pragma unroll
-                for (int i = 0; i < HC4_FCH; ++i) {
-                    const int e = min(e0 + HC4_THREADS * i, HC4_POS * F4 - 1), r = e / F4;
-                    fv[i] = reinterpret_cast<const float4*>(feat + (size_t)min(b0 + r, a.B - 1) * F)[e - r * F4];
-                }
-#pragma unroll
-                for (int i = 0; i < HC4_FCH; ++i) {
-                    const int e = e0 + HC4_THREADS * i, r = e / F4, k = (e - r * F4) * 4;
-                    if (e < HC4_POS * F4) {
-                        const bool rok = b0 + r < a.B;
-                        float* dst = fl + r * FP + k;
-                        dst[0] = rok ? fv[i].x : 0.0f; dst[1] = rok ? fv[i].y : 0.0f; dst[2] = rok ? fv[i].z : 0.0f; dst[3] = rok ? fv[i].w : 0.0f;
-                    }
-                }
-            }
-#pragma unroll
-            for (int i = 0; i < 2; ++i) w3l[tid + HC4_THREADS * i] = w3v[i];
-#pragma unroll
-            for (int i = 0; i < 8; ++i) wv[i] = reinterpret_cast<const f32x4*>(a.w2[head])[tid + HC4_THREADS * i];
-        }
-        __syncthreads();
-        f32x4 acc[2][4];
-#pragma unroll
-        for (int m = 0; m < 2; ++m)
-#pragma unroll
-            for (int t = 0; t < 4; ++t) acc[m][t] = f32x4{0.0f, 0.0f, 0.0f, 0.0f};
-        for (int s0 = sA; s0 < sB; s0 += D) {
-#pragma unroll
-            for (int d = 0; d < D; ++d) {
-                const int s = s0 + d;
-                if (s + D - 1 < sB) bq[(d + D - 1) % D] = ldw(s + D - 1);
-                if (s < sB) {
-#pragma unroll
-                    for (int m = 0; m < 2; ++m) {
-                        const float av = fl[(16 * m + c) * FP + 4 * s + kq];
-                        acc[m][0] = __builtin_amdgcn_mfma_f32_16x16x4f32(av, bq[d].x, acc[m][0], 0, 0, 0);
-                        acc[m][1] = __builtin_amdgcn_mfma_f32_16x16x4f32(av, bq[d].y, acc[m][1], 0, 0, 0);
-                        acc[m][2] = __builtin_amdgcn_mfma_f32_16x16x4f32(av, bq[d].z, acc[m][2], 0, 0, 0);
-                        acc[m][3] = __builtin_amdgcn_mfma_f32_16x16x4f32(av, bq[d].w, acc[m][3], 0, 0, 0);
-                    }
-                }
-            }
-        }
-        if (half) {
-#pragma unroll
-            for (int m = 0; m < 2; ++m)
-#pragma unroll
-                for (int r = 0; r < 4; ++r)
-                    *reinterpret_cast<float4*>(&xl[(16 * m + 4 * kq + r) * HC4_XP + n0]) = make_float4(acc[m][0][r], acc[m][1][r], acc[m][2][r], acc[m][3][r]);
-        }
-        __syncthreads();
-        if (!half) {
-            const float4 s = *reinterpret_cast<const float4*>(a.s1[head] + n0), t = *reinterpret_cast<const float4*>(a.t1[head] + n0);
-#pragma unroll
-            for (int m = 0; m < 2; ++m)
-#pragma unroll
-                for (int r = 0; r < 4; ++r) {
-                    float4* x = reinterpret_cast<float4*>(&xl[(16 * m + 4 * kq + r) * HC4_XP + n0]);
-                    const float4 pv = *x;
-                    *x = make_float4(fmaxf((acc[m][0][r] + pv.x) * s.x + t.x, 0.0f), fmaxf((acc[m][1][r] + pv.y) * s.y + t.y, 0.0f),
-                                     fmaxf((acc[m][2][r] + pv.z) * s.z + t.z, 0.0f), fmaxf((acc[m][3][r] + pv.w) * s.w + t.w, 0.0f));
-                }
-        }
-#pragma unroll
-        for (int i = 0; i < 8; ++i) reinterpret_cast<f32x4*>(w2l)[tid + HC4_THREADS * i] = wv[i];
-        __syncthreads();
-        {
-            const float* b2 = a.b2[head];
-            float h[8];
-#pragma unroll
-            for (int j = 0; j < 8; ++j) h[j] = b2[q * 8 + j];
-            for (int k = 0; k < 128; ++k) {
-                const float xv = xl[p * HC4_XP + k];
-                const float4 wa = *reinterpret_cast<const float4*>(&w2l[k * 64 + q * 8]), wb = *reinterpret_cast<const float4*>(&w2l[k * 64 + q * 8 + 4]);
-                h[0] += xv * wa.x; h[1] += xv * wa.y; h[2] += xv * wa.z; h[3] += xv * wa.w;
-                h[4] += xv * wb.x; h[5] += xv * wb.y; h[6] += xv * wb.z; h[7] += xv * wb.w;
-            }
-#pragma unroll
-            for (int j = 0; j < 8; ++j) hl[p * 64 + q * 8 + j] = h[j];
-        }
-        __syncthreads();
-        for (int o = q; o < nout; o += 8) {
-            float z = a.b3[head][o];
-            for (int k = 0; k < 64; ++k) z += hl[p * 64 + k] * w3l[k * nout + o];
-            lg[p * 8 + o] = z;
-        }
-        __syncthreads();
-        const int b = b0 + p;
-        if (b < a.B) {
-            if (head == 0) { for (int o = q; o < nout; o += 8) a.policy[(size_t)b * a.A + o] = policy_entry(lg + p * 8, nout, o, a.logits); }
-            else if (q == 0) a.value[b] = tanhf(lg[p * 8]);
-        }
-        __syncthreads();
-    }
+    for (int item = blockIdx.x; item < items; item += gridDim.x) heads_c4_item(a, item, fl);
 }
 
 static bool net_width_supported(int f) { return f == 64 || f == 128 || f == 192 || f == 256; }
@@ -578,6 +440,8 @@
     bool heads_one = true;
     int heads_wgs = 128;
     int heads_one_rows = 2048;
+    bool heads_in_launch = false;
+    HeadsInLaunch* hil_dev = nullptr; HeadsInLaunch hil_host;
     bf16_t* trunk_w = nullptr; float* trunk_prm = nullptr;
     std::string dom_label;
     uint8_t *perm_big = nullptr, *perm_small = nullptr;
@@ -671,9 +535,21 @@
         TrunkArgs& r = fused_plan.args;
         r.ready = h.ready; r.epoch = h.epoch; r.eval_done = h.eval_done; r.fuse_fault = h.fuse_fault; r.spin_ticks = h.spin_ticks; r.test_fault_mod = h.test_fault_mod; r.stamps = h.stamps;
         r.queue = (perm_big && perm_small && fused_plan.mix) ? h.queue : nullptr;
+        if (heads_in_launch && h.heads_items && h.eval_done && heads_c4_ok(n) && (int64_t)n * HW * 32 < (int64_t)1 << 31) {
+            HeadsInLaunch w; memset(&w, 0, sizeof(w));
+            w.h = heads_c4_args(h.policy, h.value, n, p0); w.items = h.heads_items; w.n_run = h.heads_run;
+            if (!hil_dev || memcmp(&w, &hil_host, sizeof(w)) != 0) {
+                if (!hil_dev && !(hil_dev = st.dalloc<HeadsInLaunch>(1))) return nullptr;
+                hipStreamSynchronize(h.stream);
+                if (hipMemcpy(hil_dev, &w, sizeof(w), hipMemcpyHostToDevice) != hipSuccess) return nullptr;
+                hil_host = w;
+            }
+            r.hil = hil_dev;
+        }
         return &fused_plan;
     }
     bool plan_uses_queue(const void* plan) const override { return plan && static_cast<const TrunkLaunchPlan*>(plan)->args.queue != nullptr; }
+    bool plan_runs_heads(const void* plan) const override { return plan && static_cast<const TrunkLaunchPlan*>(plan)->args.hil != nullptr; }
     bool shared_chip = false;
     bool grouped = false;
     void set_shared_chip(bool on) override { static const bool off = !env_on("GAZ_GROUP_BIG_TILES", true); shared_chip = on && !off; grouped = on; }
@@ -773,19 +649,25 @@
         h.feat_p = pfeat; h.feat_v = vfeat; h.p_fs = st.g("p.bn0.scale"); h.p_ft = st.g("p.bn0.shift"); h.v_fs = st.g("v.bn0.scale"); h.v_ft = st.g("v.bn0.shift");
         with_width(filters, [&](auto Fc) { conv_wide_launch<decltype(Fc)::value, 32, 9, 0, CW_EPI_HEADS>(s, h); });
     }
+    bool heads_c4_ok(int n) const { const int F = HW * 8; return heads_one && filters == 128 && F % 16 == 0 && F <= 384 && A <= 8 && !(grouped && n > heads_one_rows); }
+    HeadsC4Args heads_c4_args(float* policy, float* value, int n, int p0) {
+        HeadsC4Args h; memset(&h, 0, sizeof(h));
+        h.B = n; h.F = HW * 8; h.A = A; h.logits = logits; h.policy = policy; h.value = value;
+        h.feat[0] = this->pfeat + (size_t)p0 * HW * 8; h.feat[1] = this->vfeat + (size_t)p0 * HW * 8;
+        for (int i = 0; i < 2; ++i) {
+            const std::string p = i == 0 ? "p" : "v";
+            h.w1[i] = st.g(p + ".d1.w"); h.s1[i] = st.g(p + ".d1.scale"); h.t1[i] = st.g(p + ".d1.shift");
+            h.w2[i] = st.g(p + ".d2.w"); h.b2[i] = st.g(p + ".d2.bias"); h.w3[i] = st.g(p + ".d3.w"); h.b3[i] = st.g(p + ".d3.bias");
+        }
+        return h;
+    }
     void forward_heads(hipStream_t s, float* policy, float* value, int n, int p0) override {
         if (!loaded) return;
         float* const pfeat = this->pfeat + (size_t)p0 * HW * 8; float* const vfeat = this->vfeat + (size_t)p0 * HW * 8;
         float* const pd1 = this->pd1 + (size_t)p0 * 128; float* const vd1 = this->vd1 + (size_t)p0 * 128;
         const int F = HW * 8;
-        if (heads_one && filters == 128 && F % 16 == 0 && F <= 384 && A <= 8 && !(grouped && n > heads_one_rows)) {
-            HeadsC4Args h; h.B = n; h.F = F; h.A = A; h.logits = logits; h.policy = policy; h.value = value;
-            h.feat[0] = pfeat; h.feat[1] = vfeat;
-            for (int i = 0; i < 2; ++i) {
-                const std::string p = i == 0 ? "p" : "v";
-                h.w1[i] = st.g(p + ".d1.w"); h.s1[i] = st.g(p + ".d1.scale"); h.t1[i] = st.g(p + ".d1.shift");
-                h.w2[i] = st.g(p + ".d2.w"); h.b2[i] = st.g(p + ".d2.bias"); h.w3[i] = st.g(p + ".d3.w"); h.b3[i] = st.g(p + ".d3.bias");
-            }
+        if (heads_c4_ok(n)) {
+            const HeadsC4Args h = heads_c4_args(policy, value, n, p0);
             const int items = 2 * ((n + HC4_POS - 1) / HC4_POS);
             hipLaunchKernelGGL(k_heads_c4, dim3(grouped ? std::min(items, heads_wgs) : items), dim3(HC4_THREADS), heads_c4_lds_bytes(F), s, h);
             return;
@@ -1253,6 +1135,7 @@
     e->heads_one = env_on("GAZ_HEADS_ONE", true);
     e->heads_wgs = std::max(1, env_int("GAZ_HEADS_WGS", e->heads_wgs));
     e->heads_one_rows = env_int("GAZ_HEADS_ONE_ROWS", e->heads_one_rows);
+    e->heads_in_launch = env_on("GAZ_HEADS_IN_LAUNCH", false);
     { hipDeviceProp_t pr; int dev = 0; hipGetDevice(&dev); if (hipGetDeviceProperties(&pr, dev) == hipSuccess) e->n_cus = pr.multiProcessorCount; }
     e->X = e->st.dalloc<bf16_t>(M * CW + 1024); e->Aa = e->st.dalloc<bf16_t>(M * CW + 1024); e->Hh = e->st.dalloc<bf16_t>(M * CW + 1024);
     e->pfeat = e->st.dalloc<float>((size_t)cfg.n_games * e->HW * 8); e->vfeat = e->st.dalloc<float>((size_t)cfg.n_games * e->HW * 8);
@@ -1304,7 +1187,7 @@
     }
 }
 
-template <bool MIX, bool SKIP, class GP, class LOCAL, bool GUMBEL>
+template <bool MIX, bool SKIP, class GP, class LOCAL, bool GUMBEL, bool HIL = false>
 __device__ __forceinline__ void wave_trunk_body(const DevParams<GP>& E, int g0, int g1, int n_tree_blocks, const TrunkArgs& a) {
     if ((int)blockIdx.x < n_tree_blocks) {
         extern __shared__ uint4 lds[];
@@ -1315,13 +1198,13 @@
         return;
     }
     const int bid = (int)blockIdx.x - n_tree_blocks;
-    if (MIX && bid >= a.n_big) trunk_tile<3, 4, 8, true, true, false, true, 4, false, SKIP ? 2 : 0>(a, (long)a.n_big * a.tile_rows + (long)(bid - a.n_big) * a.small_rows, a.small_rows, SKIP ? a.perm_small : nullptr, a.boff_small);
-    else trunk_tile<2, 2, 8, true, true, false, true, 4, false, SKIP ? 1 : 0>(a, (long)bid * a.tile_rows, a.tile_rows, SKIP ? a.perm : nullptr, a.boff);
-}
-
-template <bool MIX, bool SKIP, bool SYM = false, bool SOLVE = false> __global__ __launch_bounds__(TR_THREADS, 2) void k_wave_trunk(DevParams<typename SolveSel<SOLVE, typename SymSel<SYM, GP4>::type>::type> E, int g0, int g1, int n_tree_blocks, TrunkArgs a) {
+    if (MIX && bid >= a.n_big) trunk_tile<3, 4, 8, true, true, false, true, 4, false, SKIP ? 2 : 0, false, HIL>(a, (long)a.n_big * a.tile_rows + (long)(bid - a.n_big) * a.small_rows, a.small_rows, SKIP ? a.perm_small : nullptr, a.boff_small);
+    else trunk_tile<2, 2, 8, true, true, false, true, 4, false, SKIP ? 1 : 0, false, HIL>(a, (long)bid * a.tile_rows, a.tile_rows, SKIP ? a.perm : nullptr, a.boff);
+}
+
+template <bool MIX, bool SKIP, bool SYM = false, bool SOLVE = false, bool HIL = false> __global__ __launch_bounds__(TR_THREADS, 2) void k_wave_trunk(DevParams<typename SolveSel<SOLVE, typename SymSel<SYM, GP4>::type>::type> E, int g0, int g1, int n_tree_blocks, TrunkArgs a) {
     typedef typename SolveSel<SOLVE, typename SymSel<SYM, GP4>::type>::type GP;
-    wave_trunk_body<MIX, SKIP, GP, PuctLocal<GP>, false>(E, g0, g1, n_tree_blocks, a);
+    wave_trunk_body<MIX, SKIP, GP, PuctLocal<GP>, false, HIL>(E, g0, g1, n_tree_blocks, a);
 }
 
 typedef Game<GAME_GMK> GGMK;
@@ -1383,19 +1266,24 @@
                                             (TR_THREADS / WAVE) * (teams ? WAVE / GP4::TEAM : 1), s, dev_params, g0, g1, plan);
 }
 
+template <bool SYM, bool SOLVE, bool HIL> static bool launch_wave_trunk_c4_v(hipStream_t s, const void* dev_params, int g0, int g1, const void* plan, bool mix, bool skip) {
+    typedef typename SolveSel<SOLVE, typename SymSel<SYM, GP4>::type>::type GPv;
+    return wave_trunk_launch<GPv>(mix && skip ? k_wave_trunk<true, true, SYM, SOLVE, HIL> : mix ? k_wave_trunk<true, false, SYM, SOLVE, HIL> : k_wave_trunk<false, false, SYM, SOLVE, HIL>,
+                                  TR_THREADS, (TR_THREADS / WAVE) * (WAVE / GP4::TEAM), s, dev_params, g0, g1, plan);
+}
+template <bool HIL> static bool launch_wave_trunk_c4_h(hipStream_t s, const void* dev_params, int g0, int g1, const void* plan, bool mix, bool skip, bool sym, bool solve) {
+    if (solve && sym) return launch_wave_trunk_c4_v<true, true, HIL>(s, dev_params, g0, g1, plan, mix, skip);
+    if (solve) return launch_wave_trunk_c4_v<false, true, HIL>(s, dev_params, g0, g1, plan, mix, skip);
+    if (sym) return launch_wave_trunk_c4_v<true, false, HIL>(s, dev_params, g0, g1, plan, mix, skip);
+    return launch_wave_trunk_c4_v<false, false, HIL>(s, dev_params, g0, g1, plan, mix, skip);
+}
 bool launch_wave_trunk_c4(hipStream_t s, const void* dev_params, int g0, int g1, const void* plan) {
     const bool sym = dev_params && static_cast<const DevParams<GP4>*>(dev_params)->eval_symmetry != 0;
     const TrunkLaunchPlan* P = static_cast<const TrunkLaunchPlan*>(plan);
     const bool mix = P && P->mix, skip = P && P->args.perm && P->args.perm_small;
     const bool solve = dev_params && static_cast<const DevParams<GP4>*>(dev_params)->solver != 0;
-    if (solve && sym) return wave_trunk_launch<WithSolve<WithSym<GP4>>>(mix && skip ? k_wave_trunk<true, true, true, true> : mix ? k_wave_trunk<true, false, true, true> : k_wave_trunk<false, false, true, true>,
-                                                                       TR_THREADS, (TR_THREADS / WAVE) * (WAVE / GP4::TEAM), s, dev_params, g0, g1, plan);
-    if (solve) return wave_trunk_launch<WithSolve<GP4>>(mix && skip ? k_wave_trunk<true, true, false, true> : mix ? k_wave_trunk<true, false, false, true> : k_wave_trunk<false, false, false, true>,
-                                                        TR_THREADS, (TR_THREADS / WAVE) * (WAVE / GP4::TEAM), s, dev_params, g0, g1, plan);
-    if (sym) return wave_trunk_launch<WithSym<GP4>>(mix && skip ? k_wave_trunk<true, true, true> : mix ? k_wave_trunk<true, false, true> : k_wave_trunk<false, false, true>, TR_THREADS,
-                                                    (TR_THREADS / WAVE) * (WAVE / GP4::TEAM), s, dev_params, g0, g1, plan);
-    return wave_trunk_launch<GP4>(mix && skip ? k_wave_trunk<true, true> : mix ? k_wave_trunk<true, false> : k_wave_trunk<false, false>, TR_THREADS,
-                                  (TR_THREADS / WAVE) * (WAVE / GP4::TEAM), s, dev_params, g0, g1, plan);
-}
-
-}
+    if (P && P->args.hil) return launch_wave_trunk_c4_h<true>(s, dev_params, g0, g1, plan, mix, skip, sym, solve);
+    return launch_wave_trunk_c4_h<false>(s, dev_params, g0, g1, plan, mix, skip, sym, solve);
+}
+
+}
diff --git a/grok_alpha_zero_amd/csrc/trunk.hpp b/grok_alpha_zero_amd/csrc/trunk.hpp
--- a/grok_alpha_zero_amd/csrc/trunk.hpp
+++ b/grok_alpha_zero_amd/csrc/trunk.hpp
@@ -1,5 +1,6 @@
 #pragma once
 #include "resblock.hpp"
+#include "heads_c4.hpp"
 
 namespace gaz {
 
@@ -21,6 +22,7 @@
     unsigned boff, boff_small;
     const bf16_t* hw; const float* hbias;
     const float* p_fs; const float* p_ft; const float* v_fs; const float* v_ft; float* p_feat; float* v_feat;
+    const HeadsInLaunch* hil;
 };
 
 struct TrunkLaunchPlan { TrunkArgs args; int nwg; int mix; unsigned lds_bytes; };
@@ -63,9 +65,11 @@
 template <bool M16> __device__ __forceinline__ int swz_slot(int g, int row) { return M16 ? (((g & 1) << 3) | ((g >> 1) ^ (row & 7))) : (g ^ (row & 15)); }
 template <bool M16> __device__ __forceinline__ int swz_inv(int sp, int row) { return M16 ? ((((sp & 7) ^ (row & 7)) << 1) | (sp >> 3)) : (sp ^ (row & 15)); }
 
-template <int TM, int WN, int RING, bool STEM, bool HEADS, bool RESG = false, bool M16 = false, int NW = 4, bool B0 = false, int SKIPSET = 0, bool S0 = false>
+template <int TM, int WN, int RING, bool STEM, bool HEADS, bool RESG = false, bool M16 = false, int NW = 4, bool B0 = false, int SKIPSET = 0, bool S0 = false, bool HIL = false>
 __device__ __forceinline__ void trunk_tile(const TrunkArgs& a, const long m0_, const int tile_rows, const uint8_t* perm = nullptr, const unsigned boffp = 0) {
     static_assert(!S0 || (B0 && TM == 2 && WN == 2), "in-kernel 256-channel stem: block-0 variant, 64 x 64 wave tile");
+    static_assert(!HIL || (STEM && HEADS && NW == 4 && HC4_THREADS == 64 * NW && heads_c4_lds_bytes(384) <= trunk_lds_bytes(128)),
+                  "heads in the launch: a whole-trunk tile of 256 threads in a launch with trunk_lds_bytes(128) of LDS, which hold a heads item's");
     long m0 = m0_;
     static_assert(!B0 || (M16 && !STEM && !HEADS && !RESG), "block 0 inside the launch: 16x16x32 build with both images in LDS");
     static_assert(SKIPSET == 0 || (STEM && HEADS && M16), "board offsets in the image: only where the kernel itself maps image rows to global rows");
@@ -202,7 +206,7 @@
             if (tid == 0 && a.fuse_fault) atomicAdd(a.fuse_fault, 1);
             return;
         }
-        if (tid < tile_rows / HW && Xt[1 + tid] >= 0 && a.eval_done) a.eval_done[Xt[1 + tid]] = a.epoch;
+        if (tid < tile_rows / HW && Xt[1 + tid] >= 0 && a.eval_done && !(HIL && a.hil)) a.eval_done[Xt[1 + tid]] = a.epoch;
         if (S0 && a.queue) m0 = (long)__builtin_amdgcn_readfirstlane(Xt[1]) * HW;
     }
 #pragma unroll
@@ -842,7 +846,56 @@
                 float4 o;
                 o.x = fmaxf((hacc[4 * j + 0] + bi.x) * sc.x + sh.x, 0.0f); o.y = fmaxf((hacc[4 * j + 1] + bi.y) * sc.y + sh.y, 0.0f);
                 o.z = fmaxf((hacc[4 * j + 2] + bi.z) * sc.z + sh.z, 0.0f); o.w = fmaxf((hacc[4 * j + 3] + bi.w) * sc.w + sh.w, 0.0f);
+                if (HIL && a.hil) {
+                    const __amdgpu_buffer_rsrc_t frs = __builtin_amdgcn_make_buffer_rsrc((void*)(j ? a.v_feat : a.p_feat), 0, a.M * 32, 0x00020000);
+                    __builtin_amdgcn_raw_buffer_store_b128(v4i_t{(int)__float_as_uint(o.x), (int)__float_as_uint(o.y), (int)__float_as_uint(o.z), (int)__float_as_uint(o.w)},
+                                                           frs, (int)gr * 32 + 16 * lhih, 0, 16);
+                } else
                 *reinterpret_cast<float4*>((j ? a.v_feat : a.p_feat) + (size_t)gr * 8 + 4 * lhih) = o;
+            }
+        }
+        }
+        if constexpr (HIL) {
+        if (a.hil) {
+            TR_STAMP(61);
+            asm volatile("s_waitcnt vmcnt(0)" ::: "memory");
+            __syncthreads();
+            typedef const __attribute__((address_space(4))) HeadsInLaunch* chil_t;
+            const chil_t hl = (chil_t)(size_t)a.hil;
+            if (tidh < 3) {
+                int done_item = -1;
+                const int game = tidh < tile_rows / HW ? Xt[1 + tidh] : -1;
+                if (game >= 0) {
+                    const int item = game / HC4_POS, target = min(HC4_POS, hl->h.B - item * HC4_POS);
+                    typedef __attribute__((address_space(1))) unsigned long long* gu64_t;
+                    const gu64_t cnt = (gu64_t)(size_t)(hl->items + item);
+                    unsigned long long old = __hip_atomic_load(cnt, __ATOMIC_RELAXED, __HIP_MEMORY_SCOPE_AGENT), nw;
+                    do { nw = (unsigned)(old >> 32) == a.epoch ? old + 1 : ((unsigned long long)a.epoch << 32) | 1ull; }
+                    while (!__hip_atomic_compare_exchange_strong(cnt, &old, nw, __ATOMIC_RELAXED, __ATOMIC_RELAXED, __HIP_MEMORY_SCOPE_AGENT));
+                    if ((int)(unsigned)nw == target) done_item = item;
+                }
+                Xt[8 + tidh] = done_item;
+            }
+            __syncthreads();
+            const int run0 = __builtin_amdgcn_readfirstlane(Xt[8]), run1 = __builtin_amdgcn_readfirstlane(Xt[9]), run2 = __builtin_amdgcn_readfirstlane(Xt[10]);
+            TR_STAMP(62);
+            if (run0 >= 0 || run1 >= 0 || run2 >= 0) {
+                if (waveh == 0) {
+                    __builtin_amdgcn_fence(__ATOMIC_ACQUIRE, "agent");
+                    asm volatile("s_waitcnt vmcnt(0)" ::: "memory");
+                }
+                __syncthreads();
+#pragma unroll 1
+                for (int k = 0; k < 6; ++k) {
+                    const int item = k < 2 ? run0 : k < 4 ? run1 : run2;
+                    if (item < 0) continue;
+                    heads_c4_item(hl->h, 2 * item + (k & 1), reinterpret_cast<float*>(lds));
+                    if (k & 1) {
+                        const int g = item * HC4_POS + tidh;
+                        if (tidh < HC4_POS && g < hl->h.B && a.eval_done) a.eval_done[g] = a.epoch;
+                        if (tidh == 0) atomicAdd(hl->n_run, 2ull);
+                    }
+                }
             }
         }
         }
diff --git a/grok_alpha_zero_amd/engine.py b/grok_alpha_zero_amd/engine.py
--- a/grok_alpha_zero_amd/engine.py
+++ b/grok_alpha_zero_amd/engine.py
@@ -123,6 +123,9 @@
     L.gaz_engine_probe_rules.argtypes = [H, C.c_void_p, C.c_void_p, C.c_int32, C.c_int32] + [C.c_void_p] * 7
     L.gaz_engine_set_fused_wave.argtypes = [H, C.c_int32]
     L.gaz_engine_debug_fused_fault.argtypes = [H, C.c_int32]
+    if hasattr(L, "gaz_engine_debug_heads_in_launch"):
+        L.gaz_engine_debug_heads_in_launch.argtypes = [H, C.POINTER(C.c_uint64)]
+        L.gaz_engine_debug_heads_in_launch.restype = C.c_int
     L.gaz_engine_read_positions.argtypes = [H, C.c_void_p, C.c_void_p, C.c_int32]
     L.gaz_engine_repack.argtypes = [H, C.POINTER(C.c_int32), C.POINTER(C.c_int32)]
     L.gaz_engine_read_trees.argtypes = [H, C.c_void_p, C.c_int32, C.c_int32, C.c_int32, C.c_uint32, C.c_int64, C.c_int64] + [C.c_void_p] * 4
@@ -541,6 +544,13 @@
     def debug_fused_fault(self, mod):
         self._ck(self.L.gaz_engine_debug_fused_fault(self.h, int(mod)))
 
+    def debug_heads_in_launch(self):
+        if not hasattr(self.L, "gaz_engine_debug_heads_in_launch"):
+            return 0
+        n = C.c_uint64()
+        self._ck(self.L.gaz_engine_debug_heads_in_launch(self.h, C.byref(n)))
+        return int(n.value)
+
     def timing_reset(self, enable=True):
         self._ck(self.L.gaz_engine_timing_reset(self.h, int(enable)))
 
diff --git a/include/gaz_engine.h b/include/gaz_engine.h
--- a/include/gaz_engine.h
+++ b/include/gaz_engine.h
@@ -155,6 +155,8 @@
 
 int gaz_engine_debug_fused_fault(gaz_engine* h, int32_t mod);
 
+int gaz_engine_debug_heads_in_launch(gaz_engine* h, uint64_t* n_items);
+
 int gaz_engine_repack(gaz_engine* h, int32_t* n_active, int32_t* n_launch);
 
 int gaz_engine_read_positions(gaz_engine* h, int32_t* n_hist, uint8_t* hist, int32_t stride);
```

After: 69780 positions/s. About the same (-0.5%).
